# sunzeyeah/item-alignment

Hardware: AMD Instinct MI355X
Metric: item-pairs/sec (train step) RoBERTa-large+ViT-B two-tower (higher is better)
Workload: dtype bf16

## Files before the change

include/itemalign.h:

```cpp
#ifndef ITEMALIGN_H
#define ITEMALIGN_H
#include <stddef.h>
#include <stdint.h>

#ifdef __cplusplus
extern "C" {
#endif

typedef struct ihipStream_t* ia_stream_t;

#define IA_OK 0
#define IA_ERR_ARG (-1)
#define IA_ERR_LAUNCH (-2)
#define IA_ERR_WORKSPACE (-3)
#define IA_ERR_UNSUPPORTED (-4)

const char* ia_strerror(int code);
#define IA_ABI_VERSION 15
int ia_abi_version(void);

#define IA_EPI_NONE 0
#define IA_EPI_BIAS 1
#define IA_EPI_BIAS_GELU 2
#define IA_EPI_ADD 3
#define IA_EPI_DGELU 4
#define IA_EPI_BIAS_ADD 5
#define IA_EPI_DGELU_COLSUM 6
#define IA_EPI_BIAS_GELU_ACT 7
int ia_gemm_bf16(const void* A, int a_kstrided, int lda, const void* B, int b_kstrided, int ldb, void* C, int c_is_f32, int ldc,
                 int M, int N, int K, int epilogue, const float* bias, const void* aux, int ldaux, void* C2, int accumulate,
                 void* workspace, size_t workspace_bytes, ia_stream_t stream);
int ia_gemm_bf16_qscale(const void* A, int lda, const void* B, int ldb, void* C, int ldc, int M, int N, int K, const float* bias,
                        int scaled_cols, float col_scale, ia_stream_t stream);
size_t ia_gemm_workspace_bytes(int M, int N, int K, int c_is_f32);
size_t ia_gemm_colsum_workspace_bytes(int M, int N);

int ia_prof_begin(int variant, int max_launches);
int ia_prof_end(double* total_ms, double* total_flops, int* launches);
double ia_prof_bytes(void);
int ia_debug_cu_hog(int workgroups, float milliseconds, ia_stream_t stream);
int ia_debug_gemm_dynamic(int on);

int ia_ln_fwd(const void* x, const float* bias, const void* residual, void* z_out, void* y, float* mean, float* rstd,
              const float* gamma, const float* beta, int M, int H, float eps, float drop_p, uint32_t seed, uint32_t stream_id,
              ia_stream_t stream);
size_t ia_ln_bwd_workspace_bytes(int M, int H);
int ia_ln_bwd(const void* dy, const void* dres, const void* z, const float* mean, const float* rstd, const float* gamma, void* dz,
              void* dx, float* dgamma, float* dbeta, float* dbias, int M, int H, float drop_p, uint32_t seed, uint32_t stream_id,
              void* workspace, size_t workspace_bytes, int accumulate, ia_stream_t stream);
int ia_ln_bwd2(const void* dy, const void* dy2, const void* dres, const void* z, const float* mean, const float* rstd, const float* gamma,
               void* dz, void* dx, float* dgamma, float* dbeta, float* dbias, int M, int H, float drop_p, uint32_t seed, uint32_t stream_id,
               void* workspace, size_t workspace_bytes, int accumulate, ia_stream_t stream);
int ia_ln_bwd2_rows(const void* dy, const void* dy2, const void* dres, const void* z, const float* mean, const float* rstd,
                    const float* gamma, void* dz, void* dx, float* dgamma, float* dbeta, float* dbias, int M, int H, float drop_p,
                    uint32_t seed, uint32_t stream_id, const uint8_t* row_live, void* workspace, size_t workspace_bytes, int accumulate,
                    ia_stream_t stream);
size_t ia_colsum_workspace_bytes(int M, int N);
int ia_colsum(const void* x, int ld, int M, int N, float* out, int accumulate, void* workspace, size_t workspace_bytes,
              ia_stream_t stream);

int ia_attn_fwd(const void* q, const void* k, const void* v, int ld_qkv, const uint8_t* key_mask, void* out, int ld_o, float* lse2,
                int B, int nh, int L, float scale, float drop_p, uint32_t seed, ia_stream_t stream);
int ia_attn_bwd(const void* q, const void* k, const void* v, int ld_qkv, const uint8_t* key_mask, const void* out, const void* d_out,
                int ld_o, const float* lse2, float* delta, void* dq, void* dk, void* dv, int ld_dqkv, int B, int nh, int L,
                float scale, float drop_p, uint32_t seed, ia_stream_t stream);
size_t ia_attn_bwd_bias_workspace_bytes(int B, int nh, int L);
int ia_attn_bwd_bias(const void* q, const void* k, const void* v, int ld_qkv, const uint8_t* key_mask, const void* out, const void* d_out,
                     int ld_o, const float* lse2, float* delta, void* dq, void* dk, void* dv, int ld_dqkv, float* dbias, void* workspace,
                     size_t workspace_bytes, int B, int nh, int L, float scale, float drop_p, uint32_t seed, ia_stream_t stream);

int ia_attn_fwd_ps(const void* q, const void* k, const void* v, int ld_qkv, const uint8_t* key_mask, void* out, int ld_o, float* lse2,
                   int B, int nh, int L, float scale, float drop_p, uint32_t seed, ia_stream_t stream);
int ia_attn_bwd_bias_ps(const void* q, const void* k, const void* v, int ld_qkv, const uint8_t* key_mask, const void* out, const void* d_out,
                        int ld_o, const float* lse2, float* delta, void* dq, void* dk, void* dv, int ld_dqkv, float* dbias, void* workspace,
                        size_t workspace_bytes, int B, int nh, int L, float scale, float drop_p, uint32_t seed, ia_stream_t stream);
#define IA_ATTN_Q_PRESCALED 1
#define IA_ATTN_MASKED_ROWS_DEAD 2
int ia_attn_bwd_bias_ex(int flags, const void* q, const void* k, const void* v, int ld_qkv, const uint8_t* key_mask, const void* out,
                        const void* d_out, int ld_o, const float* lse2, float* delta, void* dq, void* dk, void* dv, int ld_dqkv, float* dbias,
                        void* workspace, size_t workspace_bytes, int B, int nh, int L, float scale, float drop_p, uint32_t seed,
                        ia_stream_t stream);

int ia_attn_fwd_x(const void* q, int ld_q, const void* k, const void* v, int ld_kv, const uint8_t* key_mask, void* out, int ld_o,
                  float* lse2, int B, int nh, int Lq, int Lk, float scale, float drop_p, uint32_t seed, ia_stream_t stream);
int ia_attn_bwd_x(const void* q, int ld_q, const void* k, const void* v, int ld_kv, const uint8_t* key_mask, const void* out,
                  const void* d_out, int ld_o, const float* lse2, float* delta, void* dq, int ld_dq, void* dk, void* dv, int ld_dkv,
                  int B, int nh, int Lq, int Lk, float scale, float drop_p, uint32_t seed, ia_stream_t stream);

int ia_rotary_split_fwd(const void* src, int ld_src, void* q_out, void* kv_out, int M, int n, int nh, ia_stream_t stream);
int ia_rotary_split_bwd(const void* dq, const void* dkv, void* dsrc, int ld_src, int M, int n, int nh, ia_stream_t stream);
int ia_swiglu_fwd(const void* src, int ld_src, void* out, int M, int F, ia_stream_t stream);
int ia_swiglu_bwd(const void* dout, const void* src, int ld_src, void* dsrc, int ld_dsrc, int M, int F, ia_stream_t stream);

int ia_kg_gather_fwd(const float* ent_table, const float* rel_table, const int64_t* ids, int ld_ids, int ent_col, int rel_lo,
                     float* h_sign, float* r, int B, int P, int Dk, ia_stream_t stream);
int ia_kg_gather_bwd(const float* dr, const int64_t* ids, int ld_ids, int rel_lo, float* rel_grad, int B, int P, int Dk,
                     ia_stream_t stream);
int ia_kg_rows_fwd(const float* h, const float* r, const float* hp, float* rows, int rows_per_item, int row0, int B, int P, int H,
                   ia_stream_t stream);
int ia_kg_rows_bwd(const float* drows, int rows_per_item, int row0, float* dh, float* dr, float* dhp, int B, int P, int H,
                   ia_stream_t stream);

#define IA_SIM_INNER 0
#define IA_SIM_COSINE 1
#define IA_SIM_L1 2
#define IA_SIM_L2 3
int ia_pair_sim_fwd(const float* x, const float* y, float* sim, float* probs, int B, int D, int measure, ia_stream_t stream);
int ia_pair_sim_bwd(const float* x, const float* y, const float* sim, const float* probs, const float* dsim, const float* dprobs,
                    float* dx, float* dy, int B, int D, int measure, ia_stream_t stream);

int ia_nchw_to_nhwc_bf16(const float* in, void* out, int B, int C, int H, int W, int Cp, ia_stream_t stream);
size_t ia_conv_nhwc_workspace_bytes(int B, int H, int W, int C, int Cout, int k, int stride, int groups);
int ia_conv_nhwc_fwd(const void* x, const void* what, const float* bias, void* y, int B, int H, int W, int C, int Cout, int k, int stride,
                     int groups, void* workspace, size_t workspace_bytes, ia_stream_t stream);
int ia_conv_nhwc_bwd_data(const void* dy, const void* what, void* dx, int B, int H, int W, int C, int Cout, int k, int stride, int groups,
                          void* workspace, size_t workspace_bytes, ia_stream_t stream);
int ia_conv_nhwc_bwd_weight(const void* x, const void* dy, float* dwhat, float* dbias, int B, int H, int W, int C, int Cout, int k,
                            int stride, int groups, int cols_valid, void* workspace, size_t workspace_bytes, ia_stream_t stream);
int ia_ws_conv_weight_fwd(const float* w, const float* gain, void* what, float* mean, float* rstd, int Cout, int Cg, int kk, int Cgp,
                          float scale, float eps, ia_stream_t stream);
int ia_ws_conv_weight_bwd(const float* dwhat, const float* w, const float* gain, const float* mean, const float* rstd, float* dw,
                          float* dgain, int Cout, int Cg, int kk, int Cgp, float scale, ia_stream_t stream);
int ia_silu_fwd(const void* x, void* y, size_t n, float scale, ia_stream_t stream);
int ia_silu_bwd(const void* dy, const void* x, const void* dadd, void* dx, size_t n, float scale, ia_stream_t stream);
int ia_silu_bwd_sum(const void* dy, const void* dy2, const void* x, const void* dadd, void* dx, size_t n, float scale, ia_stream_t stream);
int ia_avgpool2_fwd(const void* x, void* y, int B, int H, int W, int C, ia_stream_t stream);
int ia_avgpool2_bwd(const void* dy, void* dx, int B, int H, int W, int C, ia_stream_t stream);
size_t ia_gap_workspace_bytes(int B, int HW, int C);
int ia_gap_fwd(const void* x, float* pooled, int B, int HW, int C, void* workspace, size_t workspace_bytes, ia_stream_t stream);
int ia_gap_bwd(const float* dpooled, void* dx, int B, int HW, int C, ia_stream_t stream);
int ia_eca_fwd(const void* x, const float* conv_w, int k, const void* shortcut, void* out, float* pooled, float* gate, int B, int HW, int C,
               float coef, void* workspace, size_t workspace_bytes, ia_stream_t stream);
size_t ia_eca_fwd_linear_workspace_bytes(int B, int HW, int Cmid);
int ia_eca_fwd_linear(const void* x, const void* a, const void* what, const float* bias, int Cmid, const float* conv_w, int k,
                      const void* shortcut, void* out, void* act_out, float act_scale, float* pooled, float* gate, int B, int HW, int C,
                      float coef, void* workspace, size_t workspace_bytes, ia_stream_t stream);
int ia_eca_silu_bwd(const void* dact, const void* dact2, const void* out, const void* dout_direct, float act_scale, const void* x,
                    const float* conv_w, int k, const float* pooled, const float* gate, void* dtot, void* dx, float* dconv_w, int B, int HW,
                    int C, float coef, void* workspace, size_t workspace_bytes, ia_stream_t stream);
size_t ia_eca_bwd_workspace_bytes(int B, int HW, int C);
int ia_eca_bwd(const void* dout, const void* x, const float* conv_w, int k, const float* pooled, const float* gate, void* dx,
               float* dconv_w, int B, int HW, int C, float coef, void* workspace, size_t workspace_bytes, ia_stream_t stream);

int ia_conv3x3_padded_fwd(const void* xp, const void* what, const float* bias, void* yp, int B, int H, int W, int Cin, int Cout, int groups,
                          ia_stream_t stream);
int ia_conv3x3_padded_bwd_data(const void* dyp, const void* what, void* dxp, int B, int H, int W, int Cin, int Cout, int groups,
                               ia_stream_t stream);
int ia_conv3x3_direct_supported(int Cin, int Cout, int groups);
int ia_conv3x3_flip_weights(const void* what, void* what_t, int Cin, int Cout, int groups, ia_stream_t stream);
int ia_conv3x3_padded_bwd_data_t(const void* dyp, const void* what_t, void* dxp, int B, int H, int W, int Cin, int Cout, int groups,
                                 ia_stream_t stream);
size_t ia_conv3x3_padded_workspace_bytes(int B, int H, int W, int Cin, int Cout, int groups);
int ia_conv3x3_padded_bwd_weight(const void* xp, const void* dyp, float* dwhat, float* dbias, int B, int H, int W, int Cin, int Cout,
                                 int groups, void* workspace, size_t workspace_bytes, ia_stream_t stream);
int ia_conv3x3_s2_supported(int Cin, int Cout, int groups);
size_t ia_conv3x3_s2_padded_workspace_bytes(int B, int H, int W, int Cin, int Cout, int groups);
int ia_conv3x3_s2_padded_fwd(const void* xp, const void* what, const float* bias, void* yp, int B, int H, int W, int Cin, int Cout,
                             int groups, int y_compact, ia_stream_t stream);
int ia_conv3x3_s2_padded_bwd_weight(const void* xp, const void* dyp, float* dwhat, float* dbias, int B, int H, int W, int Cin, int Cout,
                                    int groups, int y_compact, void* workspace, size_t workspace_bytes, ia_stream_t stream);
int ia_conv3x3_s2_padded_bwd_data_t(const void* dyp, const void* what_t, void* dxp, int B, int H, int W, int Cin, int Cout, int groups,
                                    int y_compact, ia_stream_t stream);
int ia_silu_pad_fwd(const void* x, void* y, int B, int H, int W, int C, float scale, int in_padded, int out_padded, ia_stream_t stream);
int ia_pad_rows(const void* x, void* y, int B, int H, int W, int C, int in_padded, int out_padded, ia_stream_t stream);
int ia_silu_pad_bwd(const void* dy, const void* x, void* dx, int B, int H, int W, int C, float scale, int in_padded, int out_padded,
                    ia_stream_t stream);

size_t ia_bn_act_workspace_bytes(int rows, int C, int segments);
int ia_bn_act_fwd(const void* x, const float* gamma, const float* beta, float* running_mean, float* running_var, void* y, float* mean,
                  float* rstd, int rows, int C, int segments, float eps, float momentum, int training, int relu, void* workspace,
                  size_t workspace_bytes, ia_stream_t stream);
int ia_bn_act_bwd(const void* dy, const void* x, const float* gamma, const float* beta, const float* mean, const float* rstd,
                  const void* extra, void* dx, float* dgamma, float* dbeta, int rows, int C, int segments, int training, int relu,
                  void* workspace, size_t workspace_bytes, ia_stream_t stream);
size_t ia_gn_act_workspace_bytes(int rows, int C, int images);
int ia_gn_act_fwd(const void* x, const float* gamma, const float* beta, void* y, float* mean, float* rstd, int rows, int C, int images,
                  int groups, float eps, int relu, void* workspace, size_t workspace_bytes, ia_stream_t stream);
int ia_gn_act_bwd(const void* dy, const void* x, const float* gamma, const float* beta, const float* mean, const float* rstd,
                  const void* extra, void* dx, float* dgamma, float* dbeta, int rows, int C, int images, int groups, int relu,
                  void* workspace, size_t workspace_bytes, ia_stream_t stream);
int ia_patches_nchw(const float* images, void* cols, int B, int C, int H, int W, int k, int stride, int pad, int Kp, ia_stream_t stream);
int ia_maxpool3s2_fwd(const void* x, void* y, uint8_t* arg, int B, int H, int W, int C, ia_stream_t stream);
int ia_maxpool3s2_fwd_ex(const void* x, void* y, uint8_t* arg, int B, int H, int W, int C, int pad_zero, ia_stream_t stream);
int ia_maxpool3s2_bwd(const void* dy, const uint8_t* arg, void* dx, int B, int H, int W, int C, ia_stream_t stream);
int ia_rows_subsample_fwd(const void* x, void* y, int B, int H, int W, int C, int stride, ia_stream_t stream);
int ia_rows_subsample_bwd(const void* dy, const void* base, void* dx, int B, int H, int W, int C, int stride, ia_stream_t stream);
int ia_conv_weight_pack(const float* w, void* what, int Cout, int Cg, int kk, int Cgp, int ldw, ia_stream_t stream);
int ia_conv_weight_unpack_grad(const float* dwhat, float* dw, int Cout, int Cg, int kk, int Cgp, int ldw, ia_stream_t stream);

int ia_resize_pass_u8(const uint8_t* src, uint8_t* dst, const int* bounds, const int* coeffs, int ksize, int B, int in_len, int out_len,
                      int other_len, int horizontal, ia_stream_t stream);
int ia_resize_pass_u8_ex(const uint8_t* src, size_t src_pitch_bytes, size_t src_frame_bytes, uint8_t* dst, const int* bounds,
                         const int* coeffs, int ksize, int B, int in_len, int out_len, int other_len, int horizontal, ia_stream_t stream);
int ia_color_jitter_step_u8(uint8_t* frames, const int* op, const float* factor, void* scratch, int B, int H, int W, int any_contrast,
                            ia_stream_t stream);
int ia_u8_to_nchw_normalized(const uint8_t* src, const uint8_t* flip, float* out, int B, int S0, int S1, const float* mean3,
                             const float* std3, ia_stream_t stream);

int ia_embed_ln_fwd(const int64_t* ids, const int64_t* type_ids, const int64_t* pos_ids, const int32_t* extra_idx, const float* word,
                    const float* type, const float* pos, const float* extra, const float* gamma, const float* beta, void* z_out,
                    void* y, float* mean, float* rstd, int M, int H, float eps, float drop_p, uint32_t seed, uint32_t stream_id,
                    ia_stream_t stream);
size_t ia_embed_ln_bwd_workspace_bytes(int M, int H);
int ia_embed_ln_bwd(const void* dy, const void* z, const float* mean, const float* rstd, const float* gamma, const int64_t* ids,
                    const int64_t* type_ids, const int64_t* pos_ids, const int32_t* extra_idx, const int32_t* row_order,
                    const int32_t* word_order, const int32_t* pos_order, const int32_t* type_order, float* dword, float* dtype, float* dpos, float* dextra, float* dgamma, float* dbeta, int M, int H, int L, int word_pad, int pos_pad,
                    float drop_p, uint32_t seed, uint32_t stream_id, void* workspace, size_t workspace_bytes, ia_stream_t stream);

int ia_im2col_patch(const float* images, void* patches, int B, int C, int S, int P, ia_stream_t stream);
int ia_vit_tokens_fwd(const void* patch, const float* cls, const float* pos, void* tokens, int B, int NP, int H, ia_stream_t stream);
int ia_vit_tokens_bwd(const void* dtokens, void* dpatch, float* dcls, float* dpos, int B, int NP, int H, int accumulate,
                      ia_stream_t stream);

int ia_gather_rows_fwd(const void* src, int ld, const int32_t* rows, float* out, int B, int H, float drop_p, uint32_t seed,
                       uint32_t stream_id, ia_stream_t stream);
int ia_gather_rows_bwd(const float* dout, int ld, const int32_t* rows, void* dsrc, int B, int H, float drop_p, uint32_t seed,
                       uint32_t stream_id, int accumulate, ia_stream_t stream);

#define IA_ACT_NONE 0
#define IA_ACT_TANH 1
int ia_linear_small_fwd(const float* x, int ldx, const float* W, const float* bias, float* y, int B, int N, int K, int act,
                        ia_stream_t stream);
int ia_linear_small_bwd(const float* dy, const float* y, const float* x, int ldx, const float* W, float* dx, int lddx, float* dW,
                        float* db, int B, int N, int K, int act, ia_stream_t stream);
int ia_pair_head_ce_fwd(const float* x, const float* y, const float* W, const float* bias, const int64_t* labels, float* logits,
                        float* probs, float* loss, float* loss_per, int B, int D, int C, ia_stream_t stream);
int ia_pair_head_ce_bwd(const float* probs, const int64_t* labels, const float* dloss, const float* x, const float* y, const float* W,
                        float* dx, float* dy, float* dW, float* db, int B, int D, int C, ia_stream_t stream);

int ia_span_mean_fwd(const void* seq, int ld, const int* spans, float* out, int S, int H, ia_stream_t stream);
int ia_span_mean_bwd(const float* dout, const int* spans, const int* span_ptr, void* dseq, int B, int L, int H, ia_stream_t stream);

int ia_attn_fwd_varlen(const void* q, const void* k, const void* v, int ld_qkv, const int* cu_seqlens, int total_tokens, void* out, int ld_o,
                       float* lse2, int B, int nh, int Lmax, float scale, float drop_p, uint32_t seed, ia_stream_t stream);
int ia_attn_bwd_varlen(const void* q, const void* k, const void* v, int ld_qkv, const int* cu_seqlens, int total_tokens, const void* out,
                       const void* d_out, int ld_o, const float* lse2, float* delta, void* dq, void* dk, void* dv, int ld_dqkv, int B, int nh,
                       int Lmax, float scale, float drop_p, uint32_t seed, ia_stream_t stream);

int ia_attn_fwd_varlen_ps(const void* q, const void* k, const void* v, int ld_qkv, const int* cu_seqlens, int total_tokens, void* out, int ld_o,
                          float* lse2, int B, int nh, int Lmax, float scale, float drop_p, uint32_t seed, ia_stream_t stream);
int ia_attn_bwd_varlen_ps(const void* q, const void* k, const void* v, int ld_qkv, const int* cu_seqlens, int total_tokens, const void* out,
                          const void* d_out, int ld_o, const float* lse2, float* delta, void* dq, void* dk, void* dv, int ld_dqkv, int B, int nh,
                          int Lmax, float scale, float drop_p, uint32_t seed, ia_stream_t stream);

int ia_transpose_bf16_batched(const void* src, void* dst, const void* table, int n, int max_tiles, ia_stream_t stream);
int ia_adamw_flat(float* params, const float* grads, float* exp_avg, float* exp_avg_sq, void* shadow_bf16, const void* chunk_table,
                  int n_chunks, float lr, float beta1, float beta2, float eps, float weight_decay, int step, float grad_scale,
                  ia_stream_t stream);
int ia_cast_f32_to_bf16(const float* src, void* dst, size_t n, ia_stream_t stream);
int ia_cast_bf16_to_f32(const void* src, float* dst, size_t n, ia_stream_t stream);

#define IA_KGPT_SCORE 0
#define IA_KGPT_GRAD 1
#define IA_KGPT_MARGIN 2
size_t ia_kgpt_workspace_bytes(int B, int D, int use_proj);
int ia_kgpt_score(const float* ent, const float* rel, const float* proj, const int64_t* h, const int64_t* t, const int64_t* r,
                  const int64_t* nh, const int64_t* nt, int B, int D, int n_ent, int n_rel, int norm, int mode, float margin,
                  const float* dpos, const float* dneg, float* pos, float* neg, float* loss, const int32_t* ent_order, const int32_t* rel_order,
                  float* dent, float* drel, float* dproj, void* workspace, size_t workspace_bytes, ia_stream_t stream);
int ia_kgpt_adam_l2(float* params, float* grads, float* exp_avg, float* exp_avg_sq, size_t n, float lr, float beta1, float beta2,
                    float eps, float weight_decay, int step, ia_stream_t stream);
int ia_kgpt_row_normalize(float* x, int rows, int D, ia_stream_t stream);
int ia_kgpt_corrupt(const int64_t* h, const int64_t* t, const int64_t* r, int n, const float* bern_probs, int n_probs, int n_ent,
                    uint64_t seed, int64_t* nh, int64_t* nt, ia_stream_t stream);
#define IA_KGPT_LP_TAIL 0
#define IA_KGPT_LP_HEAD 1
size_t ia_kgpt_lp_workspace_bytes(int B, int D);
int ia_kgpt_lp_rank(const float* ent, const float* rel, const int64_t* h, const int64_t* t, const int64_t* r, int B, int D, int n_ent,
                    int n_rel, int norm, int side, const int64_t* grp_off, const int64_t* grp_ids, int n_grp, const int64_t* q_grp,
                    int64_t* rank, int64_t* filt_rank, float* scores, void* workspace, size_t workspace_bytes, ia_stream_t stream);

typedef struct {
  const void* w_qkv;
  const float* b_qkv;
  const void* w_o;
  const float* b_o;
  const float* ln1_g;
  const float* ln1_b;
  const void* w_fc1;
  const float* b_fc1;
  const void* w_fc2;
  const float* b_fc2;
  const float* ln2_g;
  const float* ln2_b;
  const void* wt_qkv;
  const void* wt_o;
  const void* wt_fc1;
  const void* wt_fc2;
} ia_layer_weights;

typedef struct {
  float* w_qkv; float* b_qkv; float* w_o; float* b_o; float* ln1_g; float* ln1_b;
  float* w_fc1; float* b_fc1; float* w_fc2; float* b_fc2; float* ln2_g; float* ln2_b;
} ia_layer_grads;

typedef struct {
  int B, L, H, I, nh;
  int pre_ln;
  float eps;
  float hidden_drop, attn_drop;
  uint32_t seed;
  uint32_t layer_id;
  const int* cu_seqlens;
  int total_tokens;
  float* dx_colsum_out;
  int dy_colsum_done;
  int masked_rows_dead;
} ia_layer_cfg;

size_t ia_layer_stash_bytes(const ia_layer_cfg* cfg);
size_t ia_layer_bwd_scratch_bytes(const ia_layer_cfg* cfg);
int ia_layer_fwd(const ia_layer_cfg* cfg, const ia_layer_weights* w, const void* x, const uint8_t* key_mask, void* y, void* stash,
                 ia_stream_t stream);
size_t ia_layer_infer_scratch_bytes(const ia_layer_cfg* cfg);
int ia_layer_fwd_infer(const ia_layer_cfg* cfg, const ia_layer_weights* w, const void* x, const uint8_t* key_mask, void* y, void* scratch,
                       size_t scratch_bytes, ia_stream_t stream);
int ia_layer_bwd(const ia_layer_cfg* cfg, const ia_layer_weights* w, const ia_layer_grads* g, const void* x, const uint8_t* key_mask,
                 const void* y, const void* stash, const void* dy, void* dx, void* scratch, size_t scratch_bytes, ia_stream_t stream);
int ia_layer_bwd2(const ia_layer_cfg* cfg, const ia_layer_weights* w, const ia_layer_grads* g, const void* x, const uint8_t* key_mask,
                  const void* y, const void* stash, const void* dy, const void* dy2, void* dx, void* dx2, void* scratch,
                  size_t scratch_bytes, ia_stream_t stream);

#define IA_GCN_LONG_ROW 512
#define IA_GCN_SLAB_ROWS 1024
int ia_gcn_propagate_fwd(const int64_t* rowptr, const void* col, int col_is_64, const float* val, const float* x, const float* x0,
                         float* h, int N, int C, float alpha, float drop_p, uint32_t seed, uint32_t stream_id,
                         const int32_t* long_rows, int n_long, ia_stream_t stream);
int ia_gcn_propagate_bwd(const int64_t* rowptr_t, const void* col_t, int col_is_64, const float* val_t, const float* dh, float* dx,
                         float* dx0, int dx0_accumulate, int N, int C, float alpha, float drop_p, uint32_t seed, uint32_t stream_id,
                         const int32_t* long_rows_t, int n_long_t, ia_stream_t stream);
int ia_gcn_mix_fwd(const float* h, const float* W, float* out, int N, int C, float beta, float drop_p, uint32_t seed, uint32_t stream_id,
                   ia_stream_t stream);
size_t ia_gcn_workspace_bytes(int N, int C, int F);
int ia_gcn_mix_bwd(const float* dout, const float* out, const float* h, const float* W, float* dh, float* dW, int N, int C, float beta,
                   float drop_p, void* workspace, size_t workspace_bytes, ia_stream_t stream);
int ia_gcn_input_fwd(const float* X, const float* W, const float* bias, float* x0, int N, int F, int C, float drop_p, uint32_t seed,
                     uint32_t stream_id, ia_stream_t stream);
int ia_gcn_input_bwd(const float* dx0, const float* x0, const float* X, float* dW, float* db, int N, int F, int C, float drop_p,
                     uint32_t seed, uint32_t stream_id, void* workspace, size_t workspace_bytes, ia_stream_t stream);
int ia_gcn_pair_gather_fwd(const float* x, const int32_t* idx, float* out, int R, int C, int N, float drop_p, uint32_t seed,
                           uint32_t stream_id, ia_stream_t stream);
int ia_gcn_pair_scatter_bwd(const float* dout, const int32_t* idx, const int32_t* order, float* dnode, int R, int C, int N, float drop_p,
                            uint32_t seed, uint32_t stream_id, ia_stream_t stream);

#define IA_TEXTCNN_MAX_SIZES 8
int ia_textcnn_pack_taps(const float* const* W, const int* sizes, int S, int F, int H, void* taps, ia_stream_t stream);
int ia_textcnn_pool_fwd(const float* P, int ldp, const float* const* bias, const int* sizes, int S, int F, int B, int L, float p1,
                        float p2, uint32_t seed, uint32_t stream_id1, uint32_t stream_id2, float* feat, int32_t* argmax,
                        ia_stream_t stream);
int ia_textcnn_pool_bwd_w(const float* g, const int32_t* argmax, const void* x0, const void* x1, const int* sizes, int S, int F, int B,
                          int L, int H, float p1, float p2, uint32_t seed, uint32_t stream_id1, uint32_t stream_id2, float* const* dW,
                          float* const* db, ia_stream_t stream);
int ia_textcnn_pool_bwd_x(const float* g, const int32_t* argmax, const float* const* W, const int* sizes, int S, int F, int B, int L,
                          int H, float p1, float p2, uint32_t seed, uint32_t stream_id1, uint32_t stream_id2, void* dx,
                          ia_stream_t stream);

#define IA_COMM_ID_BYTES 128
#define IA_COMM_F32 0
#define IA_COMM_BF16 1
int ia_comm_unique_id(void* id_out);
int ia_comm_init(const void* id, int rank, int world_size, void** comm_out);
int ia_comm_allreduce_bucket(void* comm, void* buf, size_t count, int dtype, ia_stream_t stream);
int ia_comm_finalize(void* comm);
const char* ia_comm_last_error(void);

#ifdef __cplusplus
}
#endif
#endif
```

item_alignment_amd/_lib.py:

```python
import ctypes as C
import os

_HERE = os.path.dirname(os.path.abspath(__file__))
LIB_PATH = os.path.join(_HERE, "libitemalign_hip.so")

vp, i32, u32, f32, sz = C.c_void_p, C.c_int, C.c_uint32, C.c_float, C.c_size_t
PP, IP = C.POINTER(C.c_void_p), C.POINTER(C.c_int)


class LayerWeights(C.Structure):
    _fields_ = [(n, vp) for n in ("w_qkv", "b_qkv", "w_o", "b_o", "ln1_g", "ln1_b", "w_fc1", "b_fc1", "w_fc2", "b_fc2",
                                  "ln2_g", "ln2_b", "wt_qkv", "wt_o", "wt_fc1", "wt_fc2")]


class LayerGrads(C.Structure):
    _fields_ = [(n, vp) for n in ("w_qkv", "b_qkv", "w_o", "b_o", "ln1_g", "ln1_b", "w_fc1", "b_fc1", "w_fc2", "b_fc2",
                                  "ln2_g", "ln2_b")]


class LayerCfg(C.Structure):
    _fields_ = [("B", i32), ("L", i32), ("H", i32), ("I", i32), ("nh", i32), ("pre_ln", i32), ("eps", f32),
                ("hidden_drop", f32), ("attn_drop", f32), ("seed", u32), ("layer_id", u32), ("cu_seqlens", vp), ("total_tokens", i32),
                ("dx_colsum_out", vp), ("dy_colsum_done", i32), ("masked_rows_dead", i32)]


SIGNATURES = {
    "ia_strerror": (C.c_char_p, [i32]),
    "ia_abi_version": (i32, []),
    "ia_gemm_bf16": (i32, [vp, i32, i32, vp, i32, i32, vp, i32, i32, i32, i32, i32, i32, vp, vp, i32, vp, i32, vp, sz, vp]),
    "ia_gemm_workspace_bytes": (sz, [i32, i32, i32, i32]),
    "ia_gemm_colsum_workspace_bytes": (sz, [i32, i32]),
    "ia_prof_begin": (i32, [i32, i32]),
    "ia_prof_end": (i32, [C.POINTER(C.c_double), C.POINTER(C.c_double), C.POINTER(i32)]),
    "ia_prof_bytes": (C.c_double, []),
    "ia_debug_cu_hog": (i32, [i32, C.c_float, vp]),
    "ia_debug_gemm_dynamic": (i32, [i32]),
    "ia_ln_fwd": (i32, [vp, vp, vp, vp, vp, vp, vp, vp, vp, i32, i32, f32, f32, u32, u32, vp]),
    "ia_ln_bwd_workspace_bytes": (sz, [i32, i32]),
    "ia_ln_bwd": (i32, [vp, vp, vp, vp, vp, vp, vp, vp, vp, vp, vp, i32, i32, f32, u32, u32, vp, sz, i32, vp]),
    "ia_ln_bwd2": (i32, [vp, vp, vp, vp, vp, vp, vp, vp, vp, vp, vp, vp, i32, i32, f32, u32, u32, vp, sz, i32, vp]),
    "ia_ln_bwd2_rows": (i32, [vp, vp, vp, vp, vp, vp, vp, vp, vp, vp, vp, vp, i32, i32, f32, u32, u32, vp, vp, sz, i32, vp]),
    "ia_colsum_workspace_bytes": (sz, [i32, i32]),
    "ia_colsum": (i32, [vp, i32, i32, i32, vp, i32, vp, sz, vp]),
    "ia_attn_fwd": (i32, [vp, vp, vp, i32, vp, vp, i32, vp, i32, i32, i32, f32, f32, u32, vp]),
    "ia_attn_bwd": (i32, [vp, vp, vp, i32, vp, vp, vp, i32, vp, vp, vp, vp, vp, i32, i32, i32, i32, f32, f32, u32, vp]),
    "ia_attn_bwd_bias_workspace_bytes": (sz, [i32, i32, i32]),
    "ia_attn_bwd_bias": (i32, [vp, vp, vp, i32, vp, vp, vp, i32, vp, vp, vp, vp, vp, i32, vp, vp, sz, i32, i32, i32, f32, f32, u32, vp]),
    "ia_attn_fwd_ps": (i32, [vp, vp, vp, i32, vp, vp, i32, vp, i32, i32, i32, f32, f32, u32, vp]),
    "ia_attn_bwd_bias_ps": (i32, [vp, vp, vp, i32, vp, vp, vp, i32, vp, vp, vp, vp, vp, i32, vp, vp, sz, i32, i32, i32, f32, f32, u32, vp]),
    "ia_attn_bwd_bias_ex": (i32, [i32, vp, vp, vp, i32, vp, vp, vp, i32, vp, vp, vp, vp, vp, i32, vp, vp, sz, i32, i32, i32, f32, f32, u32, vp]),
    "ia_gemm_bf16_qscale": (i32, [vp, i32, vp, i32, vp, i32, i32, i32, i32, vp, i32, f32, vp]),
    "ia_attn_fwd_x": (i32, [vp, i32, vp, vp, i32, vp, vp, i32, vp, i32, i32, i32, i32, f32, f32, u32, vp]),
    "ia_attn_bwd_x": (i32, [vp, i32, vp, vp, i32, vp, vp, vp, i32, vp, vp, vp, i32, vp, vp, i32, i32, i32, i32, i32, f32, f32, u32, vp]),
    "ia_rotary_split_fwd": (i32, [vp, i32, vp, vp, i32, i32, i32, vp]),
    "ia_rotary_split_bwd": (i32, [vp, vp, vp, i32, i32, i32, i32, vp]),
    "ia_swiglu_fwd": (i32, [vp, i32, vp, i32, i32, vp]),
    "ia_swiglu_bwd": (i32, [vp, vp, i32, vp, i32, i32, i32, vp]),
    "ia_kg_gather_fwd": (i32, [vp, vp, vp, i32, i32, i32, vp, vp, i32, i32, i32, vp]),
    "ia_kg_gather_bwd": (i32, [vp, vp, i32, i32, vp, i32, i32, i32, vp]),
    "ia_kg_rows_fwd": (i32, [vp, vp, vp, vp, i32, i32, i32, i32, i32, vp]),
    "ia_kg_rows_bwd": (i32, [vp, i32, i32, vp, vp, vp, i32, i32, i32, vp]),
    "ia_pair_sim_fwd": (i32, [vp, vp, vp, vp, i32, i32, i32, vp]),
    "ia_pair_sim_bwd": (i32, [vp, vp, vp, vp, vp, vp, vp, vp, i32, i32, i32, vp]),
    "ia_nchw_to_nhwc_bf16": (i32, [vp, vp, i32, i32, i32, i32, i32, vp]),
    "ia_conv_nhwc_workspace_bytes": (sz, [i32, i32, i32, i32, i32, i32, i32, i32]),
    "ia_conv_nhwc_fwd": (i32, [vp, vp, vp, vp, i32, i32, i32, i32, i32, i32, i32, i32, vp, sz, vp]),
    "ia_conv_nhwc_bwd_data": (i32, [vp, vp, vp, i32, i32, i32, i32, i32, i32, i32, i32, vp, sz, vp]),
    "ia_conv_nhwc_bwd_weight": (i32, [vp, vp, vp, vp, i32, i32, i32, i32, i32, i32, i32, i32, i32, vp, sz, vp]),
    "ia_ws_conv_weight_fwd": (i32, [vp, vp, vp, vp, vp, i32, i32, i32, i32, f32, f32, vp]),
    "ia_ws_conv_weight_bwd": (i32, [vp, vp, vp, vp, vp, vp, vp, i32, i32, i32, i32, f32, vp]),
    "ia_silu_fwd": (i32, [vp, vp, sz, f32, vp]),
    "ia_silu_bwd": (i32, [vp, vp, vp, vp, sz, f32, vp]),
    "ia_silu_bwd_sum": (i32, [vp, vp, vp, vp, vp, sz, f32, vp]),
    "ia_avgpool2_fwd": (i32, [vp, vp, i32, i32, i32, i32, vp]),
    "ia_avgpool2_bwd": (i32, [vp, vp, i32, i32, i32, i32, vp]),
    "ia_gap_workspace_bytes": (sz, [i32, i32, i32]),
    "ia_gap_fwd": (i32, [vp, vp, i32, i32, i32, vp, sz, vp]),
    "ia_gap_bwd": (i32, [vp, vp, i32, i32, i32, vp]),
    "ia_eca_fwd": (i32, [vp, vp, i32, vp, vp, vp, vp, i32, i32, i32, f32, vp, sz, vp]),
    "ia_eca_fwd_linear_workspace_bytes": (sz, [i32, i32, i32]),
    "ia_eca_fwd_linear": (i32, [vp, vp, vp, vp, i32, vp, i32, vp, vp, vp, f32, vp, vp, i32, i32, i32, f32, vp, sz, vp]),
    "ia_eca_silu_bwd": (i32, [vp, vp, vp, vp, f32, vp, vp, i32, vp, vp, vp, vp, vp, i32, i32, i32, f32, vp, sz, vp]),
    "ia_eca_bwd_workspace_bytes": (sz, [i32, i32, i32]),
    "ia_eca_bwd": (i32, [vp, vp, vp, i32, vp, vp, vp, vp, i32, i32, i32, f32, vp, sz, vp]),
    "ia_conv3x3_padded_fwd": (i32, [vp, vp, vp, vp, i32, i32, i32, i32, i32, i32, vp]),
    "ia_conv3x3_padded_bwd_data": (i32, [vp, vp, vp, i32, i32, i32, i32, i32, i32, vp]),
    "ia_conv3x3_direct_supported": (i32, [i32, i32, i32]),
    "ia_conv3x3_flip_weights": (i32, [vp, vp, i32, i32, i32, vp]),
    "ia_conv3x3_padded_bwd_data_t": (i32, [vp, vp, vp, i32, i32, i32, i32, i32, i32, vp]),
    "ia_conv3x3_padded_workspace_bytes": (sz, [i32, i32, i32, i32, i32, i32]),
    "ia_conv3x3_padded_bwd_weight": (i32, [vp, vp, vp, vp, i32, i32, i32, i32, i32, i32, vp, sz, vp]),
    "ia_pad_rows": (i32, [vp, vp, i32, i32, i32, i32, i32, i32, vp]),
    "ia_silu_pad_fwd": (i32, [vp, vp, i32, i32, i32, i32, f32, i32, i32, vp]),
    "ia_silu_pad_bwd": (i32, [vp, vp, vp, i32, i32, i32, i32, f32, i32, i32, vp]),
    "ia_bn_act_workspace_bytes": (sz, [i32, i32, i32]),
    "ia_bn_act_fwd": (i32, [vp, vp, vp, vp, vp, vp, vp, vp, i32, i32, i32, f32, f32, i32, i32, vp, sz, vp]),
    "ia_bn_act_bwd": (i32, [vp, vp, vp, vp, vp, vp, vp, vp, vp, vp, i32, i32, i32, i32, i32, vp, sz, vp]),
    "ia_patches_nchw": (i32, [vp, vp, i32, i32, i32, i32, i32, i32, i32, i32, vp]),
    "ia_conv3x3_s2_supported": (i32, [i32, i32, i32]),
    "ia_conv3x3_s2_padded_workspace_bytes": (sz, [i32, i32, i32, i32, i32, i32]),
    "ia_conv3x3_s2_padded_fwd": (i32, [vp, vp, vp, vp, i32, i32, i32, i32, i32, i32, i32, vp]),
    "ia_conv3x3_s2_padded_bwd_weight": (i32, [vp, vp, vp, vp, i32, i32, i32, i32, i32, i32, i32, vp, sz, vp]),
    "ia_conv3x3_s2_padded_bwd_data_t": (i32, [vp, vp, vp, i32, i32, i32, i32, i32, i32, i32, vp]),
    "ia_gn_act_workspace_bytes": (sz, [i32, i32, i32]),
    "ia_gn_act_fwd": (i32, [vp, vp, vp, vp, vp, vp, i32, i32, i32, i32, f32, i32, vp, sz, vp]),
    "ia_gn_act_bwd": (i32, [vp, vp, vp, vp, vp, vp, vp, vp, vp, vp, i32, i32, i32, i32, i32, vp, sz, vp]),
    "ia_maxpool3s2_fwd": (i32, [vp, vp, vp, i32, i32, i32, i32, vp]),
    "ia_maxpool3s2_fwd_ex": (i32, [vp, vp, vp, i32, i32, i32, i32, i32, vp]),
    "ia_maxpool3s2_bwd": (i32, [vp, vp, vp, i32, i32, i32, i32, vp]),
    "ia_rows_subsample_fwd": (i32, [vp, vp, i32, i32, i32, i32, i32, vp]),
    "ia_rows_subsample_bwd": (i32, [vp, vp, vp, i32, i32, i32, i32, i32, vp]),
    "ia_conv_weight_pack": (i32, [vp, vp, i32, i32, i32, i32, i32, vp]),
    "ia_conv_weight_unpack_grad": (i32, [vp, vp, i32, i32, i32, i32, i32, vp]),
    "ia_resize_pass_u8": (i32, [vp, vp, vp, vp, i32, i32, i32, i32, i32, i32, vp]),
    "ia_resize_pass_u8_ex": (i32, [vp, sz, sz, vp, vp, vp, i32, i32, i32, i32, i32, i32, vp]),
    "ia_color_jitter_step_u8": (i32, [vp, vp, vp, vp, i32, i32, i32, i32, vp]),
    "ia_u8_to_nchw_normalized": (i32, [vp, vp, vp, i32, i32, i32, C.POINTER(f32), C.POINTER(f32), vp]),
    "ia_embed_ln_fwd": (i32, [vp, vp, vp, vp, vp, vp, vp, vp, vp, vp, vp, vp, vp, vp, i32, i32, f32, f32, u32, u32, vp]),
    "ia_embed_ln_bwd_workspace_bytes": (sz, [i32, i32]),
    "ia_embed_ln_bwd": (i32, [vp, vp, vp, vp, vp, vp, vp, vp, vp, vp, vp, vp, vp, vp, vp, vp, vp, vp, vp, i32, i32, i32, i32, i32, f32, u32, u32,
                               vp, sz, vp]),
    "ia_im2col_patch": (i32, [vp, vp, i32, i32, i32, i32, vp]),
    "ia_vit_tokens_fwd": (i32, [vp, vp, vp, vp, i32, i32, i32, vp]),
    "ia_vit_tokens_bwd": (i32, [vp, vp, vp, vp, i32, i32, i32, i32, vp]),
    "ia_gather_rows_fwd": (i32, [vp, i32, vp, vp, i32, i32, f32, u32, u32, vp]),
    "ia_gather_rows_bwd": (i32, [vp, i32, vp, vp, i32, i32, f32, u32, u32, i32, vp]),
    "ia_linear_small_fwd": (i32, [vp, i32, vp, vp, vp, i32, i32, i32, i32, vp]),
    "ia_linear_small_bwd": (i32, [vp, vp, vp, i32, vp, vp, i32, vp, vp, i32, i32, i32, i32, vp]),
    "ia_pair_head_ce_fwd": (i32, [vp, vp, vp, vp, vp, vp, vp, vp, vp, i32, i32, i32, vp]),
    "ia_attn_fwd_varlen": (i32, [vp, vp, vp, i32, vp, i32, vp, i32, vp, i32, i32, i32, f32, f32, u32, vp]),
    "ia_attn_bwd_varlen": (i32, [vp, vp, vp, i32, vp, i32, vp, vp, i32, vp, vp, vp, vp, vp, i32, i32, i32, i32, f32, f32, u32, vp]),
    "ia_attn_fwd_varlen_ps": (i32, [vp, vp, vp, i32, vp, i32, vp, i32, vp, i32, i32, i32, f32, f32, u32, vp]),
    "ia_attn_bwd_varlen_ps": (i32, [vp, vp, vp, i32, vp, i32, vp, vp, i32, vp, vp, vp, vp, vp, i32, i32, i32, i32, f32, f32, u32, vp]),
    "ia_span_mean_fwd": (i32, [vp, i32, vp, vp, i32, i32, vp]),
    "ia_span_mean_bwd": (i32, [vp, vp, vp, vp, i32, i32, i32, vp]),
    "ia_pair_head_ce_bwd": (i32, [vp, vp, vp, vp, vp, vp, vp, vp, vp, vp, i32, i32, i32, vp]),
    "ia_transpose_bf16_batched": (i32, [vp, vp, vp, i32, i32, vp]),
    "ia_adamw_flat": (i32, [vp, vp, vp, vp, vp, vp, i32, f32, f32, f32, f32, f32, i32, f32, vp]),
    "ia_kgpt_workspace_bytes": (sz, [i32, i32, i32]),
    "ia_kgpt_score": (i32, [vp, vp, vp, vp, vp, vp, vp, vp, i32, i32, i32, i32, i32, i32, f32, vp, vp, vp, vp, vp, vp, vp, vp, vp, vp, vp, sz,
                            vp]),
    "ia_kgpt_adam_l2": (i32, [vp, vp, vp, vp, sz, f32, f32, f32, f32, f32, i32, vp]),
    "ia_kgpt_row_normalize": (i32, [vp, i32, i32, vp]),
    "ia_kgpt_corrupt": (i32, [vp, vp, vp, i32, vp, i32, i32, C.c_uint64, vp, vp, vp]),
    "ia_kgpt_lp_workspace_bytes": (sz, [i32, i32]),
    "ia_kgpt_lp_rank": (i32, [vp, vp, vp, vp, vp, i32, i32, i32, i32, i32, i32, vp, vp, i32, vp, vp, vp, vp, vp, sz, vp]),
    "ia_gcn_propagate_fwd": (i32, [vp, vp, i32, vp, vp, vp, vp, i32, i32, f32, f32, u32, u32, vp, i32, vp]),
    "ia_gcn_propagate_bwd": (i32, [vp, vp, i32, vp, vp, vp, vp, i32, i32, i32, f32, f32, u32, u32, vp, i32, vp]),
    "ia_gcn_mix_fwd": (i32, [vp, vp, vp, i32, i32, f32, f32, u32, u32, vp]),
    "ia_gcn_workspace_bytes": (sz, [i32, i32, i32]),
    "ia_gcn_mix_bwd": (i32, [vp, vp, vp, vp, vp, vp, i32, i32, f32, f32, vp, sz, vp]),
    "ia_gcn_input_fwd": (i32, [vp, vp, vp, vp, i32, i32, i32, f32, u32, u32, vp]),
    "ia_gcn_input_bwd": (i32, [vp, vp, vp, vp, vp, i32, i32, i32, f32, u32, u32, vp, sz, vp]),
    "ia_gcn_pair_gather_fwd": (i32, [vp, vp, vp, i32, i32, i32, f32, u32, u32, vp]),
    "ia_gcn_pair_scatter_bwd": (i32, [vp, vp, vp, vp, i32, i32, i32, f32, u32, u32, vp]),
    "ia_textcnn_pack_taps": (i32, [PP, IP, i32, i32, i32, vp, vp]),
    "ia_textcnn_pool_fwd": (i32, [vp, i32, PP, IP, i32, i32, i32, i32, f32, f32, u32, u32, u32, vp, vp, vp]),
    "ia_textcnn_pool_bwd_w": (i32, [vp, vp, vp, vp, IP, i32, i32, i32, i32, i32, f32, f32, u32, u32, u32, PP, PP, vp]),
    "ia_textcnn_pool_bwd_x": (i32, [vp, vp, PP, IP, i32, i32, i32, i32, i32, f32, f32, u32, u32, u32, vp, vp]),
    "ia_cast_f32_to_bf16": (i32, [vp, vp, sz, vp]),
    "ia_cast_bf16_to_f32": (i32, [vp, vp, sz, vp]),
    "ia_layer_stash_bytes": (sz, [C.POINTER(LayerCfg)]),
    "ia_layer_bwd_scratch_bytes": (sz, [C.POINTER(LayerCfg)]),
    "ia_layer_fwd": (i32, [C.POINTER(LayerCfg), C.POINTER(LayerWeights), vp, vp, vp, vp, vp]),
    "ia_comm_unique_id": (i32, [vp]),
    "ia_comm_init": (i32, [vp, i32, i32, C.POINTER(vp)]),
    "ia_comm_allreduce_bucket": (i32, [vp, vp, sz, i32, vp]),
    "ia_comm_finalize": (i32, [vp]),
    "ia_comm_last_error": (C.c_char_p, []),
    "ia_layer_infer_scratch_bytes": (sz, [C.POINTER(LayerCfg)]),
    "ia_layer_fwd_infer": (i32, [C.POINTER(LayerCfg), C.POINTER(LayerWeights), vp, vp, vp, vp, sz, vp]),
    "ia_layer_bwd": (i32, [C.POINTER(LayerCfg), C.POINTER(LayerWeights), C.POINTER(LayerGrads), vp, vp, vp, vp, vp, vp, vp, sz, vp]),
    "ia_layer_bwd2": (i32, [C.POINTER(LayerCfg), C.POINTER(LayerWeights), C.POINTER(LayerGrads), vp, vp, vp, vp, vp, vp, vp, vp, vp, sz, vp]),
}

_lib = None


ABI_VERSION = 15


class ItemAlignError(RuntimeError):
    pass


def load():
    global _lib
    if _lib is not None:
        return _lib
    if not os.path.exists(LIB_PATH):
        raise ItemAlignError(
            f"{LIB_PATH} not found: build it with `python -c 'import __graft_entry__ as g; g.build()'` "
            "(or `make -C item_alignment_amd/csrc`). The MI355X path has no CPU fallback.")
    import torch
    lib = C.CDLL(LIB_PATH)
    for name, (res, args) in SIGNATURES.items():
        fn = getattr(lib, name)
        fn.restype = res
        fn.argtypes = args
    got = lib.ia_abi_version()
    if got != ABI_VERSION:
        raise ItemAlignError(f"{LIB_PATH} has ABI version {got}, this package needs {ABI_VERSION} (include/itemalign.h: IA_ABI_VERSION): "
                             "stale build, run `make -C item_alignment_amd/csrc`")
    _lib = lib
    return lib


def check(rc, what):
    if rc != 0:
        msg = load().ia_strerror(rc).decode()
        raise ItemAlignError(f"{what} failed: {msg} (code {rc})")


def stream_ptr():
    import torch
    return torch.cuda.current_stream().cuda_stream


def ptr(t):
    return None if t is None else t.data_ptr()
```

item_alignment_amd/csrc/common.h:

```cpp
#pragma once
#include <hip/hip_runtime.h>
#include <stdint.h>

typedef __bf16 bf16;
typedef __attribute__((ext_vector_type(8))) __bf16 bf16x8;
typedef __attribute__((ext_vector_type(4))) __bf16 bf16x4;
typedef __attribute__((ext_vector_type(2))) __bf16 bf16x2;
typedef __attribute__((ext_vector_type(4))) short s16x4;
typedef __attribute__((ext_vector_type(8))) short s16x8;
typedef __attribute__((ext_vector_type(4))) float f32x4;
typedef __attribute__((ext_vector_type(2))) float f32x2;
typedef __attribute__((ext_vector_type(16))) float f32x16;
typedef __attribute__((ext_vector_type(4))) uint32_t u32x4;
typedef __attribute__((ext_vector_type(2))) uint32_t u32x2;

#define IA_LDS(p) ((__attribute__((address_space(3))) void*)(p))
#define IA_DEV __device__ __forceinline__

IA_DEV uint32_t ia_lds_addr(const void* p) { return (uint32_t)(uintptr_t)IA_LDS(p); }
template <int OFF>
IA_DEV s16x4 ia_tr_read(uint32_t lds_byte_addr) {
  s16x4 d;
  asm volatile("ds_read_b64_tr_b16 %0, %1 offset:%2" : "=v"(d) : "v"(lds_byte_addr), "n"(OFF));
  return d;
}

#define IA_OK 0
#define IA_ERR_ARG (-1)
#define IA_ERR_LAUNCH (-2)
#define IA_ERR_WORKSPACE (-3)
#define IA_ERR_UNSUPPORTED (-4)

IA_DEV float bf2f(bf16 v) { return (float)v; }
IA_DEV bf16 f2bf(float v) { return (bf16)v; }

IA_DEV __amdgpu_buffer_rsrc_t ia_rsrc(const void* p, uint32_t bytes) {
  return __builtin_amdgcn_make_buffer_rsrc(const_cast<void*>(p), 0, bytes, 0x00020000);
}

IA_DEV float ia_add_xor16(float x) {
  float a = x, b = x;
  asm volatile("s_nop 1\n\tv_permlane16_swap_b32 %0, %1\n\ts_nop 1" : "+v"(a), "+v"(b));
  return a + b;
}
IA_DEV float ia_add_xor32(float x) {
  float a = x, b = x;
  asm volatile("s_nop 1\n\tv_permlane32_swap_b32 %0, %1\n\ts_nop 1" : "+v"(a), "+v"(b));
  return a + b;
}

template <int CTRL>
IA_DEV float ia_dpp(float v) {
  return __builtin_bit_cast(float, __builtin_amdgcn_update_dpp(0, __builtin_bit_cast(int, v), CTRL, 0xF, 0xF, false));
}
IA_DEV float ia_lane(float v, int lane) { return __builtin_bit_cast(float, __builtin_amdgcn_readlane(__builtin_bit_cast(int, v), lane)); }
IA_DEV float row16_sum(float v) {
  v += ia_dpp<0xB1>(v);
  v += ia_dpp<0x4E>(v);
  v += ia_dpp<0x141>(v);
  v += ia_dpp<0x140>(v);
  return v;
}
IA_DEV float wave_sum(float v) {
  v = row16_sum(v);
  return (ia_lane(v, 0) + ia_lane(v, 16)) + (ia_lane(v, 32) + ia_lane(v, 48));
}
IA_DEV void half_wave_sums(float v, float& lo, float& hi) {
  v = row16_sum(v);
  lo = ia_lane(v, 0) + ia_lane(v, 16);
  hi = ia_lane(v, 32) + ia_lane(v, 48);
}
IA_DEV float wave_max(float v) {
  v = fmaxf(v, ia_dpp<0xB1>(v));
  v = fmaxf(v, ia_dpp<0x4E>(v));
  v = fmaxf(v, ia_dpp<0x141>(v));
  v = fmaxf(v, ia_dpp<0x140>(v));
  return fmaxf(fmaxf(ia_lane(v, 0), ia_lane(v, 16)), fmaxf(ia_lane(v, 32), ia_lane(v, 48)));
}

IA_DEV uint32_t ia_mix32(uint32_t x) {
  x ^= x >> 16; x *= 0x7feb352dU; x ^= x >> 15; x *= 0x846ca68bU; x ^= x >> 16;
  return x;
}
IA_DEV uint32_t ia_rng(uint32_t seed, uint32_t stream, uint32_t idx) {
  return ia_mix32(idx ^ ia_mix32(stream ^ (seed * 0x9E3779B9U)));
}

constexpr uint32_t IA_RNG_PAIR_C = 0x9E3779B1U;
IA_DEV uint32_t ia_rng_row(uint32_t seed, uint32_t stream, uint32_t row) { return ia_mix32(row ^ ia_mix32(stream ^ (seed * 0x9E3779B9U))); }
IA_DEV uint32_t ia_rng_pair(uint32_t rowkey, uint32_t pair_c) {
  const uint32_t h = (rowkey ^ pair_c) * 0x846ca68bU;
  return h ^ (h >> 16);
}

IA_DEV void gelu_parts(float x, float& cdf, float& pdf) {
  const float z = fabsf(x) * 0.70710678118654752f;
  const float t = __builtin_amdgcn_rcpf(1.0f + 0.3275911f * z);
  const float e = __builtin_amdgcn_exp2f(x * x * (-0.5f * 1.4426950408889634f));
  const float poly = t * (0.254829592f + t * (-0.284496736f + t * (1.421413741f + t * (-1.453152027f + t * 1.061405429f))));
  const float erf_abs = 1.0f - poly * e;
  cdf = 0.5f * (1.0f + copysignf(erf_abs, x));
  pdf = 0.3989422804014327f * e;
}
typedef float f32x2_t __attribute__((ext_vector_type(2)));
IA_DEV void gelu_pair(f32x2_t x, f32x2_t& act, f32x2_t& der) {
  constexpr float L2E = 1.4426950408889634f;
  constexpr float C0 = 1.5949398799788077f, C1 = 0.07403000634661838f, C2 = -0.0007007124749191571f;
  constexpr float U_MAX = C1 / (2.f * 0.0007007124749191571f);
  f32x2_t u = x * x;
  u[0] = __builtin_fminf(u[0], U_MAX); u[1] = __builtin_fminf(u[1], U_MAX);
  const f32x2_t np = (u * (-C2 * L2E) + (-C1 * L2E)) * u + (-C0 * L2E);
  const f32x2_t t = x * np;
  const f32x2_t e = {__builtin_amdgcn_exp2f(t[0]), __builtin_amdgcn_exp2f(t[1])};
  const f32x2_t den = e + 1.0f;
  const f32x2_t s = {__builtin_amdgcn_rcpf(den[0]), __builtin_amdgcn_rcpf(den[1])};
  act = x * s;
  const f32x2_t q = (u * (5.f * C2) + (3.f * C1)) * u + C0;
  const f32x2_t r = 1.0f - s;
  der = (act * r) * q + s;
}
IA_DEV f32x2_t gelu_act_pair(f32x2_t x) {
  constexpr float L2E = 1.4426950408889634f;
  constexpr float C0 = 1.5949398799788077f, C1 = 0.07403000634661838f, C2 = -0.0007007124749191571f;
  constexpr float U_MAX = C1 / (2.f * 0.0007007124749191571f);
  f32x2_t u = x * x;
  u[0] = __builtin_fminf(u[0], U_MAX); u[1] = __builtin_fminf(u[1], U_MAX);
  const f32x2_t t = x * ((u * (-C2 * L2E) + (-C1 * L2E)) * u + (-C0 * L2E));
  const f32x2_t e = {__builtin_amdgcn_exp2f(t[0]), __builtin_amdgcn_exp2f(t[1])};
  const f32x2_t den = e + 1.0f;
  return x * f32x2_t{__builtin_amdgcn_rcpf(den[0]), __builtin_amdgcn_rcpf(den[1])};
}
IA_DEV float gelu_erf(float x) { float c, d; gelu_parts(x, c, d); return x * c; }
IA_DEV float gelu_erf_grad(float x) { float c, d; gelu_parts(x, c, d); return c + x * d; }

inline hipError_t g_ia_last_hip_error = hipSuccess;
static inline int ia_check_launch() {
  hipError_t e = hipGetLastError();
  if (e != hipSuccess) g_ia_last_hip_error = e;
  return e == hipSuccess ? IA_OK : IA_ERR_LAUNCH;
}

struct IaViewGemm {
  const void* A; int a_kstrided, lda;
  const void* B; int b_kstrided, ldb;
  void* C; int c_is_f32, ldc;
  int M, N, K;
  const float* bias;
  float* rsum_out;
  void* workspace; size_t workspace_bytes;
  int a_view, b_view, pw, lca, lcbk, lcbn;
  size_t a_window, b_window;
  int groups; long ga, gb, gc, gbias;
};
__attribute__((visibility("hidden"))) int ia_gemm_view(const IaViewGemm& v, hipStream_t stream);
__attribute__((visibility("hidden"))) int ia_sum_rows_f32(const float* part, int nblk, int N, float* out, int accumulate, hipStream_t stream);
extern "C" size_t ia_colsum_workspace_bytes(int M, int N);
extern "C" int ia_colsum(const void* x, int ld, int M, int N, float* out, int accumulate, void* workspace, size_t workspace_bytes,
                         hipStream_t stream);
__attribute__((visibility("hidden"))) size_t ia_gemm_view_workspace_bytes(int M, int N, int K, int groups);
```

item_alignment_amd/csrc/engine.hip:

```cpp
#include "common.h"
#include "../../include/itemalign.h"

namespace {

inline size_t al(size_t b) { return (b + 255) & ~(size_t)255; }
inline size_t rows_of(const ia_layer_cfg* c) { return c->cu_seqlens ? (size_t)c->total_tokens : (size_t)c->B * c->L; }

struct Carver {
  char* base; size_t bytes = 0;
  char* take(size_t b) { char* r = base ? base + bytes : nullptr; bytes += al(b); return r; }
};

struct FwdBufs {
  char* qkv; char* ctx;
  char* xn;
  char* proj;
  char* ln;
  char* ffn;
  char* hpre;
  char* hact;
  float* lse; float* mean1; float* rstd1; float* mean2; float* rstd2;
  size_t bytes;
};

void name_rows(FwdBufs& s, bool pre_ln, char* t0, char* t1, char* t2) {
  if (pre_ln) { s.xn = t0; s.proj = t1; s.ln = t2; s.ffn = nullptr; }
  else { s.xn = nullptr; s.proj = t0; s.ln = t1; s.ffn = t2; }
}

FwdBufs carve_stash(const ia_layer_cfg* c, void* base) {
  const size_t M = rows_of(c), H = c->H, I = c->I;
  Carver a{(char*)base};
  FwdBufs s;
  s.qkv = a.take(M * 3 * H * 2); s.ctx = a.take(M * H * 2);
  char* t0 = a.take(M * H * 2); char* t1 = a.take(M * H * 2); char* t2 = a.take(M * H * 2);
  name_rows(s, c->pre_ln, t0, t1, t2);
  s.hpre = a.take(M * I * 2); s.hact = a.take(M * I * 2);
  s.lse = (float*)a.take((size_t)c->B * c->nh * c->L * 4);
  s.mean1 = (float*)a.take(M * 4); s.rstd1 = (float*)a.take(M * 4);
  s.mean2 = (float*)a.take(M * 4); s.rstd2 = (float*)a.take(M * 4);
  s.bytes = a.bytes;
  return s;
}

FwdBufs carve_infer(const ia_layer_cfg* c, void* base) {
  const size_t M = rows_of(c), H = c->H, I = c->I;
  Carver a{(char*)base};
  FwdBufs s;
  s.qkv = a.take(M * 3 * H * 2); s.ctx = a.take(M * H * 2);
  char* t0 = a.take(M * H * 2); char* t1 = a.take(M * H * 2);
  name_rows(s, c->pre_ln, t0, t1, t0);
  s.hpre = nullptr; s.hact = a.take(M * I * 2);
  s.lse = (float*)a.take((size_t)c->B * c->nh * c->L * 4);
  s.mean1 = s.mean2 = (float*)a.take(M * 4); s.rstd1 = s.rstd2 = (float*)a.take(M * 4);
  s.bytes = a.bytes;
  return s;
}

struct Scratch {
  char* g0; char* g1; char* g2; char* gI; char* gqkv; float* delta; char* ws; size_t ws_bytes; char* gws; size_t gws_bytes; size_t bytes;
};

size_t max3(size_t a, size_t b, size_t c) { return a > b ? (a > c ? a : c) : (b > c ? b : c); }

Scratch carve_scratch(const ia_layer_cfg* c, void* base) {
  const size_t M = rows_of(c), H = c->H, I = c->I;
  Carver a{(char*)base};
  Scratch s;
  s.g0 = a.take(M * H * 2); s.g1 = a.take(M * H * 2); s.g2 = a.take(M * H * 2);
  s.gI = a.take(M * I * 2); s.gqkv = a.take(M * 3 * H * 2);
  s.delta = (float*)a.take((size_t)c->B * c->nh * c->L * 4);
  s.ws_bytes = max3(ia_ln_bwd_workspace_bytes((int)M, (int)H), ia_gemm_colsum_workspace_bytes((int)M, (int)I),
                    max3(ia_colsum_workspace_bytes((int)M, (int)(3 * H)), ia_attn_bwd_bias_workspace_bytes(c->B, c->nh, c->L), 0));
  s.ws = a.take(s.ws_bytes);
  s.gws_bytes = max3(ia_gemm_workspace_bytes((int)(3 * H), (int)H, (int)M, 1), ia_gemm_workspace_bytes((int)I, (int)H, (int)M, 1),
                     max3(ia_gemm_workspace_bytes((int)H, (int)I, (int)M, 1), ia_gemm_workspace_bytes((int)H, (int)H, (int)M, 1), 0));
  s.gws = a.take(s.gws_bytes);
  s.bytes = a.bytes;
  return s;
}

bool cfg_ok(const ia_layer_cfg* c) {
  if (c && c->cu_seqlens && (c->total_tokens <= 0 || c->total_tokens > c->B * c->L)) return false;
  return c && c->B > 0 && c->L > 0 && c->H > 0 && c->I > 0 && c->nh > 0 && c->H == c->nh * 64 && (c->H & 7) == 0 && (c->I & 7) == 0;
}

#define IA_TRY(expr) do { int rc_ = (expr); if (rc_) return rc_; } while (0)

int dgrad(const void* dy, int k_out, const void* w, const void* wt, int n_in, void* dx, int M, int epilogue, const void* aux, int ldaux, void* c2,
          void* ws, size_t ws_bytes, ia_stream_t st) {
  if (wt)
    return ia_gemm_bf16(dy, 0, k_out, wt, 0, k_out, dx, 0, n_in, M, n_in, k_out, epilogue, nullptr, aux, ldaux, c2, 0, ws, ws_bytes, st);
  return ia_gemm_bf16(dy, 0, k_out, w, 1, n_in, dx, 0, n_in, M, n_in, k_out, epilogue, nullptr, aux, ldaux, c2, 0, ws, ws_bytes, st);
}

bool q_prescale(const ia_layer_cfg* c) { return (c->H & 127) == 0; }
int qkv_proj(const ia_layer_cfg* c, const void* x, const ia_layer_weights* w, void* qkv, int M, float scale, ia_stream_t st) {
  const int H = c->H;
  if (q_prescale(c)) return ia_gemm_bf16_qscale(x, H, w->w_qkv, H, qkv, 3 * H, M, 3 * H, H, w->b_qkv, H, scale * 1.4426950408889634f, st);
  return ia_gemm_bf16(x, 0, H, w->w_qkv, 0, H, qkv, 0, 3 * H, M, 3 * H, H, IA_EPI_BIAS, w->b_qkv, nullptr, 0, nullptr, 0, nullptr, 0, st);
}

int attn_fwd(const ia_layer_cfg* c, const char* qkv, const uint8_t* key_mask, char* ctx, float* lse, float scale, float drop, uint32_t seed,
             ia_stream_t st) {
  const int H = c->H;
  const bool ps = q_prescale(c);
  if (c->cu_seqlens)
    return (ps ? ia_attn_fwd_varlen_ps : ia_attn_fwd_varlen)(qkv, qkv + (size_t)H * 2, qkv + (size_t)2 * H * 2, 3 * H, c->cu_seqlens, c->total_tokens, ctx, H, lse, c->B, c->nh,
                              c->L, scale, drop, seed, st);
  return (ps ? ia_attn_fwd_ps : ia_attn_fwd)(qkv, qkv + (size_t)H * 2, qkv + (size_t)2 * H * 2, 3 * H, key_mask, ctx, H, lse, c->B, c->nh, c->L, scale, drop, seed, st);
}

int attn_bwd(const ia_layer_cfg* c, const char* qkv, const uint8_t* key_mask, const char* ctx, const char* dctx, const float* lse, float* delta,
             char* gqkv, float* db_qkv, void* ws, size_t ws_bytes, float scale, float drop, uint32_t seed, ia_stream_t st) {
  const int H = c->H;
  const bool ps = q_prescale(c);
  if (c->cu_seqlens) {
    int rc = (ps ? ia_attn_bwd_varlen_ps : ia_attn_bwd_varlen)(qkv, qkv + (size_t)H * 2, qkv + (size_t)2 * H * 2, 3 * H, c->cu_seqlens, c->total_tokens, ctx, dctx, H, lse, delta,
                                gqkv, gqkv + (size_t)H * 2, gqkv + (size_t)2 * H * 2, 3 * H, c->B, c->nh, c->L, scale, drop, seed, st);
    return rc ? rc : ia_colsum(gqkv, 3 * H, (int)rows_of(c), 3 * H, db_qkv, 1, ws, ws_bytes, st);
  }
  const int flags = (ps ? IA_ATTN_Q_PRESCALED : 0) | (c->masked_rows_dead ? IA_ATTN_MASKED_ROWS_DEAD : 0);
  return ia_attn_bwd_bias_ex(flags, qkv, qkv + (size_t)H * 2, qkv + (size_t)2 * H * 2, 3 * H, key_mask, ctx, dctx, H, lse, delta, gqkv,
                             gqkv + (size_t)H * 2, gqkv + (size_t)2 * H * 2, 3 * H, db_qkv, ws, ws_bytes, c->B, c->nh, c->L, scale, drop, seed, st);
}

int layer_forward(const ia_layer_cfg* c, const ia_layer_weights* w, const void* x, const uint8_t* key_mask, void* y, const FwdBufs& s,
                  bool keep, ia_stream_t st) {
  const int M = (int)rows_of(c), H = c->H, I = c->I;
  const float scale = 0.125f;
  const int gelu = keep ? IA_EPI_BIAS_GELU : IA_EPI_BIAS_GELU_ACT;
  if (!c->pre_ln) {
    const float hidden_drop = keep ? c->hidden_drop : 0.f, attn_drop = keep ? c->attn_drop : 0.f;
    const uint32_t seed = keep ? c->seed : 0u, attn_seed = keep ? c->seed * 2654435761u + c->layer_id * 97u + 17u : 0u;
    const uint32_t ln1_stream = keep ? c->layer_id * 4u + 0u : 0u, ln2_stream = keep ? c->layer_id * 4u + 1u : 0u;
    IA_TRY(qkv_proj(c, x, w, s.qkv, M, scale, st));
    IA_TRY(attn_fwd(c, s.qkv, key_mask, s.ctx, s.lse, scale, attn_drop, attn_seed, st));
    IA_TRY(ia_gemm_bf16(s.ctx, 0, H, w->w_o, 0, H, s.proj, 0, H, M, H, H, IA_EPI_NONE, nullptr, nullptr, 0, nullptr, 0, nullptr, 0, st));
    IA_TRY(ia_ln_fwd(s.proj, w->b_o, x, keep ? s.proj : nullptr, s.ln, s.mean1, s.rstd1, w->ln1_g, w->ln1_b, M, H, c->eps, hidden_drop, seed,
                     ln1_stream, st));
    IA_TRY(ia_gemm_bf16(s.ln, 0, H, w->w_fc1, 0, H, s.hact, 0, I, M, I, H, gelu, w->b_fc1, nullptr, 0, s.hpre, 0, nullptr, 0, st));
    IA_TRY(ia_gemm_bf16(s.hact, 0, I, w->w_fc2, 0, I, s.ffn, 0, H, M, H, I, IA_EPI_NONE, nullptr, nullptr, 0, nullptr, 0, nullptr, 0, st));
    IA_TRY(ia_ln_fwd(s.ffn, w->b_fc2, s.ln, keep ? s.ffn : nullptr, y, s.mean2, s.rstd2, w->ln2_g, w->ln2_b, M, H, c->eps, hidden_drop, seed,
                     ln2_stream, st));
  } else {
    IA_TRY(ia_ln_fwd(x, nullptr, nullptr, nullptr, s.xn, s.mean1, s.rstd1, w->ln1_g, w->ln1_b, M, H, c->eps, 0.f, 0, 0, st));
    IA_TRY(qkv_proj(c, s.xn, w, s.qkv, M, scale, st));
    IA_TRY(attn_fwd(c, s.qkv, key_mask, s.ctx, s.lse, scale, 0.f, 0, st));
    IA_TRY(ia_gemm_bf16(s.ctx, 0, H, w->w_o, 0, H, s.proj, 0, H, M, H, H, IA_EPI_NONE, nullptr, nullptr, 0, nullptr, 0, nullptr, 0, st));
    IA_TRY(ia_ln_fwd(s.proj, w->b_o, x, s.proj, s.ln, s.mean2, s.rstd2, w->ln2_g, w->ln2_b, M, H, c->eps, 0.f, 0, 0, st));
    IA_TRY(ia_gemm_bf16(s.ln, 0, H, w->w_fc1, 0, H, s.hact, 0, I, M, I, H, gelu, w->b_fc1, nullptr, 0, s.hpre, 0, nullptr, 0, st));
    IA_TRY(ia_gemm_bf16(s.hact, 0, I, w->w_fc2, 0, I, y, 0, H, M, H, I, IA_EPI_BIAS_ADD, w->b_fc2, s.proj, H, nullptr, 0, nullptr, 0, st));
  }
  return IA_OK;
}

}

extern "C" size_t ia_layer_stash_bytes(const ia_layer_cfg* cfg) {
  (void)hipGetLastError();
  if (!cfg_ok(cfg)) return 0;
  return carve_stash(cfg, nullptr).bytes;
}

extern "C" size_t ia_layer_bwd_scratch_bytes(const ia_layer_cfg* cfg) {
  (void)hipGetLastError();
  if (!cfg_ok(cfg)) return 0;
  return carve_scratch(cfg, nullptr).bytes;
}

extern "C" size_t ia_layer_infer_scratch_bytes(const ia_layer_cfg* cfg) {
  (void)hipGetLastError();
  if (!cfg_ok(cfg)) return 0;
  return carve_infer(cfg, nullptr).bytes;
}

extern "C" int ia_layer_fwd(const ia_layer_cfg* c, const ia_layer_weights* w, const void* x, const uint8_t* key_mask, void* y,
                            void* stash, ia_stream_t st) {
  (void)hipGetLastError();
  if (!cfg_ok(c) || !w || !x || !y || !stash) return IA_ERR_ARG;
  if (c->pre_ln && (c->hidden_drop > 0.f || c->attn_drop > 0.f)) return IA_ERR_UNSUPPORTED;
  return layer_forward(c, w, x, key_mask, y, carve_stash(c, stash), true, st);
}

extern "C" int ia_layer_fwd_infer(const ia_layer_cfg* c, const ia_layer_weights* w, const void* x, const uint8_t* key_mask, void* y,
                                  void* scratch, size_t scratch_bytes, ia_stream_t st) {
  (void)hipGetLastError();
  if (!cfg_ok(c) || !w || !x || !y || !scratch) return IA_ERR_ARG;
  if (scratch_bytes < ia_layer_infer_scratch_bytes(c)) return IA_ERR_WORKSPACE;
  return layer_forward(c, w, x, key_mask, y, carve_infer(c, scratch), false, st);
}

extern "C" int ia_layer_bwd2(const ia_layer_cfg* c, const ia_layer_weights* w, const ia_layer_grads* g, const void* x,
                             const uint8_t* key_mask, const void* y, const void* stash, const void* dy, const void* dy2, void* dx, void* dx2,
                             void* scratch, size_t scratch_bytes, ia_stream_t st);

extern "C" int ia_layer_bwd(const ia_layer_cfg* c, const ia_layer_weights* w, const ia_layer_grads* g, const void* x,
                            const uint8_t* key_mask, const void* y, const void* stash, const void* dy, void* dx, void* scratch,
                            size_t scratch_bytes, ia_stream_t st) {
  return ia_layer_bwd2(c, w, g, x, key_mask, y, stash, dy, nullptr, dx, nullptr, scratch, scratch_bytes, st);
}

extern "C" int ia_layer_bwd2(const ia_layer_cfg* c, const ia_layer_weights* w, const ia_layer_grads* g, const void* x,
                             const uint8_t* key_mask, const void* y, const void* stash, const void* dy, const void* dy2, void* dx, void* dx2,
                             void* scratch, size_t scratch_bytes, ia_stream_t st) {
  (void)hipGetLastError();
  (void)y;
  if (!cfg_ok(c) || !w || !g || !x || !stash || !dy || !dx || !scratch) return IA_ERR_ARG;
  if (c->pre_ln && (dy2 || dx2)) return IA_ERR_UNSUPPORTED;
  if (scratch_bytes < ia_layer_bwd_scratch_bytes(c)) return IA_ERR_WORKSPACE;
  const int M = (int)rows_of(c), H = c->H, I = c->I;
  const FwdBufs s = carve_stash(c, const_cast<void*>(stash));
  const Scratch k = carve_scratch(c, scratch);
  const float scale = 0.125f;
  const uint32_t attn_seed = c->seed * 2654435761u + c->layer_id * 97u + 17u;
  const bool drop = c->hidden_drop > 0.f;
  if (!c->pre_ln) {
    const uint8_t* const live = (c->masked_rows_dead && !c->cu_seqlens) ? key_mask : nullptr;
    IA_TRY(ia_ln_bwd2_rows(dy, dy2, nullptr, s.ffn, s.mean2, s.rstd2, w->ln2_g, k.g0, drop ? k.g1 : nullptr, g->ln2_g, g->ln2_b, g->b_fc2, M, H,
                           c->hidden_drop, c->seed, c->layer_id * 4u + 1u, live, k.ws, k.ws_bytes, 1, st));
    const char* d_ffn = drop ? k.g1 : k.g0;
    IA_TRY(ia_gemm_bf16(d_ffn, 1, H, s.hact, 1, I, g->w_fc2, 1, I, H, I, M, IA_EPI_NONE, nullptr, nullptr, 0, nullptr, 1, k.gws, k.gws_bytes, st));
    IA_TRY(dgrad(d_ffn, H, w->w_fc2, w->wt_fc2, I, k.gI, M, IA_EPI_DGELU_COLSUM, s.hpre, I, g->b_fc1, k.ws, k.ws_bytes, st));
    IA_TRY(ia_gemm_bf16(k.gI, 1, I, s.ln, 1, H, g->w_fc1, 1, H, I, H, M, IA_EPI_NONE, nullptr, nullptr, 0, nullptr, 1, k.gws, k.gws_bytes, st));
    IA_TRY(dgrad(k.gI, I, w->w_fc1, w->wt_fc1, H, k.g2, M, IA_EPI_NONE, nullptr, 0, nullptr, nullptr, 0, st));
    char* dz1buf = dx2 ? (char*)dx2 : k.g0;
    IA_TRY(ia_ln_bwd2_rows(k.g2, k.g0, nullptr, s.proj, s.mean1, s.rstd1, w->ln1_g, dz1buf, drop ? k.g1 : nullptr, g->ln1_g, g->ln1_b, g->b_o, M, H,
                           c->hidden_drop, c->seed, c->layer_id * 4u + 0u, live, k.ws, k.ws_bytes, 1, st));
    const char* d_att = drop ? k.g1 : dz1buf;
    IA_TRY(ia_gemm_bf16(d_att, 1, H, s.ctx, 1, H, g->w_o, 1, H, H, H, M, IA_EPI_NONE, nullptr, nullptr, 0, nullptr, 1, k.gws, k.gws_bytes, st));
    IA_TRY(dgrad(d_att, H, w->w_o, w->wt_o, H, k.g2, M, IA_EPI_NONE, nullptr, 0, nullptr, nullptr, 0, st));
    IA_TRY(attn_bwd(c, s.qkv, key_mask, s.ctx, k.g2, s.lse, k.delta, k.gqkv, g->b_qkv, k.ws, k.ws_bytes, scale, c->attn_drop, attn_seed, st));
    IA_TRY(ia_gemm_bf16(k.gqkv, 1, 3 * H, x, 1, H, g->w_qkv, 1, H, 3 * H, H, M, IA_EPI_NONE, nullptr, nullptr, 0, nullptr, 1, k.gws, k.gws_bytes, st));
    if (dx2)
      IA_TRY(dgrad(k.gqkv, 3 * H, w->w_qkv, w->wt_qkv, H, dx, M, IA_EPI_NONE, nullptr, 0, nullptr, nullptr, 0, st));
    else
      IA_TRY(dgrad(k.gqkv, 3 * H, w->w_qkv, w->wt_qkv, H, dx, M, IA_EPI_ADD, dz1buf, H, nullptr, nullptr, 0, st));
  } else {
    if (!c->dy_colsum_done) IA_TRY(ia_colsum(dy, H, M, H, g->b_fc2, 1, k.ws, k.ws_bytes, st));
    IA_TRY(ia_gemm_bf16(dy, 1, H, s.hact, 1, I, g->w_fc2, 1, I, H, I, M, IA_EPI_NONE, nullptr, nullptr, 0, nullptr, 1, k.gws, k.gws_bytes, st));
    IA_TRY(dgrad(dy, H, w->w_fc2, w->wt_fc2, I, k.gI, M, IA_EPI_DGELU_COLSUM, s.hpre, I, g->b_fc1, k.ws, k.ws_bytes, st));
    IA_TRY(ia_gemm_bf16(k.gI, 1, I, s.ln, 1, H, g->w_fc1, 1, H, I, H, M, IA_EPI_NONE, nullptr, nullptr, 0, nullptr, 1, k.gws, k.gws_bytes, st));
    IA_TRY(dgrad(k.gI, I, w->w_fc1, w->wt_fc1, H, k.g0, M, IA_EPI_NONE, nullptr, 0, nullptr, nullptr, 0, st));
    IA_TRY(ia_ln_bwd(k.g0, dy, s.proj, s.mean2, s.rstd2, w->ln2_g, k.g1, nullptr, g->ln2_g, g->ln2_b, g->b_o, M, H, 0.f, 0, 0, k.ws,
                     k.ws_bytes, 1, st));
    IA_TRY(ia_gemm_bf16(k.g1, 1, H, s.ctx, 1, H, g->w_o, 1, H, H, H, M, IA_EPI_NONE, nullptr, nullptr, 0, nullptr, 1, k.gws, k.gws_bytes, st));
    IA_TRY(dgrad(k.g1, H, w->w_o, w->wt_o, H, k.g2, M, IA_EPI_NONE, nullptr, 0, nullptr, nullptr, 0, st));
    IA_TRY(attn_bwd(c, s.qkv, key_mask, s.ctx, k.g2, s.lse, k.delta, k.gqkv, g->b_qkv, k.ws, k.ws_bytes, scale, 0.f, 0, st));
    IA_TRY(ia_gemm_bf16(k.gqkv, 1, 3 * H, s.xn, 1, H, g->w_qkv, 1, H, 3 * H, H, M, IA_EPI_NONE, nullptr, nullptr, 0, nullptr, 1, k.gws, k.gws_bytes, st));
    IA_TRY(dgrad(k.gqkv, 3 * H, w->w_qkv, w->wt_qkv, H, k.g0, M, IA_EPI_NONE, nullptr, 0, nullptr, nullptr, 0, st));
    IA_TRY(ia_ln_bwd(k.g0, k.g1, x, s.mean1, s.rstd1, w->ln1_g, dx, nullptr, g->ln1_g, g->ln1_b, c->dx_colsum_out, M, H, 0.f, 0, 0, k.ws,
                     k.ws_bytes, 1, st));
  }
  return IA_OK;
}
```

item_alignment_amd/csrc/gemm.hip:

```cpp
#include "common.h"
#include <atomic>
#include <cstdlib>
#include <type_traits>

#ifndef IA_GEMM_DBG_HOOKS
#define IA_GEMM_DBG_HOOKS 0
#endif
#define IA_DBG(p) (IA_GEMM_DBG_HOOKS ? (p).dbg : 0)

namespace {

constexpr int BK = 64;
constexpr uint32_t OOB = 0xFFFFFFF0u;

enum { EPI_NONE = 0, EPI_BIAS = 1, EPI_BIAS_GELU = 2, EPI_ADD = 3, EPI_DGELU = 4, EPI_BIAS_ADD = 5, EPI_DGELU_CS = 6, EPI_BIAS_GELU_ACT = 7 };

struct GemmArgs {
  const bf16* A; const bf16* B; void* C; bf16* C2; const float* bias; const bf16* aux;
  int M, N, K;
  int lda, ldb, ldc, ldaux;
  uint64_t a_bytes, b_bytes;
  int accumulate;
  int qcols; float qscale;
  int tiles_m, tiles_n;
  int splits, nk_per_split;
  float* csum_part;
  int split_id;
  float* ws;
  float* rsum_out;
  float* rsum_ws;
  int dbg;
  int a_view, b_view, pw, lca, lcbk, lcbn;
  int groups;
  long ga, gb, gc, gbias;
  uint32_t* tile_ctr;
};

constexpr int CTR_SLOTS = 1024, CTR_WORDS = 16;
__device__ uint32_t g_tile_ctr[CTR_SLOTS * CTR_WORDS];

IA_DEV int tap_delta(int t, int pw) { return (t / 3 - 1) * pw + (t % 3 - 1); }

IA_DEV __amdgpu_buffer_rsrc_t rsrc_at(const bf16* base, uint64_t total_bytes, uint64_t origin) {
  const uint64_t ob = origin * 2, rem = total_bytes > ob ? total_bytes - ob : 0;
  return ia_rsrc(base + origin, (uint32_t)(rem < 0x7FFFFFF0ull ? rem : 0x7FFFFFF0ull));
}

template <int EPI, bool OUTF32>
IA_DEV void epi_store4(const GemmArgs& p, int m, int n, f32x4 v) {
  if (EPI == EPI_BIAS || EPI == EPI_BIAS_GELU || EPI == EPI_BIAS_GELU_ACT || EPI == EPI_BIAS_ADD) {
    const f32x4 b = *reinterpret_cast<const f32x4*>(p.bias + n);
    v += b;
    if (EPI == EPI_BIAS && n < p.qcols) v *= p.qscale;
  }
  if (EPI == EPI_BIAS_GELU) {
    bf16x4 der;
#pragma unroll
    for (int r = 0; r < 4; r += 2) {
      f32x2_t a, d;
      gelu_pair(f32x2_t{v[r], v[r + 1]}, a, d);
      v[r] = a[0]; v[r + 1] = a[1];
      der[r] = f2bf(d[0]); der[r + 1] = f2bf(d[1]);
    }
    *reinterpret_cast<bf16x4*>(p.C2 + (size_t)m * p.ldc + n) = der;
  }
  if (EPI == EPI_BIAS_GELU_ACT) {
#pragma unroll
    for (int r = 0; r < 4; r += 2) {
      const f32x2_t a = gelu_act_pair(f32x2_t{v[r], v[r + 1]});
      v[r] = a[0]; v[r + 1] = a[1];
    }
  }
  if (EPI == EPI_ADD || EPI == EPI_BIAS_ADD) {
    const bf16x4 a = *reinterpret_cast<const bf16x4*>(p.aux + (size_t)m * p.ldaux + n);
#pragma unroll
    for (int r = 0; r < 4; ++r) v[r] += bf2f(a[r]);
  }
  if (EPI == EPI_DGELU || EPI == EPI_DGELU_CS) {
    const bf16x4 a = *reinterpret_cast<const bf16x4*>(p.aux + (size_t)m * p.ldaux + n);
#pragma unroll
    for (int r = 0; r < 4; ++r) v[r] *= bf2f(a[r]);
  }
  if (OUTF32) {
    if (p.splits > 1) {
      *reinterpret_cast<f32x4*>(p.ws + ((size_t)p.split_id * p.M + m) * p.N + n) = v;
      return;
    }
    float* c = reinterpret_cast<float*>(p.C) + (size_t)m * p.ldc + n;
    if (p.accumulate) { const f32x4 o = *reinterpret_cast<const f32x4*>(c); v += o; }
    *reinterpret_cast<f32x4*>(c) = v;
  } else {
    bf16x4 o = {f2bf(v[0]), f2bf(v[1]), f2bf(v[2]), f2bf(v[3])};
    *reinterpret_cast<bf16x4*>(reinterpret_cast<bf16*>(p.C) + (size_t)m * p.ldc + n) = o;
  }
}

template <typename V>
IA_DEV void gstore16(void* ptr, V v) {
  static_assert(sizeof(V) == 16, "16-byte store");
  *reinterpret_cast<V*>(ptr) = v;
}
template <int EPI, bool OUTF32>
constexpr int epi_stores_per_call() { return OUTF32 ? 2 : (EPI == EPI_BIAS_GELU ? 2 : 1); }
template <int EPI>
constexpr int epi_extra_stores() { return EPI == EPI_DGELU_CS ? 2 : 0; }

struct BufIO { __amdgpu_buffer_rsrc_t rsC, rsC2; uint32_t off; };
template <int EPI, bool OUTF32, bool PRE, bool BUF = false>
IA_DEV void epi_store8(const GemmArgs& p, int m, int n, f32x4 lo, f32x4 hi, f32x4 pb0, f32x4 pb1, bf16x8 ax, float (&cs)[8], const BufIO* io = nullptr) {
  float v[8] = {lo[0], lo[1], lo[2], lo[3], hi[0], hi[1], hi[2], hi[3]};
  if (EPI == EPI_BIAS || EPI == EPI_BIAS_GELU || EPI == EPI_BIAS_GELU_ACT || EPI == EPI_BIAS_ADD) {
    const f32x4 b0 = PRE ? pb0 : *reinterpret_cast<const f32x4*>(p.bias + n), b1 = PRE ? pb1 : *reinterpret_cast<const f32x4*>(p.bias + n + 4);
#pragma unroll
    for (int r = 0; r < 4; ++r) { v[r] += b0[r]; v[4 + r] += b1[r]; }
    if (EPI == EPI_BIAS && n < p.qcols) {
#pragma unroll
      for (int r = 0; r < 8; ++r) v[r] *= p.qscale;
    }
  }
  if (EPI == EPI_BIAS_GELU) {
    bf16x8 der;
    {
      constexpr float L2E = 1.4426950408889634f;
      constexpr float C0 = 1.5949398799788077f, C1 = 0.07403000634661838f, C2 = -0.0007007124749191571f;
      constexpr float U_MAX = C1 / (2.f * 0.0007007124749191571f);
      f32x2_t x[4], u[4], t[4], e[4], sg[4], act[4], q[4], d[4];
#pragma unroll
      for (int i = 0; i < 4; ++i) { x[i] = f32x2_t{v[2 * i], v[2 * i + 1]}; u[i] = x[i] * x[i]; }
#pragma unroll
      for (int i = 0; i < 4; ++i) { u[i][0] = __builtin_fminf(u[i][0], U_MAX); u[i][1] = __builtin_fminf(u[i][1], U_MAX); }
#pragma unroll
      for (int i = 0; i < 4; ++i) t[i] = x[i] * ((u[i] * (-C2 * L2E) + (-C1 * L2E)) * u[i] + (-C0 * L2E));
#pragma unroll
      for (int i = 0; i < 4; ++i) e[i] = f32x2_t{__builtin_amdgcn_exp2f(t[i][0]), __builtin_amdgcn_exp2f(t[i][1])};
#pragma unroll
      for (int i = 0; i < 4; ++i) { e[i] = e[i] + 1.0f; q[i] = (u[i] * (5.f * C2) + (3.f * C1)) * u[i] + C0; }
#pragma unroll
      for (int i = 0; i < 4; ++i) sg[i] = f32x2_t{__builtin_amdgcn_rcpf(e[i][0]), __builtin_amdgcn_rcpf(e[i][1])};
#pragma unroll
      for (int i = 0; i < 4; ++i) { act[i] = x[i] * sg[i]; d[i] = (act[i] * (1.0f - sg[i])) * q[i] + sg[i]; }
#pragma unroll
      for (int i = 0; i < 4; ++i) {
        v[2 * i] = act[i][0]; v[2 * i + 1] = act[i][1];
        der[2 * i] = f2bf(d[i][0]); der[2 * i + 1] = f2bf(d[i][1]);
      }
    }
    if (BUF) __builtin_amdgcn_raw_buffer_store_b128(__builtin_bit_cast(u32x4, der), io->rsC2, (int)io->off, 0, 0);
    else gstore16(((IA_DBG(p) & 1024) ? reinterpret_cast<bf16*>(p.C) : p.C2) + (size_t)m * p.ldc + n, der);
  }
  if (EPI == EPI_BIAS_GELU_ACT) {
    constexpr float L2E = 1.4426950408889634f;
    constexpr float C0 = 1.5949398799788077f, C1 = 0.07403000634661838f, C2 = -0.0007007124749191571f;
    constexpr float U_MAX = C1 / (2.f * 0.0007007124749191571f);
    f32x2_t x[4], u[4], t[4], e[4];
#pragma unroll
    for (int i = 0; i < 4; ++i) { x[i] = f32x2_t{v[2 * i], v[2 * i + 1]}; u[i] = x[i] * x[i]; }
#pragma unroll
    for (int i = 0; i < 4; ++i) { u[i][0] = __builtin_fminf(u[i][0], U_MAX); u[i][1] = __builtin_fminf(u[i][1], U_MAX); }
#pragma unroll
    for (int i = 0; i < 4; ++i) t[i] = x[i] * ((u[i] * (-C2 * L2E) + (-C1 * L2E)) * u[i] + (-C0 * L2E));
#pragma unroll
    for (int i = 0; i < 4; ++i) e[i] = f32x2_t{__builtin_amdgcn_exp2f(t[i][0]), __builtin_amdgcn_exp2f(t[i][1])} + 1.0f;
    f32x2_t sg[4], act[4];
#pragma unroll
    for (int i = 0; i < 4; ++i) sg[i] = f32x2_t{__builtin_amdgcn_rcpf(e[i][0]), __builtin_amdgcn_rcpf(e[i][1])};
#pragma unroll
    for (int i = 0; i < 4; ++i) act[i] = x[i] * sg[i];
#pragma unroll
    for (int i = 0; i < 4; ++i) { v[2 * i] = act[i][0]; v[2 * i + 1] = act[i][1]; }
  }
  if (EPI == EPI_ADD || EPI == EPI_BIAS_ADD || EPI == EPI_DGELU || EPI == EPI_DGELU_CS) {
    const bf16x8 a = PRE ? ax : *reinterpret_cast<const bf16x8*>(p.aux + (size_t)m * p.ldaux + n);
#pragma unroll
    for (int r = 0; r < 8; ++r) {
      if (EPI == EPI_DGELU || EPI == EPI_DGELU_CS) v[r] *= bf2f(a[r]);
      else v[r] += bf2f(a[r]);
      if (EPI == EPI_DGELU_CS) cs[r] += v[r];
    }
  }
  if (OUTF32) {
    float* c = p.splits > 1 ? p.ws + ((size_t)p.split_id * p.M + m) * p.N + n : reinterpret_cast<float*>(p.C) + (size_t)m * p.ldc + n;
    f32x4 o0 = {v[0], v[1], v[2], v[3]}, o1 = {v[4], v[5], v[6], v[7]};
    if (p.splits <= 1 && p.accumulate) { o0 += *reinterpret_cast<const f32x4*>(c); o1 += *reinterpret_cast<const f32x4*>(c + 4); }
    gstore16(c, o0);
    gstore16(c + 4, o1);
  } else {
    bf16x8 o;
#pragma unroll
    for (int r = 0; r < 8; ++r) o[r] = f2bf(v[r]);
    if (BUF) __builtin_amdgcn_raw_buffer_store_b128(__builtin_bit_cast(u32x4, o), io->rsC, (int)io->off, 0, 0);
    else gstore16(reinterpret_cast<bf16*>(p.C) + (size_t)m * p.ldc + n, o);
  }
}

IA_DEV int xcd_chunk(int bid, int nwg) {
  const int q = nwg >> 3, r = nwg & 7, xcd = bid & 7, idx = bid >> 3;
  return (xcd < r ? xcd * (q + 1) : r * (q + 1) + (xcd - r) * q) + idx;
}
IA_DEV void tile_of_order(const GemmArgs& p, int t, int& bm, int& bn) {
  const int GM = 8;
  const int group = t / (GM * p.tiles_n);
  const int first_m = group * GM;
  const int gsz = min(p.tiles_m - first_m, GM);
  bm = first_m + (t % (GM * p.tiles_n)) % gsz;
  bn = (t % (GM * p.tiles_n)) / gsz;
}
IA_DEV void tile_of_index(const GemmArgs& p, int bid, int nwg, int& bm, int& bn) { tile_of_order(p, xcd_chunk(bid, nwg), bm, bn); }

namespace t128 {
constexpr int BM = 128, BN = 128, TILE_BYTES = 16384;
constexpr int A3_ROWS = 136, A3_BYTES = A3_ROWS * 128, SMEM_BYTES = 2 * A3_BYTES + 2 * TILE_BYTES;
static_assert(SMEM_BYTES >= 4 * TILE_BYTES && 2 * SMEM_BYTES <= 160 * 1024, "two workgroups per CU");

IA_DEV int ks_swz(int k) { return ((k & 3) | (((k >> 3) & 1) << 2)) << 1; }

template <bool KS>
IA_DEV void stage_tile(__amdgpu_buffer_rsrc_t rs, char* s, int kt, int x0, int ld, int K, int tid, int wave, int korg, int view = 0, int pw = 0,
                       int lck = 6, int lcn = 6) {
#pragma unroll
  for (int issue = 0; issue < 4; ++issue) {
    uint32_t off;
    if (!KS) {
      const int row = issue * 32 + (tid >> 3);
      const int c = (tid & 7) ^ (row & 7);
      const int k = kt * BK + c * 8;
      if (view == 0) off = (uint32_t)(((x0 + row) * ld + k) * 2);
      else off = (uint32_t)(((x0 + row + view * tap_delta(k >> lck, pw)) * ld + (k & ((1 << lck) - 1))) * 2);
      if (k >= K) off = OOB;
    } else {
      const int row = issue * 16 + (tid >> 4);
      const int c = (tid & 15) ^ ks_swz(row);
      const int k = kt * BK + row;
      if (view == 0) off = (uint32_t)(((k - korg) * ld + x0 + c * 8) * 2);
      else if (view == 1) off = (uint32_t)(((k & ((1 << lck) - 1)) * ld + ((k >> lck) << lcn) + x0 + c * 8) * 2);
      else { const int col = x0 + c * 8; off = (uint32_t)(((k - korg + tap_delta(col >> lcn, pw)) * ld + (col & ((1 << lcn) - 1))) * 2); }
      if (k >= K) off = OOB;
    }
    __builtin_amdgcn_raw_ptr_buffer_load_lds(rs, IA_LDS(s + issue * 4096 + wave * 1024), 16, off, 0, 0, 0);
  }
}

IA_DEV bf16x8 frag_kc(const char* s, int row, int chunk) {
  return *reinterpret_cast<const bf16x8*>(s + row * 128 + ((chunk ^ (row & 7)) << 4));
}

IA_DEV bf16x8 frag_ks(const char* s, int k, int col) {
  const int addr = k * 256 + ((((col >> 3) ^ ks_swz(k))) << 4) + (col & 7) * 2;
  const uint32_t a = ia_lds_addr(s) + (uint32_t)addr;
  s16x4 lo = ia_tr_read<0>(a);
  s16x4 hi = ia_tr_read<4 * 256>(a);
  s16x8 r = {lo[0], lo[1], lo[2], lo[3], hi[0], hi[1], hi[2], hi[3]};
  return __builtin_bit_cast(bf16x8, r);
}

template <bool AKS, bool BKS, int EPI, bool OUTF32>
__global__ __launch_bounds__(256, 2) void gemm_kernel(GemmArgs p) {
  __shared__ __attribute__((aligned(16))) char smem[SMEM_BYTES];
  const int tid = threadIdx.x, lane = tid & 63;
  const int wave = __builtin_amdgcn_readfirstlane(tid >> 6);
  const int wm = wave >> 1, wn = wave & 1;
  int bm, bn, grp = 0;
  p.split_id = 0;
  if (p.groups > 1 || p.splits > 1) {
    int w = xcd_chunk(blockIdx.x, gridDim.x);
    bn = w % p.tiles_n; w /= p.tiles_n;
    grp = w % p.groups; w /= p.groups;
    bm = w % p.tiles_m;
    p.split_id = w / p.tiles_m;
  } else {
    tile_of_index(p, blockIdx.x, gridDim.x, bm, bn);
  }
  const int m0 = bm * BM, n0 = bn * BN;
  if (p.groups > 1) {
    const long z = grp;
    p.A += z * p.ga; p.B += z * p.gb;
    p.a_bytes -= (uint64_t)(z * p.ga * 2); p.b_bytes -= (uint64_t)(z * p.gb * 2);
    p.C = reinterpret_cast<char*>(p.C) + z * p.gc * (OUTF32 ? 4 : 2);
    if (p.bias) p.bias += z * p.gbias;
    if (p.ws) p.ws += z * (long)p.splits * p.M * p.N;
  }

  f32x4 acc[4][4];
#pragma unroll
  for (int i = 0; i < 4; ++i)
#pragma unroll
    for (int j = 0; j < 4; ++j) acc[i][j] = f32x4{0.f, 0.f, 0.f, 0.f};

  const int nk_all = (p.K + BK - 1) / BK;
  const int kt0 = p.split_id * p.nk_per_split;
  const int nk = min(nk_all, kt0 + p.nk_per_split);
  const int a_org = !AKS ? max(0, m0 - (p.a_view ? p.pw + 1 : 0)) : kt0 * BK;
  const int b_org = !BKS ? n0 : (p.b_view == 1 ? 0 : max(0, kt0 * BK - (p.b_view == 2 ? p.pw + 1 : 0)));
  const __amdgpu_buffer_rsrc_t rsA = rsrc_at(p.A, p.a_bytes, (uint64_t)a_org * p.lda);
  const __amdgpu_buffer_rsrc_t rsB = rsrc_at(p.B, p.b_bytes, (uint64_t)b_org * p.ldb);
  const int xa = AKS ? m0 : m0 - a_org, xb = BKS ? n0 : 0;
  const bool row3 = !AKS && p.a_view != 0 && p.lca == 6 && p.K == 9 * BK && p.splits == 1 && p.N <= 64;
  if (!row3) {
    stage_tile<AKS>(rsA, smem, kt0, xa, p.lda, p.K, tid, wave, a_org, p.a_view, p.pw, p.lca, 0);
    stage_tile<BKS>(rsB, smem + TILE_BYTES, kt0, xb, p.ldb, p.K, tid, wave, b_org, p.b_view, p.pw, p.lcbk, p.lcbn);
    asm volatile("s_waitcnt vmcnt(0)" ::: "memory");
    __syncthreads();
  }

  const int g = lane >> 4, li = lane & 15;
  const bool m_narrow = p.M - m0 <= 64, n_narrow = p.N - n0 <= 64;
  const bool ksplit = m_narrow || n_narrow;
  int qm = wm, qn = wn, my_ks = 0;
  bool helper_idle = false;
  if (n_narrow && !m_narrow) { qn = 0; my_ks = wn; }
  else if (m_narrow && !n_narrow) { qm = 0; my_ks = wm; }
  else if (m_narrow && n_narrow) { qm = 0; qn = 0; my_ks = wave & 1; helper_idle = wave >= 2; }
  const bool quadrant_live = !helper_idle && m0 + qm * 64 < p.M && n0 + qn * 64 < p.N;
  constexpr bool WGRAD = AKS && BKS && OUTF32 && EPI == EPI_NONE;
  const bool row_sums = WGRAD && p.rsum_out != nullptr && bn == 0 && qn == 0;
  f32x4 racc[4];
  bf16x8 ones;
#pragma unroll
  for (int i = 0; i < 4; ++i) racc[i] = f32x4{0.f, 0.f, 0.f, 0.f};
#pragma unroll
  for (int i = 0; i < 8; ++i) ones[i] = f2bf(1.0f);
  if (row3) {
    char* const A3 = smem;
    char* const B2 = smem + 2 * A3_BYTES;
    auto stage_a3 = [&](int gy, int b3) {
      char* const s3 = A3 + b3 * A3_BYTES;
      const int shift = p.a_view * (gy - 1) * p.pw - 1;
#pragma unroll
      for (int issue = 0; issue < 4; ++issue) {
        const int j = issue * 32 + (tid >> 3);
        const uint32_t off = (uint32_t)(((xa + j + shift) * p.lda + (((tid & 7) ^ (j & 7)) * 8)) * 2);
        __builtin_amdgcn_raw_ptr_buffer_load_lds(rsA, IA_LDS(s3 + issue * 4096 + wave * 1024), 16, off, 0, 0, 0);
      }
      if (wave == 0) {
        const int j = 128 + (lane >> 3);
        const uint32_t off = (uint32_t)(((xa + j + shift) * p.lda + (((lane & 7) ^ (j & 7)) * 8)) * 2);
        __builtin_amdgcn_raw_ptr_buffer_load_lds(rsA, IA_LDS(s3 + 16384), 16, off, 0, 0, 0);
      }
    };
    stage_a3(0, 0);
    stage_tile<BKS>(rsB, B2, 0, xb, p.ldb, p.K, tid, wave, b_org, p.b_view, p.pw, p.lcbk, p.lcbn);
    asm volatile("s_waitcnt vmcnt(0)" ::: "memory");
    __syncthreads();
    for (int kt = 0; kt < 9; ++kt) {
      const int gy = kt / 3, dxi = kt - 3 * gy, bb = kt & 1;
      if (kt + 1 < 9) stage_tile<BKS>(rsB, B2 + (bb ^ 1) * TILE_BYTES, kt + 1, xb, p.ldb, p.K, tid, wave, b_org, p.b_view, p.pw, p.lcbk, p.lcbn);
      if (dxi == 0 && gy < 2) stage_a3(gy + 1, (gy + 1) & 1);
      const char* sA = A3 + (gy & 1) * A3_BYTES;
      const char* sB = B2 + bb * TILE_BYTES;
      const int rowoff = 1 + p.a_view * (dxi - 1);
      if (quadrant_live)
#pragma unroll
      for (int ks = 0; ks < 2; ++ks) {
        if (ksplit && ks != my_ks) continue;
        bf16x8 af[4], bfr[4];
#pragma unroll
        for (int mi = 0; mi < 4; ++mi) af[mi] = frag_kc(sA, qm * 64 + mi * 16 + li + rowoff, ks * 4 + g);
#pragma unroll
        for (int ni = 0; ni < 4; ++ni) {
          if (!BKS) bfr[ni] = frag_kc(sB, qn * 64 + (li >> 2) * 16 + ni * 4 + (li & 3), ks * 4 + g);
          else      bfr[ni] = frag_ks(sB, ks * 32 + g * 8 + (li >> 2), qn * 64 + ni * 16 + (li & 3) * 4);
        }
        if (BKS) {
          asm volatile("s_waitcnt lgkmcnt(0)" ::: "memory");
          __builtin_amdgcn_sched_barrier(0);
        }
#pragma unroll
        for (int mi = 0; mi < 4; ++mi)
#pragma unroll
          for (int ni = 0; ni < 4; ++ni)
            acc[mi][ni] = __builtin_amdgcn_mfma_f32_16x16x32_bf16(bfr[ni], af[mi], acc[mi][ni], 0, 0, 0);
      }
      asm volatile("s_waitcnt vmcnt(0)" ::: "memory");
      __syncthreads();
    }
  } else
  for (int kt = kt0; kt < nk; ++kt) {
    const int buf = (kt - kt0) & 1;
    if (kt + 1 < nk) {
      char* nb = smem + (buf ^ 1) * 2 * TILE_BYTES;
      stage_tile<AKS>(rsA, nb, kt + 1, xa, p.lda, p.K, tid, wave, a_org, p.a_view, p.pw, p.lca, 0);
      stage_tile<BKS>(rsB, nb + TILE_BYTES, kt + 1, xb, p.ldb, p.K, tid, wave, b_org, p.b_view, p.pw, p.lcbk, p.lcbn);
    }
    const char* sA = smem + buf * 2 * TILE_BYTES;
    const char* sB = sA + TILE_BYTES;
    if (quadrant_live)
#pragma unroll
    for (int ks = 0; ks < 2; ++ks) {
      if (ksplit && ks != my_ks) continue;
      bf16x8 af[4], bfr[4];
#pragma unroll
      for (int mi = 0; mi < 4; ++mi) {
        if (!AKS) af[mi] = frag_kc(sA, qm * 64 + mi * 16 + li, ks * 4 + g);
        else      af[mi] = frag_ks(sA, ks * 32 + g * 8 + (li >> 2), qm * 64 + mi * 16 + (li & 3) * 4);
      }
#pragma unroll
      for (int ni = 0; ni < 4; ++ni) {
        if (!BKS) bfr[ni] = frag_kc(sB, qn * 64 + (li >> 2) * 16 + ni * 4 + (li & 3), ks * 4 + g);
        else      bfr[ni] = frag_ks(sB, ks * 32 + g * 8 + (li >> 2), qn * 64 + ni * 16 + (li & 3) * 4);
      }
      if (AKS || BKS) {
        asm volatile("s_waitcnt lgkmcnt(0)" ::: "memory");
        __builtin_amdgcn_sched_barrier(0);
      }
#pragma unroll
      for (int mi = 0; mi < 4; ++mi)
#pragma unroll
        for (int ni = 0; ni < 4; ++ni)
          acc[mi][ni] = __builtin_amdgcn_mfma_f32_16x16x32_bf16(bfr[ni], af[mi], acc[mi][ni], 0, 0, 0);
      if (WGRAD && row_sums)
#pragma unroll
        for (int mi = 0; mi < 4; ++mi) racc[mi] = __builtin_amdgcn_mfma_f32_16x16x32_bf16(ones, af[mi], racc[mi], 0, 0, 0);
    }
    asm volatile("s_waitcnt vmcnt(0)" ::: "memory");
    __syncthreads();
  }

  if (ksplit) {
    float* const xch = reinterpret_cast<float*>(smem) + (size_t)(qm * 2 + qn) * (20 * 64 * 4);
    if (quadrant_live && my_ks == 1) {
#pragma unroll
      for (int mi = 0; mi < 4; ++mi) {
#pragma unroll
        for (int ni = 0; ni < 4; ++ni) *reinterpret_cast<f32x4*>(xch + ((mi * 4 + ni) * 64 + lane) * 4) = acc[mi][ni];
        *reinterpret_cast<f32x4*>(xch + ((16 + mi) * 64 + lane) * 4) = racc[mi];
      }
    }
    __syncthreads();
    if (!quadrant_live || my_ks == 1) return;
#pragma unroll
    for (int mi = 0; mi < 4; ++mi) {
#pragma unroll
      for (int ni = 0; ni < 4; ++ni) acc[mi][ni] += *reinterpret_cast<const f32x4*>(xch + ((mi * 4 + ni) * 64 + lane) * 4);
      racc[mi] += *reinterpret_cast<const f32x4*>(xch + ((16 + mi) * 64 + lane) * 4);
    }
  }

#pragma unroll
  for (int mi = 0; mi < 4; ++mi) {
    const int m = m0 + qm * 64 + mi * 16 + li;
    if (m >= p.M) continue;
#pragma unroll
    for (int ni = 0; ni < 4; ++ni) {
      const int n = n0 + qn * 64 + (BKS ? ni * 16 + g * 4 : g * 16 + ni * 4);
      if (n >= p.N) continue;
      epi_store4<EPI, OUTF32>(p, m, n, acc[mi][ni]);
    }
  }
  if (WGRAD && row_sums && g == 0) {
#pragma unroll
    for (int mi = 0; mi < 4; ++mi) {
      const int m = m0 + qm * 64 + mi * 16 + li;
      if (m >= p.M) continue;
      if (p.splits > 1) p.rsum_ws[((size_t)grp * p.splits + p.split_id) * p.M + m] = racc[mi][0];
      else p.rsum_out[(size_t)grp * p.M + m] += racc[mi][0];
    }
  }
}
}

namespace t256w {
constexpr int BM = 256, BN = 256, TILE_BYTES = 32768;
constexpr int STAGE_BYTES = 16 * 64 * 4;
constexpr int LDS_BYTES = 2 * 2 * TILE_BYTES + 8 * STAGE_BYTES;

template <bool KS> struct Op;
template <> struct Op<false> { bf16x8 v[4]; };
template <> struct Op<true> { s16x4 lo[4], hi[4]; };
IA_DEV bf16x8 frag_of(const Op<false>& o, int j) { return o.v[j]; }
IA_DEV bf16x8 frag_of(const Op<true>& o, int j) {
  s16x8 r = {o.lo[j][0], o.lo[j][1], o.lo[j][2], o.lo[j][3], o.hi[j][0], o.hi[j][1], o.hi[j][2], o.hi[j][3]};
  return __builtin_bit_cast(bf16x8, r);
}

template <int IMM>
IA_DEV bf16x8 rd128(uint32_t addr) {
  bf16x8 d;
  asm volatile("ds_read_b128 %0, %1 offset:%2" : "=v"(d) : "v"(addr), "n"(IMM));
  return d;
}
template <int IMM>
IA_DEV s16x4 rd_tr(uint32_t addr) {
  s16x4 d;
  asm volatile("ds_read_b64_tr_b16 %0, %1 offset:%2" : "=v"(d) : "v"(addr), "n"(IMM));
  return d;
}

template <bool KS>
IA_DEV void frag_bases(uint32_t (&base)[4], uint32_t tile_addr, int x0, int lane, int nperm_row) {
  if (!KS) {
    const int hh = lane >> 5;
    const int row = x0 + nperm_row;
#pragma unroll
    for (int ks = 0; ks < 4; ++ks) base[ks] = tile_addr + row * 128 + ((((ks * 2 + hh) ^ ((row >> 1) & 7))) << 4);
  } else {
    const int p = lane & 15, G = lane >> 4;
#pragma unroll
    for (int j = 0; j < 4; ++j) {
      const int row = 8 * (G >> 1) + (p >> 2);
      const int col = x0 + j * 32 + 16 * (G & 1) + (p & 3) * 4;
      base[j] = tile_addr + row * 512 + ((((col >> 3) ^ ((row & 3) << 2))) << 4) + (col & 7) * 2;
    }
  }
}

template <int N> IA_DEV void tie(Op<false>& o) {
  asm volatile("s_waitcnt lgkmcnt(%4)" : "+v"(o.v[0]), "+v"(o.v[1]), "+v"(o.v[2]), "+v"(o.v[3]) : "n"(N));
}
template <int N> IA_DEV void tie2(Op<false>& a, Op<false>& b) {
  asm volatile("s_waitcnt lgkmcnt(%8)" : "+v"(a.v[0]), "+v"(a.v[1]), "+v"(a.v[2]), "+v"(a.v[3]), "+v"(b.v[0]), "+v"(b.v[1]), "+v"(b.v[2]), "+v"(b.v[3]) : "n"(N));
}
template <int N> IA_DEV void tie6(Op<false>& a, Op<false>& b, Op<false>& c, Op<false>& d, Op<false>& e, Op<false>& f) {
  asm volatile("s_waitcnt lgkmcnt(%24)"
               : "+v"(a.v[0]), "+v"(a.v[1]), "+v"(a.v[2]), "+v"(a.v[3]), "+v"(b.v[0]), "+v"(b.v[1]), "+v"(b.v[2]), "+v"(b.v[3]),
                 "+v"(c.v[0]), "+v"(c.v[1]), "+v"(c.v[2]), "+v"(c.v[3]), "+v"(d.v[0]), "+v"(d.v[1]), "+v"(d.v[2]), "+v"(d.v[3]),
                 "+v"(e.v[0]), "+v"(e.v[1]), "+v"(e.v[2]), "+v"(e.v[3]), "+v"(f.v[0]), "+v"(f.v[1]), "+v"(f.v[2]), "+v"(f.v[3])
               : "n"(N));
}
template <int N> IA_DEV void tie(Op<true>& o) {
  asm volatile("s_waitcnt lgkmcnt(%8)" : "+v"(o.lo[0]), "+v"(o.lo[1]), "+v"(o.lo[2]), "+v"(o.lo[3]), "+v"(o.hi[0]), "+v"(o.hi[1]), "+v"(o.hi[2]), "+v"(o.hi[3]) : "n"(N));
}
template <int N> IA_DEV void tie2(Op<true>& a, Op<true>& b) { tie<N>(a); tie<N>(b); }
template <int N> IA_DEV void tie6(Op<true>& a, Op<true>& b, Op<true>& c, Op<true>& d, Op<true>& e, Op<true>& f) {
  tie<N>(a); tie<N>(b); tie<N>(c); tie<N>(d); tie<N>(e); tie<N>(f);
}


template <int S, bool KS>
IA_DEV void read_frag(Op<KS>& f, int j, const uint32_t (&base)[4], uint32_t bufoff) {
  if constexpr (!KS) {
    const uint32_t a = base[S] + bufoff;
    if (j == 0) f.v[0] = rd128<0>(a);
    if (j == 1) f.v[1] = rd128<4096>(a);
    if (j == 2) f.v[2] = rd128<8192>(a);
    if (j == 3) f.v[3] = rd128<12288>(a);
  } else {
    f.lo[j] = rd_tr<S * 8192>(base[j] + bufoff);
    f.hi[j] = rd_tr<S * 8192 + 4 * 512>(base[j] + bufoff);
  }
}

template <bool FRESH, typename FA, typename FB, typename Filler>
IA_DEV void mfma_step(f32x16 (&acc)[4][4], const FA& fa, const FB& fb, Filler&& filler) {
  bf16x8 va[4], vb[4];
#pragma unroll
  for (int j = 0; j < 4; ++j) { va[j] = frag_of(fa, j); vb[j] = frag_of(fb, j); }
#pragma unroll
  for (int mi = 0; mi < 4; ++mi)
#pragma unroll
    for (int ni = 0; ni < 4; ++ni) {
      if constexpr (FRESH) {
        const f32x16 z = {0.f, 0.f, 0.f, 0.f, 0.f, 0.f, 0.f, 0.f, 0.f, 0.f, 0.f, 0.f, 0.f, 0.f, 0.f, 0.f};
        acc[mi][ni] = __builtin_amdgcn_mfma_f32_32x32x16_bf16(vb[ni], va[mi], z, 0, 0, 0);
      } else acc[mi][ni] = __builtin_amdgcn_mfma_f32_32x32x16_bf16(vb[ni], va[mi], acc[mi][ni], 0, 0, 0);
      filler(mi * 4 + ni);
      __builtin_amdgcn_sched_barrier(0);
    }
}

template <bool AKS, bool BKS, int PEND, bool PEEL_OK = true>
IA_DEV void main_loop(const GemmArgs& p, char* smem, f32x16 (&acc)[4][4], __amdgpu_buffer_rsrc_t rsA, __amdgpu_buffer_rsrc_t rsB, int xa, int xb,
                      int kt0, int ktaA0, int ktaB0, int n_tiles, int nk_all, int wm, int wn, int wave, int lane, bool prologue_only,
                      bool stores_in_flight) {
  constexpr bool ROUND = !AKS && !BKS;
  const int li = lane & 31;
  const int gt = wave * 64 + lane;
  uint32_t voffA, stepA, voffB, stepB;
  if (!AKS) { const int row = gt >> 3; voffA = (uint32_t)(((xa + row) * p.lda + (((gt & 7) ^ ((row >> 1) & 7)) * 8)) * 2); stepA = (uint32_t)(32 * p.lda * 2); }
  else { const int row = gt >> 5; voffA = (uint32_t)((row * p.lda + xa + (((gt & 31) ^ ((row & 3) << 2)) * 8)) * 2); stepA = (uint32_t)(8 * p.lda * 2); }
  if (!BKS) { const int row = gt >> 3; voffB = (uint32_t)(((xb + row) * p.ldb + (((gt & 7) ^ ((row >> 1) & 7)) * 8)) * 2); stepB = (uint32_t)(32 * p.ldb * 2); }
  else { const int row = gt >> 5; voffB = (uint32_t)((row * p.ldb + xb + (((gt & 31) ^ ((row & 3) << 2)) * 8)) * 2); stepB = (uint32_t)(8 * p.ldb * 2); }
  const uint32_t kstepA = AKS ? (uint32_t)(BK * p.lda * 2) : (uint32_t)(BK * 2), kstepB = BKS ? (uint32_t)(BK * p.ldb * 2) : (uint32_t)(BK * 2);
  const int klA = AKS ? (gt >> 5) : ((gt & 7) ^ (((gt >> 3) >> 1) & 7)) * 8;
  const int klB = BKS ? (gt >> 5) : ((gt & 7) ^ (((gt >> 3) >> 1) & 7)) * 8;
  char* const my_part = smem + wave * 1024;
  const int dbg = IA_GEMM_DBG_HOOKS ? p.dbg : 0;
  const bool dma_on = !(dbg & 2);

  auto dma_piece = [&](int u, int i) {
    const bool isB = i >= 8;
    const int j = i & 7;
    char* dst = my_part + (isB ? TILE_BYTES : 0) + (u & 1) * 2 * TILE_BYTES + j * 4096;
    const int kt = kt0 + u, kta = (dbg & 4) ? 0 : (isB ? ktaB0 : ktaA0) + u;
    const bool ks = isB ? BKS : AKS;
    const uint32_t soff = (uint32_t)kta * (isB ? kstepB : kstepA) + (uint32_t)j * (isB ? stepB : stepA);
    if (ks) {
      const uint32_t off = dma_on ? (isB ? voffB : voffA) + soff : OOB;
      __builtin_amdgcn_raw_ptr_buffer_load_lds(isB ? rsB : rsA, IA_LDS(dst), 16, off, 0, 0, 0);
    } else {
      const int lim = (u < n_tiles && dma_on) ? p.K - kt * BK : 0;
      const uint32_t off = (isB ? klB : klA) + (ks ? j * 8 : 0) < lim ? (isB ? voffB : voffA) : OOB;
      __builtin_amdgcn_raw_ptr_buffer_load_lds(isB ? rsB : rsA, IA_LDS(dst), 16, off, (int)soff, 0, 0);
    }
  };

  auto off_of = [&](int u, bool isB) -> uint32_t {
    const int lim = (u < n_tiles && dma_on) ? p.K - (kt0 + u) * BK : 0;
    return (isB ? klB : klA) < lim ? (isB ? voffB : voffA) : OOB;
  };
  auto dma_c = [&](int u, int i, uint32_t off) {
    const bool isB = i >= 8;
    const int j = i & 7;
    char* dst = my_part + (isB ? TILE_BYTES : 0) + (u & 1) * 2 * TILE_BYTES + j * 4096;
    const int kta = (dbg & 4) ? 0 : (isB ? ktaB0 : ktaA0) + u;
    const uint32_t soff = (uint32_t)kta * (isB ? kstepB : kstepA) + (uint32_t)j * (isB ? stepB : stepA);
    __builtin_amdgcn_raw_ptr_buffer_load_lds(isB ? rsB : rsA, IA_LDS(dst), 16, off, (int)soff, 0, 0);
  };

  uint32_t runA = voffA + (uint32_t)((dbg & 4) ? 0 : ktaA0 + 2) * kstepA, runB = voffB + (uint32_t)((dbg & 4) ? 0 : ktaB0 + 2) * kstepB;
  auto dma_run = [&](int u, int i) {
    const bool isB = i >= 8;
    if (!(isB ? BKS : AKS) || (dbg & 4)) { dma_piece(u, i); return; }
    const int j = i & 7;
    char* dst = my_part + (isB ? TILE_BYTES : 0) + (u & 1) * 2 * TILE_BYTES + j * 4096;
    const uint32_t off = (isB ? runB : runA) + (uint32_t)j * (isB ? stepB : stepA);
    __builtin_amdgcn_raw_ptr_buffer_load_lds(isB ? rsB : rsA, IA_LDS(dst), 16, dma_on ? off : OOB, 0, 0, 0);
  };

  if (prologue_only) {
#pragma unroll
    for (int i = 0; i < 16; ++i) dma_piece(0, i);
#pragma unroll
    for (int i = 0; i < (ROUND ? 12 : 16); ++i) dma_piece(1, i);
    return;
  }
  if (stores_in_flight) asm volatile("s_waitcnt vmcnt(%0)" : : "n"(PEND < 60 ? PEND : 60) : "memory");
  else asm volatile("s_waitcnt vmcnt(0)" ::: "memory");
  __builtin_amdgcn_s_barrier();

  const int nperm = ((li >> 2) & 1) * 16 + (li >> 3) * 4 + (li & 3);
  uint32_t baseA[4], baseB[4];
  const uint32_t smem_addr = ia_lds_addr(smem);
  frag_bases<AKS>(baseA, smem_addr, wm * 128, lane, li);
  frag_bases<BKS>(baseB, smem_addr + TILE_BYTES, wn * 128, lane, nperm);
  constexpr int NRA = AKS ? 8 : 4, NRB = BKS ? 8 : 4, NR = NRA + NRB;
  constexpr int NR15 = NR > 15 ? 15 : NR;

  Op<AKS> a0, a1, a2, a3;
  Op<BKS> b0, b1, b2, b3;
#pragma unroll
  for (int j = 0; j < 4; ++j) read_frag<0>(a0, j, baseA, 0u);
#pragma unroll
  for (int j = 0; j < 4; ++j) read_frag<0>(b0, j, baseB, 0u);

  using Acc = std::false_type;

  uint32_t bo = 0;
  int u = 0;
  if constexpr (ROUND) {
  uint32_t offA = OOB, offB = off_of(1, true);
  auto trip = [&](auto FIRST_T) {
    const uint32_t bn = bo ^ (uint32_t)(2 * TILE_BYTES);
    tie2<0>(a0, b0);
    mfma_step<decltype(FIRST_T)::value>(acc, a0, b0, [&](int i) {
      if (i < 4) { read_frag<1>(a1, i, baseA, bo); read_frag<1>(b1, i, baseB, bo); }
      else if (i < 8) { read_frag<2>(a2, i - 4, baseA, bo); read_frag<2>(b2, i - 4, baseB, bo); }
      else if (i < 12) { read_frag<3>(a3, i - 8, baseA, bo); read_frag<3>(b3, i - 8, baseB, bo); }
      if (i % 4 == 3) dma_c(u + 1, 12 + i / 4, offB);
      if (i == 12) offA = off_of(u + 2, false);
    });
    tie6<0>(a1, b1, a2, b2, a3, b3);
    __builtin_amdgcn_sched_barrier(0);
    if (!(dbg & 16)) __builtin_amdgcn_s_barrier();
    __builtin_amdgcn_sched_barrier(0);
    mfma_step<false>(acc, a1, b1, [&](int i) {
      if (i % 4 == 1) dma_c(u + 2, i / 4, offA);
    });
    mfma_step<false>(acc, a2, b2, [&](int i) {
      if (i % 4 == 1) dma_c(u + 2, 4 + i / 4, offA);
      if (i == 14) offB = off_of(u + 2, true);
    });
    asm volatile("s_waitcnt vmcnt(8)" ::: "memory");
    __builtin_amdgcn_sched_barrier(0);
    if (!(dbg & 16)) __builtin_amdgcn_s_barrier();
    __builtin_amdgcn_sched_barrier(0);
    mfma_step<false>(acc, a3, b3, [&](int i) {
      if (i < 4) read_frag<0>(a0, i, baseA, bn);
      else if (i < 8) read_frag<0>(b0, i - 4, baseB, bn);
      if (i % 4 == 3) dma_c(u + 2, 8 + i / 4, offB);
    });
    bo = bn;
    ++u;
    };
  if constexpr (PEEL_OK) {
    trip(std::true_type{});
    do { trip(Acc{}); } while (u < n_tiles);
  } else {
    do { trip(Acc{}); } while (u < n_tiles);
  }
  tie2<0>(a0, b0);
  return;
  }
  do {
    const uint32_t bn = bo ^ (uint32_t)(2 * TILE_BYTES);
    tie<0>(a0); tie<0>(b0);
    mfma_step<false>(acc, a0, b0, [&](int i) {
      if (i < 4) read_frag<1>(a1, i, baseA, bo);
      else if (i < 8) read_frag<1>(b1, i - 4, baseB, bo);
      else if (i < 12) read_frag<2>(a2, i - 8, baseA, bo);
      else read_frag<2>(b2, i - 12, baseB, bo);
    });
    tie<NR15>(a1); tie<NR15>(b1);
    mfma_step<false>(acc, a1, b1, [&](int i) {
      if (i < 4) read_frag<3>(a3, i, baseA, bo);
      else if (i < 8) read_frag<3>(b3, i - 4, baseB, bo);
    });
    tie<0>(a2); tie<0>(b2); tie<0>(a3); tie<0>(b3);
    __builtin_amdgcn_sched_barrier(0);
    if (!(dbg & 16)) __builtin_amdgcn_s_barrier();
    __builtin_amdgcn_sched_barrier(0);
    mfma_step<false>(acc, a2, b2, [&](int i) {
      if (i & 1) dma_run(u + 2, i >> 1);
    });
    asm volatile("s_waitcnt vmcnt(8)" ::: "memory");
    __builtin_amdgcn_sched_barrier(0);
    if (!(dbg & 16)) __builtin_amdgcn_s_barrier();
    __builtin_amdgcn_sched_barrier(0);
    mfma_step<false>(acc, a3, b3, [&](int i) {
      if (i & 1) dma_run(u + 2, 8 + (i >> 1));
      if (!(i & 1)) {
        if (i < 8) read_frag<0>(a0, i >> 1, baseA, bn);
        else read_frag<0>(b0, (i - 8) >> 1, baseB, bn);
      }
    });
    bo = bn;
    ++u;
    if (AKS) { runA += kstepA; asm volatile("" : "+v"(runA)); }
    if (BKS) { runB += kstepB; asm volatile("" : "+v"(runB)); }
  } while (u < n_tiles);
  tie<0>(a0); tie<0>(b0);
}

template <bool BKS, int NH, bool WITH_BIAS>
IA_DEV void drain_half_plain(const GemmArgs& p, f32x16 (&acc)[4][4], int m0, int n0, char* stg, int lane_e, const f32x4 (&bct)[4][4], float ts = 1.f) {
  static_assert(!(WITH_BIAS && BKS), "bias rows are laid out for the k-contiguous B fragment permutation");
  const int hh = lane_e >> 5, li = lane_e & 31, rrow = lane_e >> 3, c8 = lane_e & 7;
  auto stage = [&](int mi) {
    char* const sl = stg + (mi & 1) * 4096;
#pragma unroll
    for (int ni = 0; ni < 2; ++ni) {
      f32x16& a = acc[mi][NH * 2 + ni];
      if (!BKS) {
#pragma unroll
        for (int h8 = 0; h8 < 2; ++h8) {
          f32x4 t0, t1;
#pragma unroll
          for (int j = 0; j < 4; ++j) {
            asm volatile("v_accvgpr_read_b32 %0, %1" : "=v"(t0[j]) : "a"(a[h8 * 8 + j]));
            asm volatile("v_accvgpr_read_b32 %0, %1" : "=v"(t1[j]) : "a"(a[h8 * 8 + 4 + j]));
          }
          if (WITH_BIAS) { t0 = t0 * ts + bct[NH * 2 + ni][h8 * 2]; t1 = t1 * ts + bct[NH * 2 + ni][h8 * 2 + 1]; }
          const bf16x8 v = {f2bf(t0[0]), f2bf(t0[1]), f2bf(t0[2]), f2bf(t0[3]), f2bf(t1[0]), f2bf(t1[1]), f2bf(t1[2]), f2bf(t1[3])};
          const int chunk = (ni * 32 + hh * 16 + h8 * 8) >> 3;
          *reinterpret_cast<bf16x8*>(sl + li * 128 + ((chunk ^ (li & 7)) << 4)) = v;
        }
      } else {
#pragma unroll
        for (int rg = 0; rg < 4; ++rg) {
          f32x4 t0;
#pragma unroll
          for (int j = 0; j < 4; ++j) asm volatile("v_accvgpr_read_b32 %0, %1" : "=v"(t0[j]) : "a"(a[rg * 4 + j]));
          const bf16x4 v = {f2bf(t0[0]), f2bf(t0[1]), f2bf(t0[2]), f2bf(t0[3])};
          const int col = ni * 32 + rg * 8 + hh * 4;
          *reinterpret_cast<bf16x4*>(sl + li * 128 + (((col >> 3) ^ (li & 7)) << 4) + (col & 7) * 2) = v;
        }
      }
#pragma unroll
      for (int r = 0; r < 16; ++r) a[r] = 0.f;
      __builtin_amdgcn_sched_barrier(0);
    }
  };
  const int rows_left = p.M - m0;
  const uint64_t wbytes = rows_left > 0 ? (uint64_t)rows_left * p.ldc * 2 : 0;
  const __amdgpu_buffer_rsrc_t rsC = ia_rsrc(reinterpret_cast<bf16*>(p.C) + (size_t)m0 * p.ldc, (uint32_t)(wbytes < 0x7FFFFFF0ull ? wbytes : 0x7FFFFFF0ull));
  const int ncol = n0 + c8 * 8;
  const uint32_t voffC = ncol < p.N ? (uint32_t)((rrow * p.ldc + ncol) * 2) : 0x80000000u;
  stage(0);
#pragma unroll
  for (int mi = 0; mi < 4; ++mi) {
    __builtin_amdgcn_wave_barrier();
    const char* const sl = stg + (mi & 1) * 4096;
    u32x4 v[4];
#pragma unroll
    for (int it = 0; it < 4; ++it) {
      const int row = it * 8 + rrow;
      v[it] = *reinterpret_cast<const u32x4*>(sl + row * 128 + ((c8 ^ (row & 7)) << 4));
    }
    __builtin_amdgcn_wave_barrier();
    if (mi < 3) stage(mi + 1);
#pragma unroll
    for (int it = 0; it < 4; ++it) {
      const uint32_t off = voffC + (uint32_t)((mi * 32 + it * 8) * p.ldc * 2);
      if (!IA_GEMM_DBG_HOOKS || !(p.dbg & 64)) __builtin_amdgcn_raw_buffer_store_b128(v[it], rsC, (int)off, 0, 0);
      else asm volatile("" : : "v"(v[it]));
    }
  }
}

template <int EPI, bool OUTF32, bool BKS, int NH>
IA_DEV void drain_half(const GemmArgs& p, f32x16 (&acc)[4][4], int m0, int n0, char* stg, int lane_e, bool full, bool bias_ready, f32x4 bias_lo,
                       f32x4 bias_hi) {
  const int hh = lane_e >> 5, li = lane_e & 31;
  const int rrow = lane_e >> 3, c8 = lane_e & 7;
  constexpr bool HAS_BIAS = EPI == EPI_BIAS || EPI == EPI_BIAS_GELU || EPI == EPI_BIAS_GELU_ACT || EPI == EPI_BIAS_ADD;
  constexpr bool HAS_AUX = EPI == EPI_ADD || EPI == EPI_BIAS_ADD || EPI == EPI_DGELU || EPI == EPI_DGELU_CS;
  constexpr int AHEAD = 4;
  auto drain = [&](auto PREFETCHED) {
    constexpr bool PRE = decltype(PREFETCHED)::value;
    f32x4 pb0, pb1;
    float cs[8];
    if (EPI == EPI_DGELU_CS) {
#pragma unroll
      for (int j = 0; j < 8; ++j) asm volatile("v_mov_b32 %0, 0" : "=v"(cs[j]));
    }
    bf16x8 ax[AHEAD + 1];
    constexpr bool BUF = PRE && !OUTF32;
    const auto window = [&](const void* base, int ld) {
      const uint64_t bytes = (uint64_t)(p.M - m0) * ld * 2;
      return ia_rsrc(reinterpret_cast<const bf16*>(base) + (size_t)m0 * ld, (uint32_t)(bytes < 0x7FFFFFF0ull ? bytes : 0x7FFFFFF0ull));
    };
    BufIO io{ia_rsrc(nullptr, 0), ia_rsrc(nullptr, 0), 0u};
    __amdgpu_buffer_rsrc_t rsAux = ia_rsrc(nullptr, 0);
    uint32_t voffC = 0, voffAux = 0;
    if (BUF) {
      io.rsC = window(p.C, p.ldc);
      if (EPI == EPI_BIAS_GELU) io.rsC2 = window(p.C2, p.ldc);
      voffC = (uint32_t)((rrow * p.ldc + n0 + c8 * 8) * 2);
      if (HAS_AUX) { rsAux = window(p.aux, p.ldaux); voffAux = (uint32_t)((rrow * p.ldaux + n0 + c8 * 8) * 2); }
    }
    auto aux_of = [&](int c) {
      const int row_in = (c >> 2) * 32 + ((c >> 1) & 1) * 16 + (c & 1) * 8;
      if (BUF) return __builtin_bit_cast(bf16x8, __builtin_amdgcn_raw_buffer_load_b128(rsAux, (int)(voffAux + (uint32_t)(row_in * p.ldaux * 2)), 0, 0));
      return *reinterpret_cast<const bf16x8*>(p.aux + (size_t)(m0 + row_in + rrow) * p.ldaux + n0 + c8 * 8);
    };
    if (PRE && HAS_BIAS) {
      if (bias_ready) { pb0 = bias_lo; pb1 = bias_hi; }
      else { pb0 = *reinterpret_cast<const f32x4*>(p.bias + n0 + c8 * 8); pb1 = *reinterpret_cast<const f32x4*>(p.bias + n0 + c8 * 8 + 4); }
    }
    if (PRE && HAS_AUX) {
#pragma unroll
      for (int c = 0; c < AHEAD; ++c) ax[c] = aux_of(c);
    }
    auto stage = [&](int mi) {
#pragma unroll
      for (int ni = 0; ni < 2; ++ni)
#pragma unroll
        for (int rg = 0; rg < 4; ++rg) {
          const int chunk = (ni * 32 + (BKS ? rg * 8 + hh * 4 : hh * 16 + rg * 4)) >> 2;
          f32x16& a = acc[mi][NH * 2 + ni];
          const f32x4 v = {a[rg * 4], a[rg * 4 + 1], a[rg * 4 + 2], a[rg * 4 + 3]};
          *reinterpret_cast<f32x4*>(stg + li * 256 + ((chunk ^ (li & 15)) << 4)) = v;
          a[rg * 4] = 0.f; a[rg * 4 + 1] = 0.f; a[rg * 4 + 2] = 0.f; a[rg * 4 + 3] = 0.f;
        }
    };
    stage(0);
#pragma unroll
    for (int mi = 0; mi < 4; ++mi) {
      __builtin_amdgcn_wave_barrier();
      f32x4 lo[4], hi[4];
#pragma unroll
      for (int it = 0; it < 4; ++it) {
        const int row = it * 8 + rrow;
        lo[it] = *reinterpret_cast<const f32x4*>(stg + row * 256 + (((2 * c8) ^ (row & 15)) << 4));
        hi[it] = *reinterpret_cast<const f32x4*>(stg + row * 256 + (((2 * c8 + 1) ^ (row & 15)) << 4));
      }
      asm volatile("s_waitcnt lgkmcnt(0)" : "+v"(lo[0]), "+v"(lo[1]), "+v"(lo[2]), "+v"(lo[3]), "+v"(hi[0]), "+v"(hi[1]), "+v"(hi[2]), "+v"(hi[3]));
      __builtin_amdgcn_wave_barrier();
      if (mi < 3) stage(mi + 1);
#pragma unroll
      for (int it = 0; it < 4; ++it) {
        const int row = it * 8 + rrow;
        const int m = m0 + mi * 32 + row, n = n0 + c8 * 8;
        const int c = mi * 4 + it;
        if (PRE) {
          if (HAS_AUX && c + AHEAD < 16) {
            ax[(c + AHEAD) % (AHEAD + 1)] = aux_of(c + AHEAD);
            asm volatile("" ::: "memory");
          }
          io.off = voffC + (uint32_t)((mi * 32 + it * 8) * p.ldc * 2);
          if (!(IA_DBG(p) & 64)) epi_store8<EPI, OUTF32, true, BUF>(p, m, n, lo[it], hi[it], pb0, pb1, ax[c % (AHEAD + 1)], cs, &io);
        } else {
          if (m < p.M && n < p.N && !(IA_DBG(p) & 64)) epi_store8<EPI, OUTF32, false>(p, m, n, lo[it], hi[it], pb0, pb1, ax[0], cs);
        }
        if (IA_DBG(p) & 64) asm volatile("" : : "v"(lo[it]), "v"(hi[it]));
      }
    }
    if (EPI == EPI_DGELU_CS) {
#pragma unroll
      for (int r = 0; r < 8; ++r) {
        float v = cs[r];
        v += __builtin_bit_cast(float, __builtin_amdgcn_update_dpp(__builtin_bit_cast(int, v), __builtin_bit_cast(int, v), 0x128, 0xF, 0xF, false));
        v = ia_add_xor32(ia_add_xor16(v));
        cs[r] = v;
      }
      if (rrow == 0 && n0 + c8 * 8 < p.N) {
        float* dst = p.csum_part + (size_t)(m0 >> 7) * p.N + n0 + c8 * 8;
        gstore16(dst, f32x4{cs[0], cs[1], cs[2], cs[3]});
        gstore16(dst + 4, f32x4{cs[4], cs[5], cs[6], cs[7]});
      }
    }
  };
  if (full && (HAS_BIAS || HAS_AUX) && !(IA_DBG(p) & 256)) drain(std::true_type{}); else drain(std::false_type{});
}

template <bool AKS, bool BKS, int EPI, bool OUTF32>
__global__ __launch_bounds__(256) void gemm_kernel(GemmArgs p) {
  extern __shared__ __attribute__((aligned(16))) char smem[];
  const int tid = threadIdx.x, lane0 = tid & 63;
  const int wave = __builtin_amdgcn_readfirstlane(tid >> 6);
  const int wm = wave >> 1, wn = wave & 1;
  const int nk_all = (p.K + BK - 1) / BK;
  const int total_tiles = p.tiles_m * p.tiles_n;
  int first_tile = blockIdx.x;
  bool ordered = false;
  p.split_id = 0;
  if (p.splits > 1) {
    const int w = xcd_chunk(blockIdx.x, gridDim.x);
    p.split_id = w / total_tiles;
    first_tile = w % total_tiles;
    ordered = true;
  }
  const int kt0 = p.split_id * p.nk_per_split;
  const int n_tiles = min(nk_all, kt0 + p.nk_per_split) - kt0;
  constexpr int PEND = 2 * (16 * epi_stores_per_call<EPI, OUTF32>() + epi_extra_stores<EPI>());
  auto coords = [&](int tile, int& bm, int& bn) {
    if (ordered) tile_of_order(p, tile, bm, bn); else tile_of_index(p, tile, total_tiles, bm, bn);
  };
  auto run = [&](int tile, bool prologue_only, f32x16 (&acc)[4][4], bool stores_in_flight) {
    int bm, bn;
    coords(tile, bm, bn);
    int lane = lane0;
    asm volatile("" : "+v"(lane));
    const uint64_t oa = (uint64_t)(AKS ? kt0 * BK : bm * BM) * p.lda, ob = (uint64_t)(BKS ? kt0 * BK : bn * BN) * p.ldb;
    constexpr bool PEEL_OK = !(EPI == EPI_BIAS && !OUTF32 && !BKS);
    main_loop<AKS, BKS, PEND, PEEL_OK>(p, smem, acc, rsrc_at(p.A, p.a_bytes, oa), rsrc_at(p.B, p.b_bytes, ob), AKS ? bm * BM : 0, BKS ? bn * BN : 0, kt0,
                              AKS ? 0 : kt0, BKS ? 0 : kt0, n_tiles, nk_all, wm, wn, wave, lane, prologue_only, stores_in_flight);
  };

  const bool dyn = p.tile_ctr != nullptr && !ordered;
  const int xcd = blockIdx.x & 7, q8 = total_tiles >> 3, r8 = total_tiles & 7;
  auto run_start = [&](int x) { return x < r8 ? x * (q8 + 1) : r8 * (q8 + 1) + (x - r8) * q8; };
  auto run_len = [&](int x) { return q8 + (x < r8 ? 1 : 0); };
  int* const mailbox = reinterpret_cast<int*>(smem + 2 * 2 * TILE_BYTES);
  uint32_t claimed = 0;
  auto claim_issue = [&]() {
    if (wave == 0 && lane0 == 0)
      {
        const uint64_t a64 = (uint64_t)(p.tile_ctr + xcd);
        const uint32_t alo = __builtin_amdgcn_readfirstlane((uint32_t)a64), ahi = __builtin_amdgcn_readfirstlane((uint32_t)(a64 >> 32));
        const uint64_t addr = ((uint64_t)ahi << 32) | alo;
        asm volatile("s_nop 4\n\tglobal_atomic_add %0, %1, %2, %3 sc0" : "=v"(claimed) : "v"(0u), "v"(1u), "s"(addr) : "memory");
      }
  };
  auto claim_resolve = [&]() -> int {
    asm volatile("s_waitcnt vmcnt(0)" : "+v"(claimed));
    if (wave == 0) {
      int pos = (int)__builtin_amdgcn_readfirstlane(claimed), w = -1;
      if (pos < run_len(xcd)) w = run_start(xcd) + pos;
      else {
        uint32_t seen = 0xFFFFFFFFu;
        if (lane0 < 8) seen = __hip_atomic_load(p.tile_ctr + lane0, __ATOMIC_RELAXED, __HIP_MEMORY_SCOPE_AGENT);
        const uint32_t mask = (uint32_t)__ballot((int)seen >= q8 + (lane0 < r8 ? 1 : 0)) | (1u << xcd);
        for (int d = 1; d < 8 && w < 0; ++d) {
          const int x = (xcd + d) & 7;
          if ((mask >> x) & 1u) continue;
          uint32_t got = 0;
          if (lane0 == 0) got = __hip_atomic_fetch_add(p.tile_ctr + x, 1u, __ATOMIC_RELAXED, __HIP_MEMORY_SCOPE_AGENT);
          pos = (int)__builtin_amdgcn_readfirstlane(got);
          if (pos < run_len(x)) w = run_start(x) + pos;
        }
      }
      if (lane0 == 0) *reinterpret_cast<volatile int*>(mailbox) = w;
    }
    __syncthreads();
    const int w = __builtin_amdgcn_readfirstlane(*reinterpret_cast<volatile int*>(mailbox));
    __syncthreads();
    return w;
  };
  auto leave = [&]() {
    asm volatile("s_waitcnt vmcnt(0)" : "+v"(claimed) : : "memory");
    if (dyn && wave == 0 && lane0 == 0) {
      const uint32_t d = __hip_atomic_fetch_add(p.tile_ctr + 8, 1u, __ATOMIC_RELAXED, __HIP_MEMORY_SCOPE_AGENT);
      if (d == gridDim.x - 1) {
#pragma unroll
        for (int i = 0; i < 9; ++i) __hip_atomic_store(p.tile_ctr + i, 0u, __ATOMIC_RELAXED, __HIP_MEMORY_SCOPE_AGENT);
      }
    }
  };
  if (dyn) {
    ordered = true;
    claim_issue();
    first_tile = claim_resolve();
    if (first_tile < 0) { leave(); return; }
    claim_issue();
  }

  f32x16 acc[4][4];
#pragma unroll
  for (int i = 0; i < 4; ++i)
#pragma unroll
    for (int j = 0; j < 4; ++j)
#pragma unroll
      for (int r = 0; r < 16; ++r) acc[i][j][r] = 0.f;
  int tile = first_tile;
  run(tile, true, acc, false);
  bool stores_in_flight = false;
  constexpr bool HAS_BIAS_K = EPI == EPI_BIAS || EPI == EPI_BIAS_GELU || EPI == EPI_BIAS_GELU_ACT || EPI == EPI_BIAS_ADD;
  while (true) {
    int bm, bn;
    coords(tile, bm, bn);
    const int m0_pre = bm * BM + wm * 128, n0_pre = bn * BN + wn * 128;
    const bool full = m0_pre + 128 <= p.M && n0_pre + 128 <= p.N;
    constexpr bool BIAS_CT = EPI == EPI_BIAS && !OUTF32 && !BKS;
    f32x4 pbv[4] = {};
    f32x4 bct[4][4] = {};
    int lane_b = lane0;
    asm volatile("" : "+v"(lane_b));
    const bool bias_pre = HAS_BIAS_K && full;
    if (bias_pre && BIAS_CT) {
      const float* bp = p.bias + n0_pre + (lane_b >> 5) * 16;
#pragma unroll
      for (int ni = 0; ni < 4; ++ni)
#pragma unroll
        for (int q = 0; q < 4; ++q) bct[ni][q] = *reinterpret_cast<const f32x4*>(bp + ni * 32 + q * 4);
    } else if (bias_pre) {
      const float* bp = p.bias + n0_pre + (lane_b & 7) * 8;
      pbv[0] = *reinterpret_cast<const f32x4*>(bp); pbv[1] = *reinterpret_cast<const f32x4*>(bp + 4);
      pbv[2] = *reinterpret_cast<const f32x4*>(bp + 64); pbv[3] = *reinterpret_cast<const f32x4*>(bp + 68);
    }
    run(tile, false, acc, stores_in_flight);
    float ts = 1.f;
    if (bias_pre && BIAS_CT) {
#pragma unroll
      for (int ni = 0; ni < 4; ++ni)
        asm volatile("s_waitcnt vmcnt(0)" : "+v"(bct[ni][0]), "+v"(bct[ni][1]), "+v"(bct[ni][2]), "+v"(bct[ni][3]));
      if (n0_pre < p.qcols) {
        ts = p.qscale;
#pragma unroll
        for (int ni = 0; ni < 4; ++ni)
#pragma unroll
          for (int q = 0; q < 4; ++q) bct[ni][q] *= ts;
      }
    } else if (bias_pre) asm volatile("s_waitcnt vmcnt(0)" : "+v"(pbv[0]), "+v"(pbv[1]), "+v"(pbv[2]), "+v"(pbv[3]));
    int next = ordered ? total_tiles : tile + gridDim.x;
    if (dyn) {
      next = claim_resolve();
      claim_issue();
      if (next < 0) next = total_tiles;
    }
    if (next < total_tiles) run(next, true, acc, false);

    int lane_e = lane0;
    asm volatile("" : "+v"(lane_e));
    int m0 = m0_pre, n0 = n0_pre;
    asm volatile("" : "+s"(m0), "+s"(n0));
    char* stg = smem + 2 * 2 * TILE_BYTES + wave * 2 * STAGE_BYTES;
    if (!(IA_DBG(p) & 32)) {
      if constexpr (EPI == EPI_NONE && !OUTF32) {
        drain_half_plain<BKS, 0, false>(p, acc, m0, n0, stg, lane_e, bct);
        drain_half_plain<BKS, 1, false>(p, acc, m0, n0 + 64, stg, lane_e, bct);
      } else if (BIAS_CT && bias_pre) {
        drain_half_plain<false, 0, BIAS_CT>(p, acc, m0, n0, stg, lane_e, bct, ts);
        drain_half_plain<false, 1, BIAS_CT>(p, acc, m0, n0 + 64, stg, lane_e, bct, ts);
      } else {
        drain_half<EPI, OUTF32, BKS, 0>(p, acc, m0, n0, stg, lane_e, full || (m0 + 128 <= p.M && n0 + 64 <= p.N), bias_pre, pbv[0], pbv[1]);
        drain_half<EPI, OUTF32, BKS, 1>(p, acc, m0, n0 + 64, stg, lane_e, full, bias_pre, pbv[2], pbv[3]);
      }
    }
    if (next >= total_tiles) break;
    stores_in_flight = !(IA_DBG(p) & 96) && full;
    if (!stores_in_flight) asm volatile("s_waitcnt vmcnt(0)" ::: "memory");
    tile = next;
  }
  leave();
}
}



namespace t256la {
using namespace t256w;

__global__ __launch_bounds__(256) void gemm_kernel(GemmArgs p) {
  extern __shared__ __attribute__((aligned(16))) char smem[];
  const int tid = threadIdx.x, lane0 = tid & 63;
  const int wave = __builtin_amdgcn_readfirstlane(tid >> 6);
  const int wm = wave >> 1, wn = wave & 1;
  const int nk_all = (p.K + BK - 1) / BK;
  const int total_tiles = p.tiles_m * p.tiles_n;
  const int n_tiles = nk_all;
  auto coords = [&](int tile, int& bm, int& bn) { tile_of_index(p, tile, total_tiles, bm, bn); };
  auto window_a = [&](int tile) {
    int bm = 0, bn = 0;
    if (tile < total_tiles) coords(tile, bm, bn);
    return tile < total_tiles ? rsrc_at(p.A, p.a_bytes, (uint64_t)bm * BM * p.lda) : ia_rsrc(p.A, 0u);
  };
  auto window_b = [&](int tile) {
    int bm = 0, bn = 0;
    if (tile < total_tiles) coords(tile, bm, bn);
    return tile < total_tiles ? rsrc_at(p.B, p.b_bytes, (uint64_t)bn * BN * p.ldb) : ia_rsrc(p.B, 0u);
  };

  int lane = lane0;
  asm volatile("" : "+v"(lane));
  const int li = lane & 31;
  const int gt = wave * 64 + lane;
  const int rowd = gt >> 3;
  const uint32_t voffA = (uint32_t)((rowd * p.lda + (((gt & 7) ^ ((rowd >> 1) & 7)) * 8)) * 2), stepA = (uint32_t)(32 * p.lda * 2);
  const uint32_t voffB = (uint32_t)((rowd * p.ldb + (((gt & 7) ^ ((rowd >> 1) & 7)) * 8)) * 2), stepB = (uint32_t)(32 * p.ldb * 2);
  const int kl = ((gt & 7) ^ (((gt >> 3) >> 1) & 7)) * 8;
  char* const my_part = smem + wave * 1024;
  const int nperm = ((li >> 2) & 1) * 16 + (li >> 3) * 4 + (li & 3);
  uint32_t baseA[4], baseB[4];
  const uint32_t smem_addr = ia_lds_addr(smem);
  frag_bases<false>(baseA, smem_addr, wm * 128, lane, li);
  frag_bases<false>(baseB, smem_addr + TILE_BYTES, wn * 128, lane, nperm);

  int tile = blockIdx.x;
  __amdgpu_buffer_rsrc_t rsA = window_a(tile), rsB = window_b(tile);
  __amdgpu_buffer_rsrc_t rsAn = window_a(tile + (int)gridDim.x), rsBn = window_b(tile + (int)gridDim.x);

  auto off_of = [&](int v) -> uint32_t {
    const int kt = v >= n_tiles ? v - n_tiles : v;
    return kl < p.K - kt * BK ? 1u : 0u;
  };
  auto dma = [&](int v, int i, uint32_t ok, uint32_t buf) {
    const bool isB = i >= 8, nx = v >= n_tiles;
    const int j = i & 7, kt = nx ? v - n_tiles : v;
    char* dst = my_part + (isB ? TILE_BYTES : 0) + buf + j * 4096;
    const uint32_t soff = (uint32_t)kt * (uint32_t)(BK * 2) + (uint32_t)j * (isB ? stepB : stepA);
    const uint32_t off = ok ? (isB ? voffB : voffA) : OOB;
    __builtin_amdgcn_raw_ptr_buffer_load_lds(isB ? (nx ? rsBn : rsB) : (nx ? rsAn : rsA), IA_LDS(dst), 16, off, (int)soff, 0, 0);
  };

#pragma unroll
  for (int i = 0; i < 16; ++i) dma(0, i, off_of(0), 0u);
#pragma unroll
  for (int i = 0; i < 16; ++i) dma(1, i, off_of(1), (uint32_t)(2 * TILE_BYTES));
  asm volatile("s_waitcnt vmcnt(0)" ::: "memory");
  __builtin_amdgcn_s_barrier();
  Op<false> a0, a1, a2, a3, b0, b1, b2, b3;
#pragma unroll
  for (int j = 0; j < 4; ++j) read_frag<0>(a0, j, baseA, 0u);
#pragma unroll
  for (int j = 0; j < 4; ++j) read_frag<0>(b0, j, baseB, 0u);
  uint32_t bo = 0;

  f32x16 acc[4][4];
#pragma unroll
  for (int i = 0; i < 4; ++i)
#pragma unroll
    for (int j = 0; j < 4; ++j)
#pragma unroll
      for (int r = 0; r < 16; ++r) acc[i][j][r] = 0.f;

  using Acc = std::false_type;

  const f32x4 no_bias[4][4] = {};
  while (true) {
    int bm, bn;
    coords(tile, bm, bn);
    const int m0_pre = bm * BM + wm * 128, n0_pre = bn * BN + wn * 128;
    int u = 0;
    uint32_t okA = 0u, okB = off_of(1);
    auto trip = [&](auto FIRST_T) {
      constexpr bool FIRST = decltype(FIRST_T)::value;
      const uint32_t bn_ = bo ^ (uint32_t)(2 * TILE_BYTES);
      tie2<0>(a0, b0);
      mfma_step<FIRST>(acc, a0, b0, [&](int i) {
        if (i < 4) { read_frag<1>(a1, i, baseA, bo); read_frag<1>(b1, i, baseB, bo); }
        else if (i < 8) { read_frag<2>(a2, i - 4, baseA, bo); read_frag<2>(b2, i - 4, baseB, bo); }
        else if (i < 12) { read_frag<3>(a3, i - 8, baseA, bo); read_frag<3>(b3, i - 8, baseB, bo); }
        if (!FIRST && i % 4 == 3) dma(u + 1, 12 + i / 4, okB, bn_);
        if (i == 12) okA = off_of(u + 2);
      });
      tie6<0>(a1, b1, a2, b2, a3, b3);
      __builtin_amdgcn_sched_barrier(0);
      __builtin_amdgcn_s_barrier();
      __builtin_amdgcn_sched_barrier(0);
      mfma_step<false>(acc, a1, b1, [&](int i) {
        if (i % 4 == 1) dma(u + 2, i / 4, okA, bo);
      });
      mfma_step<false>(acc, a2, b2, [&](int i) {
        if (i % 4 == 1) dma(u + 2, 4 + i / 4, okA, bo);
        if (i == 14) okB = off_of(u + 2);
      });
      if constexpr (FIRST) asm volatile("s_waitcnt vmcnt(40)" ::: "memory");
      else asm volatile("s_waitcnt vmcnt(8)" ::: "memory");
      __builtin_amdgcn_sched_barrier(0);
      __builtin_amdgcn_s_barrier();
      __builtin_amdgcn_sched_barrier(0);
      mfma_step<false>(acc, a3, b3, [&](int i) {
        if (i < 4) read_frag<0>(a0, i, baseA, bn_);
        else if (i < 8) read_frag<0>(b0, i - 4, baseB, bn_);
        if (i % 4 == 3) dma(u + 2, 8 + i / 4, okB, bo);
      });
      bo = bn_;
      ++u;
    };
    trip(std::true_type{});
    do { trip(Acc{}); } while (u < n_tiles);
    {
      const uint32_t ok1 = off_of(n_tiles + 1), b1_ = bo ^ (uint32_t)(2 * TILE_BYTES);
#pragma unroll
      for (int i = 12; i < 16; ++i) dma(n_tiles + 1, i, ok1, b1_);
    }

    int lane_e = lane0;
    asm volatile("" : "+v"(lane_e));
    int m0 = m0_pre, n0 = n0_pre;
    asm volatile("" : "+s"(m0), "+s"(n0));
    char* stg = smem + 2 * 2 * TILE_BYTES + wave * 2 * STAGE_BYTES;
    drain_half_plain<false, 0, false>(p, acc, m0, n0, stg, lane_e, no_bias);
    drain_half_plain<false, 1, false>(p, acc, m0, n0 + 64, stg, lane_e, no_bias);
    tile += (int)gridDim.x;
    if (tile >= total_tiles) break;
    rsA = rsAn; rsB = rsBn;
    rsAn = window_a(tile + (int)gridDim.x); rsBn = window_b(tile + (int)gridDim.x);
  }
  tie2<0>(a0, b0);
  asm volatile("s_waitcnt vmcnt(0)" ::: "memory");
}
}

struct GemmProf {
  bool on = false;
  int variant = -1, n = 0, cap = 0;
  double flops = 0.0, bytes = 0.0;
  hipEvent_t* ev = nullptr;
};
GemmProf g_prof;

IA_DEV void fold_row_sums(const float* rsum_ws, float* rsum_out, int M, int splits) {
  __shared__ float rs[256];
  if (!rsum_ws || (int)blockIdx.x * 32 >= M) return;
  const int lane = threadIdx.x & 7, m = blockIdx.x * 32 + (threadIdx.x >> 3);
  float a = 0.f;
  if (m < M)
    for (int sp = lane; sp < splits; sp += 8) a += rsum_ws[((size_t)blockIdx.y * splits + sp) * M + m];
  rs[threadIdx.x] = a;
  __syncthreads();
  if (lane == 0 && m < M) {
    float sum = rs[threadIdx.x];
#pragma unroll
    for (int l = 1; l < 8; ++l) sum += rs[threadIdx.x + l];
    rsum_out[(size_t)blockIdx.y * M + m] += sum;
  }
  __syncthreads();
}

__global__ __launch_bounds__(256) void splitk_reduce_kernel(const float* __restrict__ ws, float* __restrict__ C, int M, int N, int ldc,
                                                            int splits, int accumulate, long gc, const float* rsum_ws, float* rsum_out) {
  fold_row_sums(rsum_ws, rsum_out, M, splits);
  ws += (size_t)blockIdx.y * splits * M * N;
  C += (size_t)blockIdx.y * gc;
  const size_t total4 = (size_t)M * N / 4;
  for (size_t t = (size_t)blockIdx.x * 256 + threadIdx.x; t < total4; t += (size_t)gridDim.x * 256) {
    const size_t e = t * 4;
    const int m = (int)(e / N), n = (int)(e % N);
    f32x4 acc = *reinterpret_cast<const f32x4*>(ws + e);
    for (int s = 1; s < splits; ++s) acc += *reinterpret_cast<const f32x4*>(ws + (size_t)s * M * N + e);
    float* c = C + (size_t)m * ldc + n;
    if (accumulate) acc += *reinterpret_cast<const f32x4*>(c);
    *reinterpret_cast<f32x4*>(c) = acc;
  }
}

__global__ __launch_bounds__(256) void splitk_reduce_deep_kernel(const float* __restrict__ ws, float* __restrict__ C, int M, int N, int ldc,
                                                                 int splits, int accumulate, long gc, const float* rsum_ws, float* rsum_out) {
  __shared__ f32x4 red[256];
  fold_row_sums(rsum_ws, rsum_out, M, splits);
  ws += (size_t)blockIdx.y * splits * M * N;
  C += (size_t)blockIdx.y * gc;
  const size_t total4 = (size_t)M * N / 4;
  const int lane = threadIdx.x & 7;
  const size_t t = (size_t)blockIdx.x * 32 + (threadIdx.x >> 3);
  f32x4 acc = {0.f, 0.f, 0.f, 0.f};
  if (t < total4)
    for (int sp = lane; sp < splits; sp += 8) acc += *reinterpret_cast<const f32x4*>(ws + (size_t)sp * M * N + t * 4);
  red[threadIdx.x] = acc;
  __syncthreads();
  if (lane == 0 && t < total4) {
    f32x4 sum = red[threadIdx.x];
#pragma unroll
    for (int l = 1; l < 8; ++l) sum += red[threadIdx.x + l];
    const size_t e = t * 4;
    float* c = C + (size_t)(e / N) * ldc + (e % N);
    if (accumulate) sum += *reinterpret_cast<const f32x4*>(c);
    *reinterpret_cast<f32x4*>(c) = sum;
  }
}

struct Plan { bool big; int splits; };

Plan make_plan(int M, int N, int K, bool f32_out, int groups = 1) {
  Plan pl;
  const int nk = (K + BK - 1) / BK;
  const long t256n = (long)((M + 255) / 256) * ((N + 255) / 256);
  const int smax = f32_out ? (nk / 8 > 32 ? 32 : (nk / 8 < 1 ? 1 : nk / 8)) : 1;
  pl.big = M >= 256 && N >= 256 && (N & 7) == 0 && t256n * smax >= 160;
  if (groups > 1) pl.big = false;
  const long tiles = pl.big ? t256n : (long)((M + 127) / 128) * ((N + 127) / 128) * groups;
  const long slots = pl.big ? 256 : 512;
  int smax2 = smax;
  if (f32_out && slots / tiles > smax2) { smax2 = (int)(slots / tiles); if (smax2 > nk / 8) smax2 = nk / 8 < 1 ? 1 : nk / 8; if (smax2 < smax) smax2 = smax; }
  const double reduce_per_split = (double)tiles * (pl.big ? 0.0244 : 0.0061);
  int best = 1;
  double best_cost = 1e30;
  for (int s = 1; s <= smax2; ++s) {
    const long rounds = (tiles * s + slots - 1) / slots;
    const double cost = (double)rounds * ((nk + s - 1) / s + 6) + (s > 1 ? s * reduce_per_split : 0.0);
    if (cost < best_cost - 1e-9) { best_cost = cost; best = s; }
  }
  pl.splits = best;
  return pl;
}

int g_dynamic = -1;
constexpr int MAX_DEVICES = 16;
uint32_t* g_ctr_base[MAX_DEVICES] = {};
std::atomic<unsigned> g_launch_seq{0};
uint32_t* next_ctr_slot() {
  if (g_dynamic < 0) {
    const char* e = getenv("IA_GEMM_DYNAMIC");
    g_dynamic = e ? atoi(e) : 0;
  }
  if (!g_dynamic) return nullptr;
  int dev = 0;
  if (hipGetDevice(&dev) != hipSuccess || dev < 0 || dev >= MAX_DEVICES) return nullptr;
  uint32_t* base = __atomic_load_n(&g_ctr_base[dev], __ATOMIC_ACQUIRE);
  if (!base) {
    if (hipGetSymbolAddress((void**)&base, HIP_SYMBOL(g_tile_ctr)) != hipSuccess || !base) return nullptr;
    __atomic_store_n(&g_ctr_base[dev], base, __ATOMIC_RELEASE);
  }
  return base + (size_t)(g_launch_seq.fetch_add(1u, std::memory_order_relaxed) % CTR_SLOTS) * CTR_WORDS;
}

template <bool AKS, bool BKS, int EPI, bool OUTF32>
int launch(GemmArgs a, bool big, hipStream_t st) {
  constexpr int vid = AKS * 1000 + BKS * 100 + EPI * 10 + (OUTF32 ? 1 : 0);
  const bool rec = g_prof.on && g_prof.variant == vid && g_prof.n < g_prof.cap;
  if (rec) (void)hipEventRecord(g_prof.ev[2 * g_prof.n], st);
  if (big) {
    a.tiles_m = (a.M + t256w::BM - 1) / t256w::BM; a.tiles_n = (a.N + t256w::BN - 1) / t256w::BN;
    const int ntile = a.tiles_m * a.tiles_n;
    const int gx = a.splits > 1 ? ntile * a.splits : (ntile < 256 ? ntile : 256);
    a.tile_ctr = (a.splits == 1 && ntile > gx) ? next_ctr_slot() : nullptr;
    void (*kern)(GemmArgs) = t256w::gemm_kernel<AKS, BKS, EPI, OUTF32>;
    static bool attr_set[2] = {false, false};
    int la = 0;
    if constexpr (!AKS && !BKS && EPI == EPI_NONE && !OUTF32) {
      const char* e = getenv("IA_GEMM_LA");
      if ((e ? atoi(e) : 1) && a.splits == 1 && ntile > gx && !a.tile_ctr && a.K >= 2 * BK && !(IA_DBG(a))) { kern = t256la::gemm_kernel; la = 1; }
    }
    if (!attr_set[la]) {
      if (hipFuncSetAttribute((const void*)kern, hipFuncAttributeMaxDynamicSharedMemorySize, t256w::LDS_BYTES) != hipSuccess) return IA_ERR_LAUNCH;
      attr_set[la] = true;
    }
    hipLaunchKernelGGL(kern, dim3(gx), dim3(256), t256w::LDS_BYTES, st, a);
  } else {
    a.tiles_m = (a.M + t128::BM - 1) / t128::BM; a.tiles_n = (a.N + t128::BN - 1) / t128::BN;
    hipLaunchKernelGGL((t128::gemm_kernel<AKS, BKS, EPI, OUTF32>), dim3(a.tiles_m * a.tiles_n * a.splits * a.groups), dim3(256), 0, st, a);
  }
  if (OUTF32 && a.splits > 16) {
    size_t g = ((size_t)a.M * a.N / 4 + 31) / 32;
    if (a.rsum_out && g < (size_t)(a.M + 31) / 32) g = (size_t)(a.M + 31) / 32;
    hipLaunchKernelGGL(splitk_reduce_deep_kernel, dim3((unsigned)g, a.groups), dim3(256), 0, st, a.ws, (float*)a.C, a.M, a.N, a.ldc, a.splits,
                       a.accumulate, a.gc, a.rsum_out ? a.rsum_ws : nullptr, a.rsum_out);
  } else if (OUTF32 && a.splits > 1) {
    size_t g = ((size_t)a.M * a.N / 4 + 255) / 256; if (g > 4096) g = 4096;
    if (a.rsum_out && g < (size_t)(a.M + 31) / 32) g = (size_t)(a.M + 31) / 32;
    hipLaunchKernelGGL(splitk_reduce_kernel, dim3((int)g, a.groups), dim3(256), 0, st, a.ws, (float*)a.C, a.M, a.N, a.ldc, a.splits, a.accumulate,
                       a.gc, a.rsum_out ? a.rsum_ws : nullptr, a.rsum_out);
  }
  if (rec) {
    (void)hipEventRecord(g_prof.ev[2 * g_prof.n + 1], st);
    g_prof.flops += 2.0 * a.M * a.N * a.K;
    g_prof.bytes += 2.0 * ((double)a.M * a.K + (double)a.N * a.K) + (OUTF32 ? 4.0 : 2.0) * a.M * a.N;
    ++g_prof.n;
  }
  return ia_check_launch();
}

}

extern "C" size_t ia_gemm_workspace_bytes(int M, int N, int K, int c_is_f32) {
  if (!c_is_f32 || M <= 0 || N <= 0 || K <= 0) return 0;
  const Plan pl = make_plan(M, N, K, true);
  return pl.splits > 1 ? (size_t)pl.splits * M * (N + 1) * sizeof(float) : 0;
}

static int gemm_core(const void* A, int a_kstrided, int lda, const void* B, int b_kstrided, int ldb, void* C, int c_is_f32, int ldc, int M,
                     int N, int K, int epilogue, const float* bias, const void* aux, int ldaux, void* C2, int accumulate, void* workspace,
                     size_t workspace_bytes, const IaViewGemm* view, hipStream_t stream, int qcols = 0, float qscale = 1.f);

extern "C" size_t ia_gemm_colsum_workspace_bytes(int M, int N) {
  if (M <= 0 || N <= 0) return 0;
  const size_t fused = (size_t)((M + 255) / 256) * 2 * N * sizeof(float), plain = ia_colsum_workspace_bytes(M, N);
  return fused > plain ? fused : plain;
}

extern "C" int ia_gemm_bf16(const void* A, int a_kstrided, int lda, const void* B, int b_kstrided, int ldb,
                            void* C, int c_is_f32, int ldc, int M, int N, int K, int epilogue,
                            const float* bias, const void* aux, int ldaux, void* C2, int accumulate, void* workspace,
                            size_t workspace_bytes, hipStream_t stream) {
  return gemm_core(A, a_kstrided, lda, B, b_kstrided, ldb, C, c_is_f32, ldc, M, N, K, epilogue, bias, aux, ldaux, C2, accumulate, workspace,
                   workspace_bytes, nullptr, stream);
}

extern "C" int ia_gemm_bf16_qscale(const void* A, int lda, const void* B, int ldb, void* C, int ldc, int M, int N, int K, const float* bias,
                                   int scaled_cols, float col_scale, hipStream_t stream) {
  return gemm_core(A, 0, lda, B, 0, ldb, C, 0, ldc, M, N, K, EPI_BIAS, bias, nullptr, 0, nullptr, 0, nullptr, 0, nullptr, stream, scaled_cols,
                   col_scale);
}

int ia_gemm_view(const IaViewGemm& v, hipStream_t stream) {
  if ((v.a_view && (v.a_kstrided || (v.a_view != 1 && v.a_view != -1))) || (v.b_view && (!v.b_kstrided || v.b_view < 1 || v.b_view > 2)) ||
      v.pw <= 2 || (!v.a_view && !v.b_view) || v.groups < 1 || v.lca < 3 || v.lcbk < 3 || v.lcbn < 3)
    return IA_ERR_ARG;
  return gemm_core(v.A, v.a_kstrided, v.lda, v.B, v.b_kstrided, v.ldb, v.C, v.c_is_f32, v.ldc, v.M, v.N, v.K, v.bias ? EPI_BIAS : EPI_NONE,
                   v.bias, nullptr, 0, v.rsum_out, 0, v.workspace, v.workspace_bytes, &v, stream);
}

size_t ia_gemm_view_workspace_bytes(int M, int N, int K, int groups) {
  if (M <= 0 || N <= 0 || K <= 0 || groups <= 0) return 0;
  const Plan pl = make_plan(M, N, K, true, groups);
  return pl.splits > 1 ? (size_t)groups * pl.splits * M * (N + 1) * sizeof(float) : 0;
}

template <bool BKS>
static int launch_dgelu_colsum(GemmArgs& g, bool big, float* csum, void* workspace, size_t workspace_bytes, hipStream_t stream) {
  if (!csum || !workspace || workspace_bytes < ia_gemm_colsum_workspace_bytes(g.M, g.N) || g.ldc != g.N) return IA_ERR_WORKSPACE;
  if (!big) {
    int rc = launch<false, BKS, EPI_DGELU, false>(g, false, stream);
    return rc ? rc : ia_colsum(g.C, g.ldc, g.M, g.N, csum, 1, workspace, workspace_bytes, stream);
  }
  g.csum_part = (float*)workspace;
  int rc = launch<false, BKS, EPI_DGELU_CS, false>(g, true, stream);
  return rc ? rc : ia_sum_rows_f32((const float*)workspace, ((g.M + 255) / 256) * 2, g.N, csum, 1, stream);
}

static int gemm_core(const void* A, int a_kstrided, int lda, const void* B, int b_kstrided, int ldb, void* C, int c_is_f32, int ldc, int M,
                     int N, int K, int epilogue, const float* bias, const void* aux, int ldaux, void* C2, int accumulate, void* workspace,
                     size_t workspace_bytes, const IaViewGemm* view, hipStream_t stream, int qcols, float qscale) {
  const uint64_t a_window = view ? view->a_window : 0, b_window = view ? view->b_window : 0;
  const int groups = view ? view->groups : 1;
  (void)hipGetLastError();
  if (!A || !B || !C || M <= 0 || N <= 0 || K <= 0) return IA_ERR_ARG;
  if ((lda & 7) || (ldb & 7) || (ldc & 3) || (N & 3)) return IA_ERR_ARG;
  if (((uintptr_t)A & 15) || ((uintptr_t)B & 15) || ((uintptr_t)C & 15)) return IA_ERR_ARG;
  GemmArgs g;
  g.A = (const bf16*)A; g.B = (const bf16*)B; g.C = C; g.C2 = (bf16*)C2; g.bias = bias; g.aux = (const bf16*)aux;
  g.M = M; g.N = N; g.K = K; g.lda = lda; g.ldb = ldb; g.ldc = ldc; g.ldaux = ldaux; g.accumulate = accumulate;
  if (qcols < 0 || qcols > N || (qcols & 127) || (qcols && (epilogue != EPI_BIAS || c_is_f32 || a_kstrided || b_kstrided))) return IA_ERR_ARG;
  g.qcols = qcols; g.qscale = qscale;
  const uint64_t ab = a_window ? a_window : (a_kstrided ? ((uint64_t)(K - 1) * lda + M) * 2 : ((uint64_t)(M - 1) * lda + K) * 2);
  const uint64_t bb = b_window ? b_window : (b_kstrided ? ((uint64_t)(K - 1) * ldb + N) * 2 : ((uint64_t)(N - 1) * ldb + K) * 2);
  g.csum_part = nullptr; g.split_id = 0; g.tile_ctr = nullptr;
  g.a_view = g.b_view = g.pw = 0; g.lca = g.lcbk = g.lcbn = 6;
  g.groups = 1; g.ga = g.gb = g.gc = g.gbias = 0;
  if (view) {
    g.a_view = view->a_view; g.b_view = view->b_view; g.pw = view->pw; g.lca = view->lca; g.lcbk = view->lcbk; g.lcbn = view->lcbn;
    g.groups = groups; g.ga = view->ga; g.gb = view->gb; g.gc = view->gc; g.gbias = view->gbias;
  }
  if (!a_kstrided && (K & 7)) return IA_ERR_ARG;
  g.a_bytes = ab; g.b_bytes = bb;
  g.tiles_m = g.tiles_n = 0;
  { static int dbg = -1; if (dbg < 0) { const char* e = getenv("IA_GEMM_DBG"); dbg = e ? atoi(e) : 0; } g.dbg = dbg; }
  const int nk = (K + BK - 1) / BK;
  Plan pl = make_plan(M, N, K, c_is_f32 != 0, groups);
  g.splits = 1; g.nk_per_split = nk; g.ws = nullptr;
  const bool big = pl.big && !view && !(g.dbg & 128);
  const bool wgrad_form = a_kstrided && b_kstrided && c_is_f32 && epilogue == EPI_NONE;
  g.rsum_out = (wgrad_form && !big) ? (float*)C2 : nullptr;
  g.rsum_ws = nullptr;
  if (c_is_f32 && epilogue == EPI_NONE && pl.splits > 1 && workspace &&
      workspace_bytes >= (size_t)groups * pl.splits * M * (N + (g.rsum_out ? 1 : 0)) * sizeof(float)) {
    g.nk_per_split = (nk + pl.splits - 1) / pl.splits;
    g.splits = (nk + g.nk_per_split - 1) / g.nk_per_split;
    g.ws = (float*)workspace;
    g.rsum_ws = g.ws + (size_t)groups * g.splits * M * N;
  }
  {
    const uint64_t margin = view ? 2 * (uint64_t)(view->pw + 1) : 0, slab = (uint64_t)g.nk_per_split * BK + margin, tile = 256 + margin;
    const uint64_t wa = (a_kstrided ? slab : tile) * (uint64_t)lda * 2 + (a_kstrided ? 0 : (uint64_t)K * 2);
    const uint64_t wb = (b_kstrided ? slab : tile) * (uint64_t)ldb * 2 + (b_kstrided ? 0 : (uint64_t)K * 2);
    if (wa >= 0x7FFFFFF0ull || wb >= 0x7FFFFFF0ull) return IA_ERR_ARG;
  }
  const bool needs_bias = epilogue == EPI_BIAS || epilogue == EPI_BIAS_GELU || epilogue == EPI_BIAS_GELU_ACT || epilogue == EPI_BIAS_ADD;
  const bool needs_aux = epilogue == EPI_ADD || epilogue == EPI_DGELU || epilogue == EPI_BIAS_ADD || epilogue == EPI_DGELU_CS;
  if (needs_bias && !bias) return IA_ERR_ARG;
  if (needs_aux && (!aux || (ldaux & 3))) return IA_ERR_ARG;
  if (epilogue == EPI_BIAS_GELU && !C2) return IA_ERR_ARG;

  if (!a_kstrided && !b_kstrided && !c_is_f32) {
    switch (epilogue) {
      case EPI_NONE: return launch<false, false, EPI_NONE, false>(g, big, stream);
      case EPI_BIAS: return launch<false, false, EPI_BIAS, false>(g, big, stream);
      case EPI_BIAS_GELU: return launch<false, false, EPI_BIAS_GELU, false>(g, big, stream);
      case EPI_BIAS_GELU_ACT: return launch<false, false, EPI_BIAS_GELU_ACT, false>(g, big, stream);
      case EPI_BIAS_ADD: return launch<false, false, EPI_BIAS_ADD, false>(g, big, stream);
      case EPI_ADD: return launch<false, false, EPI_ADD, false>(g, big, stream);
      case EPI_DGELU: return launch<false, false, EPI_DGELU, false>(g, big, stream);
      case EPI_DGELU_CS: return launch_dgelu_colsum<false>(g, big, (float*)C2, workspace, workspace_bytes, stream);
    }
  } else if (!a_kstrided && b_kstrided && !c_is_f32) {
    switch (epilogue) {
      case EPI_NONE: return launch<false, true, EPI_NONE, false>(g, big, stream);
      case EPI_ADD: return launch<false, true, EPI_ADD, false>(g, big, stream);
      case EPI_DGELU: return launch<false, true, EPI_DGELU, false>(g, big, stream);
      case EPI_DGELU_CS: return launch_dgelu_colsum<true>(g, big, (float*)C2, workspace, workspace_bytes, stream);
    }
  } else if (a_kstrided && b_kstrided && c_is_f32) {
    if (epilogue == EPI_NONE) {
      int rc = launch<true, true, EPI_NONE, true>(g, big, stream);
      if (!rc && C2 && big) rc = ia_colsum(A, lda, K, M, (float*)C2, 1, workspace, workspace_bytes, stream);
      return rc;
    }
  } else if (!a_kstrided && !b_kstrided && c_is_f32) {
    if (epilogue == EPI_NONE) return launch<false, false, EPI_NONE, true>(g, big, stream);
    if (epilogue == EPI_BIAS) return launch<false, false, EPI_BIAS, true>(g, big, stream);
  }
  return IA_ERR_UNSUPPORTED;
}

extern "C" int ia_prof_begin(int variant, int max_launches) {
  (void)hipGetLastError();
  if (max_launches <= 0) return IA_ERR_ARG;
  if (g_prof.cap < max_launches) {
    for (int i = 0; i < 2 * g_prof.cap; ++i) (void)hipEventDestroy(g_prof.ev[i]);
    delete[] g_prof.ev;
    g_prof.ev = new hipEvent_t[2 * max_launches];
    for (int i = 0; i < 2 * max_launches; ++i)
      if (hipEventCreate(&g_prof.ev[i]) != hipSuccess) return IA_ERR_LAUNCH;
    g_prof.cap = max_launches;
  }
  g_prof.variant = variant; g_prof.n = 0; g_prof.flops = 0.0; g_prof.bytes = 0.0; g_prof.on = true;
  return IA_OK;
}

extern "C" int ia_prof_end(double* total_ms, double* total_flops, int* launches) {
  (void)hipGetLastError();
  g_prof.on = false;
  double ms = 0.0;
  for (int i = 0; i < g_prof.n; ++i) {
    if (hipEventSynchronize(g_prof.ev[2 * i + 1]) != hipSuccess) return IA_ERR_LAUNCH;
    float t = 0.f;
    if (hipEventElapsedTime(&t, g_prof.ev[2 * i], g_prof.ev[2 * i + 1]) != hipSuccess) return IA_ERR_LAUNCH;
    ms += t;
  }
  if (total_ms) *total_ms = ms;
  if (total_flops) *total_flops = g_prof.flops;
  if (launches) *launches = g_prof.n;
  return IA_OK;
}

namespace {
__global__ __launch_bounds__(256) void cu_hog_kernel(unsigned long long ticks) {
  extern __shared__ __attribute__((aligned(16))) char hog_smem[];
  if (threadIdx.x == 0) *reinterpret_cast<volatile int*>(hog_smem) = 1;
  const unsigned long long t0 = wall_clock64();
  while (wall_clock64() - t0 < ticks) __builtin_amdgcn_s_sleep(32);
}
}
extern "C" int ia_debug_gemm_dynamic(int on) {
  if (g_dynamic < 0) (void)next_ctr_slot();
  const int prev = g_dynamic;
  if (on >= 0) g_dynamic = on ? 1 : 0;
  return prev;
}
extern "C" int ia_debug_cu_hog(int workgroups, float milliseconds, hipStream_t stream) {
  (void)hipGetLastError();
  if (workgroups <= 0 || workgroups > 256 || !(milliseconds > 0.f) || milliseconds > 1000.f) return IA_ERR_ARG;
  static bool attr_set = false;
  if (!attr_set) {
    if (hipFuncSetAttribute((const void*)cu_hog_kernel, hipFuncAttributeMaxDynamicSharedMemorySize, t256w::LDS_BYTES) != hipSuccess) return IA_ERR_LAUNCH;
    attr_set = true;
  }
  hipLaunchKernelGGL(cu_hog_kernel, dim3(workgroups), dim3(256), t256w::LDS_BYTES, stream, (unsigned long long)(milliseconds * 1e5f));
  return ia_check_launch();
}

extern "C" double ia_prof_bytes(void) { return g_prof.bytes; }
```

item_alignment_amd/ops.py:

```python
import torch

from . import _lib
from ._lib import check, ptr, stream_ptr

EPI_NONE, EPI_BIAS, EPI_BIAS_GELU, EPI_ADD, EPI_DGELU, EPI_BIAS_ADD, EPI_DGELU_COLSUM = 0, 1, 2, 3, 4, 5, 6
ACT_NONE, ACT_TANH = 0, 1
BF16, F32 = torch.bfloat16, torch.float32


def _need(t, dtype, name):
    if t is None:
        return
    if not t.is_cuda:
        raise _lib.ItemAlignError(f"{name} must live on the GPU (the HIP path has no CPU fallback)")
    if t.dtype != dtype:
        raise TypeError(f"{name}: expected {dtype}, got {t.dtype}")
    if not t.is_contiguous():
        raise ValueError(f"{name} must be contiguous")


def gemm(a, b, *, a_kstrided=False, b_kstrided=False, epilogue=EPI_NONE, bias=None, aux=None, out=None, out_f32=False,
         accumulate=False, pre_out=None, colsum_out=None):
    lib = _lib.load()
    _need(a, BF16, "a"); _need(b, BF16, "b"); _need(bias, F32, "bias"); _need(aux, BF16, "aux")
    if a_kstrided:
        K, M = a.shape
    else:
        M, K = a.shape
    if b_kstrided:
        Kb, N = b.shape
    else:
        N, Kb = b.shape
    if K != Kb:
        raise ValueError(f"gemm: inner dims differ ({K} vs {Kb})")
    if out is None:
        out = torch.empty((M, N), device=a.device, dtype=F32 if out_f32 else BF16)
    _need(out, F32 if out_f32 else BF16, "out")
    if epilogue == EPI_BIAS_GELU and pre_out is None:
        pre_out = torch.empty((M, N), device=a.device, dtype=BF16)
    ws_bytes = lib.ia_gemm_workspace_bytes(M, N, K, int(out_f32))
    if epilogue == EPI_DGELU_COLSUM:
        _need(colsum_out, F32, "colsum_out")
        if colsum_out is None:
            raise ValueError("gemm: EPI_DGELU_COLSUM needs colsum_out")
        pre_out = colsum_out
        ws_bytes = max(ws_bytes, lib.ia_gemm_colsum_workspace_bytes(M, N))
    ws = torch.empty(ws_bytes, device=a.device, dtype=torch.uint8) if ws_bytes else None
    check(lib.ia_gemm_bf16(a.data_ptr(), int(a_kstrided), a.shape[1], b.data_ptr(), int(b_kstrided), b.shape[1], out.data_ptr(),
                           int(out_f32), N, M, N, K, epilogue, ptr(bias), ptr(aux), N if aux is not None else 0, ptr(pre_out),
                           int(accumulate), ptr(ws), ws_bytes, stream_ptr()), "ia_gemm_bf16")
    if epilogue == EPI_BIAS_GELU:
        return out, pre_out
    return out


def ln_fwd(x, gamma, beta, eps, *, bias=None, residual=None, write_z=True, drop_p=0.0, seed=0, stream_id=0):
    lib = _lib.load()
    _need(x, BF16, "x"); _need(gamma, F32, "gamma"); _need(beta, F32, "beta"); _need(bias, F32, "bias"); _need(residual, BF16, "residual")
    M, H = x.shape
    y = torch.empty_like(x)
    z = torch.empty_like(x) if write_z else None
    mean = torch.empty(M, device=x.device, dtype=F32)
    rstd = torch.empty(M, device=x.device, dtype=F32)
    check(lib.ia_ln_fwd(x.data_ptr(), ptr(bias), ptr(residual), ptr(z), y.data_ptr(), mean.data_ptr(), rstd.data_ptr(),
                        gamma.data_ptr(), ptr(beta), M, H, eps, drop_p, seed, stream_id, stream_ptr()), "ia_ln_fwd")
    return y, z, mean, rstd


def ln_bwd(dy, z, mean, rstd, gamma, *, dres=None, dgamma=None, dbeta=None, dbias=None, drop_p=0.0, seed=0, stream_id=0):
    lib = _lib.load()
    _need(dy, BF16, "dy"); _need(z, BF16, "z"); _need(dres, BF16, "dres")
    M, H = dy.shape
    dz = torch.empty_like(dy)
    dx = torch.empty_like(dy) if drop_p > 0 else None
    ws_bytes = lib.ia_ln_bwd_workspace_bytes(M, H)
    ws = torch.empty(ws_bytes, device=dy.device, dtype=torch.uint8)
    check(lib.ia_ln_bwd(dy.data_ptr(), ptr(dres), z.data_ptr(), mean.data_ptr(), rstd.data_ptr(), gamma.data_ptr(), dz.data_ptr(),
                        ptr(dx), ptr(dgamma), ptr(dbeta), ptr(dbias), M, H, drop_p, seed, stream_id, ws.data_ptr(), ws_bytes, 1,
                        stream_ptr()), "ia_ln_bwd")
    return dz, dx


def colsum(x, out, accumulate=True):
    lib = _lib.load()
    _need(x, BF16, "x"); _need(out, F32, "out")
    M, N = x.shape
    ws_bytes = lib.ia_colsum_workspace_bytes(M, N)
    ws = torch.empty(ws_bytes, device=x.device, dtype=torch.uint8)
    check(lib.ia_colsum(x.data_ptr(), N, M, N, out.data_ptr(), int(accumulate), ws.data_ptr(), ws_bytes, stream_ptr()), "ia_colsum")
    return out


def gemm_qscale(a, b, bias, scaled_cols, col_scale):
    lib = _lib.load()
    _need(a, BF16, "a"); _need(b, BF16, "b"); _need(bias, F32, "bias")
    M, K = a.shape
    N = b.shape[0]
    out = torch.empty((M, N), device=a.device, dtype=BF16)
    check(lib.ia_gemm_bf16_qscale(a.data_ptr(), K, b.data_ptr(), K, out.data_ptr(), N, M, N, K, bias.data_ptr(), scaled_cols, col_scale,
                                  stream_ptr()), "ia_gemm_bf16_qscale")
    return out


def attn_fwd(qkv, B, L, nh, *, key_mask=None, scale=0.125, drop_p=0.0, seed=0, q_prescaled=False):
    lib = _lib.load()
    _need(qkv, BF16, "qkv"); _need(key_mask, torch.uint8, "key_mask")
    H = nh * 64
    out = torch.empty((B * L, H), device=qkv.device, dtype=BF16)
    lse = torch.empty((B, nh, L), device=qkv.device, dtype=F32)
    base = qkv.data_ptr()
    fn = lib.ia_attn_fwd_ps if q_prescaled else lib.ia_attn_fwd
    check(fn(base, base + 2 * H, base + 4 * H, 3 * H, ptr(key_mask), out.data_ptr(), H, lse.data_ptr(), B, nh, L, scale, drop_p, seed,
             stream_ptr()), "ia_attn_fwd")
    return out, lse


def attn_bwd(qkv, ctx, d_ctx, lse, B, L, nh, *, key_mask=None, scale=0.125, drop_p=0.0, seed=0, dbias=None, q_prescaled=False, return_delta=False,
             masked_rows_dead=False):
    lib = _lib.load()
    _need(qkv, BF16, "qkv"); _need(ctx, BF16, "ctx"); _need(d_ctx, BF16, "d_ctx"); _need(lse, F32, "lse")
    H = nh * 64
    dqkv = torch.empty_like(qkv)
    delta = torch.empty((B, nh, L), device=qkv.device, dtype=F32)
    base, dbase = qkv.data_ptr(), dqkv.data_ptr()
    if (q_prescaled or masked_rows_dead) and dbias is None:
        dbias = torch.zeros(3 * H, device=qkv.device, dtype=F32)
    if masked_rows_dead:
        ws = torch.empty(lib.ia_attn_bwd_bias_workspace_bytes(B, nh, L), device=qkv.device, dtype=torch.uint8)
        check(lib.ia_attn_bwd_bias_ex((1 if q_prescaled else 0) | 2, base, base + 2 * H, base + 4 * H, 3 * H, ptr(key_mask), ctx.data_ptr(),
                                      d_ctx.data_ptr(), H, lse.data_ptr(), delta.data_ptr(), dbase, dbase + 2 * H, dbase + 4 * H, 3 * H,
                                      dbias.data_ptr(), ws.data_ptr(), ws.numel(), B, nh, L, scale, drop_p, seed, stream_ptr()), "ia_attn_bwd_bias_ex")
        return (dqkv, delta) if return_delta else dqkv
    if dbias is not None:
        _need(dbias, F32, "dbias")
        ws = torch.empty(lib.ia_attn_bwd_bias_workspace_bytes(B, nh, L), device=qkv.device, dtype=torch.uint8)
        fn = lib.ia_attn_bwd_bias_ps if q_prescaled else lib.ia_attn_bwd_bias
        check(fn(base, base + 2 * H, base + 4 * H, 3 * H, ptr(key_mask), ctx.data_ptr(), d_ctx.data_ptr(), H, lse.data_ptr(),
                                   delta.data_ptr(), dbase, dbase + 2 * H, dbase + 4 * H, 3 * H, dbias.data_ptr(), ws.data_ptr(), ws.numel(),
                                   B, nh, L, scale, drop_p, seed, stream_ptr()), "ia_attn_bwd_bias")
        return (dqkv, delta) if return_delta else dqkv
    check(lib.ia_attn_bwd(base, base + 2 * H, base + 4 * H, 3 * H, ptr(key_mask), ctx.data_ptr(), d_ctx.data_ptr(), H, lse.data_ptr(),
                          delta.data_ptr(), dbase, dbase + 2 * H, dbase + 4 * H, 3 * H, B, nh, L, scale, drop_p, seed, stream_ptr()),
          "ia_attn_bwd")
    return (dqkv, delta) if return_delta else dqkv


def cast_to_bf16(src, dst=None):
    lib = _lib.load()
    _need(src, F32, "src")
    if dst is None:
        dst = torch.empty(src.shape, device=src.device, dtype=BF16)
    check(lib.ia_cast_f32_to_bf16(src.data_ptr(), dst.data_ptr(), src.numel(), stream_ptr()), "ia_cast_f32_to_bf16")
    return dst


def cast_to_f32(src, dst=None):
    lib = _lib.load()
    _need(src, BF16, "src")
    if dst is None:
        dst = torch.empty(src.shape, device=src.device, dtype=F32)
    check(lib.ia_cast_bf16_to_f32(src.data_ptr(), dst.data_ptr(), src.numel(), stream_ptr()), "ia_cast_bf16_to_f32")
    return dst


def textcnn_taps(sizes, num_filters):
    nt = num_filters * sum(sizes)
    return nt, (nt + 7) & ~7


def _ptr_array(tensors):
    return (_lib.vp * len(tensors))(*(None if t is None else t.data_ptr() for t in tensors))


def _int_array(values):
    return (_lib.i32 * len(values))(*values)


def textcnn_pack_taps(weights, sizes, taps=None):
    lib = _lib.load()
    for w in weights:
        _need(w, F32, "conv weight")
    F_, H = weights[0].shape[0], weights[0].shape[3]
    if taps is None:
        taps = torch.empty((2, textcnn_taps(sizes, F_)[1], H), device=weights[0].device, dtype=BF16)
    _need(taps, BF16, "taps")
    check(lib.ia_textcnn_pack_taps(_ptr_array(weights), _int_array(sizes), len(sizes), F_, H, taps.data_ptr(), stream_ptr()),
          "ia_textcnn_pack_taps")
    return taps


def textcnn_pool_fwd(P, biases, sizes, B, L, *, p1=0.0, p2=0.0, seed=0, stream_id1=0, stream_id2=0):
    lib = _lib.load()
    _need(P, F32, "P")
    for b in biases:
        _need(b, F32, "conv bias")
    F_ = biases[0].shape[0]
    feat = torch.empty((B, F_ * len(sizes)), device=P.device, dtype=F32)
    arg = torch.empty((B, F_ * len(sizes)), device=P.device, dtype=torch.int32)
    check(lib.ia_textcnn_pool_fwd(P.data_ptr(), P.shape[1], _ptr_array(biases), _int_array(sizes), len(sizes), F_, B, L, p1, p2, seed,
                                  stream_id1, stream_id2, feat.data_ptr(), arg.data_ptr(), stream_ptr()), "ia_textcnn_pool_fwd")
    return feat, arg


def textcnn_pool_bwd_w(g, arg, x0, x1, sizes, num_filters, L, *, p1=0.0, p2=0.0, seed=0, stream_id1=0, stream_id2=0):
    lib = _lib.load()
    _need(g, F32, "g"); _need(arg, torch.int32, "argmax"); _need(x0, BF16, "x0"); _need(x1, BF16, "x1")
    B, H = g.shape[0], x0.shape[1]
    dW = [torch.empty((num_filters, 2, K, H), device=g.device, dtype=F32) for K in sizes]
    db = [torch.empty(num_filters, device=g.device, dtype=F32) for _ in sizes]
    check(lib.ia_textcnn_pool_bwd_w(g.data_ptr(), arg.data_ptr(), x0.data_ptr(), x1.data_ptr(), _int_array(sizes), len(sizes), num_filters,
                                    B, L, H, p1, p2, seed, stream_id1, stream_id2, _ptr_array(dW), _ptr_array(db), stream_ptr()),
          "ia_textcnn_pool_bwd_w")
    return dW, db


def textcnn_pool_bwd_x(g, arg, weights, sizes, L, *, p1=0.0, p2=0.0, seed=0, stream_id1=0, stream_id2=0):
    lib = _lib.load()
    _need(g, F32, "g"); _need(arg, torch.int32, "argmax")
    for w in weights:
        _need(w, F32, "conv weight")
    B, F_, H = g.shape[0], weights[0].shape[0], weights[0].shape[3]
    dx = torch.empty((B * L, H), device=g.device, dtype=BF16)
    check(lib.ia_textcnn_pool_bwd_x(g.data_ptr(), arg.data_ptr(), _ptr_array(weights), _int_array(sizes), len(sizes), F_, B, L, H, p1, p2,
                                    seed, stream_id1, stream_id2, dx.data_ptr(), stream_ptr()), "ia_textcnn_pool_bwd_x")
    return dx
```

Measured before the change: 610.2.

## Skip fully-masked K-tiles in weight-gradient GEMMs using a live-row tile mask

Adds a per-K-tile liveness bitmask built from the padded-row key mask, and a variant of the 256x256 weight-gradient GEMM that visits only live K-tiles while walking buffer offsets by the gap between them. The post-LN layer backward routes its four weight-gradient GEMMs through this path when masked rows are known dead, so padding tokens no longer cost any MMA or load work. It adds one small mask kernel per layer and some wave-level bookkeeping in the main loop, and dead rows must contribute exactly zero for the result to stay correct.

```diff
diff --git a/include/itemalign.h b/include/itemalign.h
--- a/include/itemalign.h
+++ b/include/itemalign.h
@@ -16,7 +16,7 @@
 #define IA_ERR_UNSUPPORTED (-4)
 
 const char* ia_strerror(int code);
-#define IA_ABI_VERSION 15
+#define IA_ABI_VERSION 16
 int ia_abi_version(void);
 
 #define IA_EPI_NONE 0
@@ -34,6 +34,13 @@
                         int scaled_cols, float col_scale, ia_stream_t stream);
 size_t ia_gemm_workspace_bytes(int M, int N, int K, int c_is_f32);
 size_t ia_gemm_colsum_workspace_bytes(int M, int N);
+size_t ia_gemm_wgrad_rows_workspace_bytes(int N_out, int N_in, int M_rows);
+int ia_gemm_wgrad_rows_filters(int N_out, int N_in, int M_rows);
+int ia_gemm_wgrad_rows(const void* dY, int ldy, const void* X, int ldx, float* dW, int ldw, int N_out, int N_in, int M_rows,
+                       const uint8_t* row_live, int accumulate, void* workspace, size_t workspace_bytes, ia_stream_t stream);
+size_t ia_ktile_mask_bytes(int M_rows);
+int ia_ktile_mask(const uint8_t* row_live, int M_rows, uint32_t* mask, ia_stream_t stream);
+int ia_ktile_mask_host(const uint8_t* row_live, int M_rows, uint32_t* mask);
 
 int ia_prof_begin(int variant, int max_launches);
 int ia_prof_end(double* total_ms, double* total_flops, int* launches);
diff --git a/item_alignment_amd/_lib.py b/item_alignment_amd/_lib.py
--- a/item_alignment_amd/_lib.py
+++ b/item_alignment_amd/_lib.py
@@ -30,6 +30,12 @@
     "ia_gemm_bf16": (i32, [vp, i32, i32, vp, i32, i32, vp, i32, i32, i32, i32, i32, i32, vp, vp, i32, vp, i32, vp, sz, vp]),
     "ia_gemm_workspace_bytes": (sz, [i32, i32, i32, i32]),
     "ia_gemm_colsum_workspace_bytes": (sz, [i32, i32]),
+    "ia_gemm_wgrad_rows_workspace_bytes": (sz, [i32, i32, i32]),
+    "ia_gemm_wgrad_rows_filters": (i32, [i32, i32, i32]),
+    "ia_gemm_wgrad_rows": (i32, [vp, i32, vp, i32, vp, i32, i32, i32, i32, vp, i32, vp, sz, vp]),
+    "ia_ktile_mask_bytes": (sz, [i32]),
+    "ia_ktile_mask": (i32, [vp, i32, vp, vp]),
+    "ia_ktile_mask_host": (i32, [vp, i32, vp]),
     "ia_prof_begin": (i32, [i32, i32]),
     "ia_prof_end": (i32, [C.POINTER(C.c_double), C.POINTER(C.c_double), C.POINTER(i32)]),
     "ia_prof_bytes": (C.c_double, []),
@@ -177,7 +183,7 @@
 _lib = None
 
 
-ABI_VERSION = 15
+ABI_VERSION = 16
 
 
 class ItemAlignError(RuntimeError):
diff --git a/item_alignment_amd/csrc/common.h b/item_alignment_amd/csrc/common.h
--- a/item_alignment_amd/csrc/common.h
+++ b/item_alignment_amd/csrc/common.h
@@ -158,3 +158,6 @@
 extern "C" int ia_colsum(const void* x, int ld, int M, int N, float* out, int accumulate, void* workspace, size_t workspace_bytes,
                          hipStream_t stream);
 __attribute__((visibility("hidden"))) size_t ia_gemm_view_workspace_bytes(int M, int N, int K, int groups);
+__attribute__((visibility("hidden"))) int ia_gemm_wgrad_masked(const void* dY, int ldy, const void* X, int ldx, float* dW, int ldw, int N_out,
+                                                               int N_in, int M_rows, const uint32_t* ktile_mask, int accumulate,
+                                                               void* workspace, size_t workspace_bytes, hipStream_t stream);
diff --git a/item_alignment_amd/csrc/engine.hip b/item_alignment_amd/csrc/engine.hip
--- a/item_alignment_amd/csrc/engine.hip
+++ b/item_alignment_amd/csrc/engine.hip
@@ -58,7 +58,7 @@
 }
 
 struct Scratch {
-  char* g0; char* g1; char* g2; char* gI; char* gqkv; float* delta; char* ws; size_t ws_bytes; char* gws; size_t gws_bytes; size_t bytes;
+  char* g0; char* g1; char* g2; char* gI; char* gqkv; float* delta; char* ws; size_t ws_bytes; char* gws; size_t gws_bytes; uint32_t* live_kt; size_t bytes;
 };
 
 size_t max3(size_t a, size_t b, size_t c) { return a > b ? (a > c ? a : c) : (b > c ? b : c); }
@@ -76,6 +76,7 @@
   s.gws_bytes = max3(ia_gemm_workspace_bytes((int)(3 * H), (int)H, (int)M, 1), ia_gemm_workspace_bytes((int)I, (int)H, (int)M, 1),
                      max3(ia_gemm_workspace_bytes((int)H, (int)I, (int)M, 1), ia_gemm_workspace_bytes((int)H, (int)H, (int)M, 1), 0));
   s.gws = a.take(s.gws_bytes);
+  s.live_kt = (uint32_t*)a.take(ia_ktile_mask_bytes((int)M));
   s.bytes = a.bytes;
   return s;
 }
@@ -92,6 +93,11 @@
   if (wt)
     return ia_gemm_bf16(dy, 0, k_out, wt, 0, k_out, dx, 0, n_in, M, n_in, k_out, epilogue, nullptr, aux, ldaux, c2, 0, ws, ws_bytes, st);
   return ia_gemm_bf16(dy, 0, k_out, w, 1, n_in, dx, 0, n_in, M, n_in, k_out, epilogue, nullptr, aux, ldaux, c2, 0, ws, ws_bytes, st);
+}
+
+int wgrad(const void* dy, int n_out, const void* x, int n_in, float* dw, int M, const uint32_t* live_kt, void* ws, size_t ws_bytes, ia_stream_t st) {
+  if (live_kt) return ia_gemm_wgrad_masked(dy, n_out, x, n_in, dw, n_in, n_out, n_in, M, live_kt, 1, ws, ws_bytes, st);
+  return ia_gemm_bf16(dy, 1, n_out, x, 1, n_in, dw, 1, n_in, n_out, n_in, M, IA_EPI_NONE, nullptr, nullptr, 0, nullptr, 1, ws, ws_bytes, st);
 }
 
 bool q_prescale(const ia_layer_cfg* c) { return (c->H & 127) == 0; }
@@ -217,21 +223,23 @@
   const bool drop = c->hidden_drop > 0.f;
   if (!c->pre_ln) {
     const uint8_t* const live = (c->masked_rows_dead && !c->cu_seqlens) ? key_mask : nullptr;
+    const uint32_t* const live_kt = live ? k.live_kt : nullptr;
+    if (live) IA_TRY(ia_ktile_mask(live, M, k.live_kt, st));
     IA_TRY(ia_ln_bwd2_rows(dy, dy2, nullptr, s.ffn, s.mean2, s.rstd2, w->ln2_g, k.g0, drop ? k.g1 : nullptr, g->ln2_g, g->ln2_b, g->b_fc2, M, H,
                            c->hidden_drop, c->seed, c->layer_id * 4u + 1u, live, k.ws, k.ws_bytes, 1, st));
     const char* d_ffn = drop ? k.g1 : k.g0;
-    IA_TRY(ia_gemm_bf16(d_ffn, 1, H, s.hact, 1, I, g->w_fc2, 1, I, H, I, M, IA_EPI_NONE, nullptr, nullptr, 0, nullptr, 1, k.gws, k.gws_bytes, st));
+    IA_TRY(wgrad(d_ffn, H, s.hact, I, (float*)g->w_fc2, M, live_kt, k.gws, k.gws_bytes, st));
     IA_TRY(dgrad(d_ffn, H, w->w_fc2, w->wt_fc2, I, k.gI, M, IA_EPI_DGELU_COLSUM, s.hpre, I, g->b_fc1, k.ws, k.ws_bytes, st));
-    IA_TRY(ia_gemm_bf16(k.gI, 1, I, s.ln, 1, H, g->w_fc1, 1, H, I, H, M, IA_EPI_NONE, nullptr, nullptr, 0, nullptr, 1, k.gws, k.gws_bytes, st));
+    IA_TRY(wgrad(k.gI, I, s.ln, H, (float*)g->w_fc1, M, live_kt, k.gws, k.gws_bytes, st));
     IA_TRY(dgrad(k.gI, I, w->w_fc1, w->wt_fc1, H, k.g2, M, IA_EPI_NONE, nullptr, 0, nullptr, nullptr, 0, st));
     char* dz1buf = dx2 ? (char*)dx2 : k.g0;
     IA_TRY(ia_ln_bwd2_rows(k.g2, k.g0, nullptr, s.proj, s.mean1, s.rstd1, w->ln1_g, dz1buf, drop ? k.g1 : nullptr, g->ln1_g, g->ln1_b, g->b_o, M, H,
                            c->hidden_drop, c->seed, c->layer_id * 4u + 0u, live, k.ws, k.ws_bytes, 1, st));
     const char* d_att = drop ? k.g1 : dz1buf;
-    IA_TRY(ia_gemm_bf16(d_att, 1, H, s.ctx, 1, H, g->w_o, 1, H, H, H, M, IA_EPI_NONE, nullptr, nullptr, 0, nullptr, 1, k.gws, k.gws_bytes, st));
+    IA_TRY(wgrad(d_att, H, s.ctx, H, (float*)g->w_o, M, live_kt, k.gws, k.gws_bytes, st));
     IA_TRY(dgrad(d_att, H, w->w_o, w->wt_o, H, k.g2, M, IA_EPI_NONE, nullptr, 0, nullptr, nullptr, 0, st));
     IA_TRY(attn_bwd(c, s.qkv, key_mask, s.ctx, k.g2, s.lse, k.delta, k.gqkv, g->b_qkv, k.ws, k.ws_bytes, scale, c->attn_drop, attn_seed, st));
-    IA_TRY(ia_gemm_bf16(k.gqkv, 1, 3 * H, x, 1, H, g->w_qkv, 1, H, 3 * H, H, M, IA_EPI_NONE, nullptr, nullptr, 0, nullptr, 1, k.gws, k.gws_bytes, st));
+    IA_TRY(wgrad(k.gqkv, 3 * H, x, H, (float*)g->w_qkv, M, live_kt, k.gws, k.gws_bytes, st));
     if (dx2)
       IA_TRY(dgrad(k.gqkv, 3 * H, w->w_qkv, w->wt_qkv, H, dx, M, IA_EPI_NONE, nullptr, 0, nullptr, nullptr, 0, st));
     else
diff --git a/item_alignment_amd/csrc/gemm.hip b/item_alignment_amd/csrc/gemm.hip
--- a/item_alignment_amd/csrc/gemm.hip
+++ b/item_alignment_amd/csrc/gemm.hip
@@ -14,9 +14,15 @@
 constexpr uint32_t OOB = 0xFFFFFFF0u;
 
 enum { EPI_NONE = 0, EPI_BIAS = 1, EPI_BIAS_GELU = 2, EPI_ADD = 3, EPI_DGELU = 4, EPI_BIAS_ADD = 5, EPI_DGELU_CS = 6, EPI_BIAS_GELU_ACT = 7 };
+constexpr int EPI_NONE_LIVE = 8;
 
 struct GemmArgs {
-  const bf16* A; const bf16* B; void* C; bf16* C2; const float* bias; const bf16* aux;
+  const bf16* A; const bf16* B; void* C; bf16* C2;
+  union {
+    const float* bias;
+    const uint32_t* live_kt;
+  };
+  const bf16* aux;
   int M, N, K;
   int lda, ldb, ldc, ldaux;
   uint64_t a_bytes, b_bytes;
@@ -461,6 +467,7 @@
 namespace t256w {
 constexpr int BM = 256, BN = 256, TILE_BYTES = 32768;
 constexpr int STAGE_BYTES = 16 * 64 * 4;
+constexpr int LIVE_MAX_KTILES = 64 * 32;
 constexpr int LDS_BYTES = 2 * 2 * TILE_BYTES + 8 * STAGE_BYTES;
 
 template <bool KS> struct Op;
@@ -557,10 +564,28 @@
     }
 }
 
-template <bool AKS, bool BKS, int PEND, bool PEEL_OK = true>
+struct LiveWalk {
+  uint64_t rest;
+  uint32_t w;
+  int wi, cur;
+};
+IA_DEV void live_start(LiveWalk& k, uint32_t mv) { k.rest = __ballot(mv != 0u); k.w = 0u; k.wi = 0; k.cur = -1; }
+IA_DEV int live_next(LiveWalk& k, uint32_t mv) {
+  const bool open = k.w == 0u, any = k.rest != 0ull;
+  const int wi = open ? (any ? __builtin_ctzll(k.rest) : 0) : k.wi;
+  const uint32_t fetched = __builtin_amdgcn_readlane(mv, wi);
+  const uint32_t w = open ? (any ? fetched : 0u) : k.w;
+  k.rest = open ? (k.rest & (k.rest - 1ull)) : k.rest;
+  const int idx = w != 0u ? wi * 32 + __builtin_ctz(w) : k.cur + 1;
+  k.w = w & (w - 1u); k.wi = wi; k.cur = idx;
+  return idx;
+}
+
+template <bool AKS, bool BKS, int PEND, bool PEEL_OK = true, bool LIVE = false>
 IA_DEV void main_loop(const GemmArgs& p, char* smem, f32x16 (&acc)[4][4], __amdgpu_buffer_rsrc_t rsA, __amdgpu_buffer_rsrc_t rsB, int xa, int xb,
                       int kt0, int ktaA0, int ktaB0, int n_tiles, int nk_all, int wm, int wn, int wave, int lane, bool prologue_only,
-                      bool stores_in_flight) {
+                      bool stores_in_flight, uint32_t live_mv = 0u) {
+  static_assert(!LIVE || (AKS && BKS), "the live-k-tile walk advances the running lane offsets of two k-strided operands");
   constexpr bool ROUND = !AKS && !BKS;
   const int li = lane & 31;
   const int gt = wave * 64 + lane;
@@ -575,16 +600,20 @@
   char* const my_part = smem + wave * 1024;
   const int dbg = IA_GEMM_DBG_HOOKS ? p.dbg : 0;
   const bool dma_on = !(dbg & 2);
+  [[maybe_unused]] LiveWalk lw;
+  int live0 = 0, live1 = 1;
+  if constexpr (LIVE) { live_start(lw, live_mv); live0 = live_next(lw, live_mv); live1 = live_next(lw, live_mv); }
 
   auto dma_piece = [&](int u, int i) {
     const bool isB = i >= 8;
     const int j = i & 7;
     char* dst = my_part + (isB ? TILE_BYTES : 0) + (u & 1) * 2 * TILE_BYTES + j * 4096;
-    const int kt = kt0 + u, kta = (dbg & 4) ? 0 : (isB ? ktaB0 : ktaA0) + u;
+    const int kt = kt0 + u;
+    const int kta = (dbg & 4) ? 0 : (isB ? ktaB0 : ktaA0) + (LIVE ? (u == 0 ? live0 : live1) : u);
     const bool ks = isB ? BKS : AKS;
     const uint32_t soff = (uint32_t)kta * (isB ? kstepB : kstepA) + (uint32_t)j * (isB ? stepB : stepA);
     if (ks) {
-      const uint32_t off = dma_on ? (isB ? voffB : voffA) + soff : OOB;
+      const uint32_t off = (dma_on && (!LIVE || u < n_tiles)) ? (isB ? voffB : voffA) + soff : OOB;
       __builtin_amdgcn_raw_ptr_buffer_load_lds(isB ? rsB : rsA, IA_LDS(dst), 16, off, 0, 0, 0);
     } else {
       const int lim = (u < n_tiles && dma_on) ? p.K - kt * BK : 0;
@@ -606,7 +635,9 @@
     __builtin_amdgcn_raw_ptr_buffer_load_lds(isB ? rsB : rsA, IA_LDS(dst), 16, off, (int)soff, 0, 0);
   };
 
-  uint32_t runA = voffA + (uint32_t)((dbg & 4) ? 0 : ktaA0 + 2) * kstepA, runB = voffB + (uint32_t)((dbg & 4) ? 0 : ktaB0 + 2) * kstepB;
+  int live2 = 2;
+  if constexpr (LIVE) { if (!prologue_only) live2 = live_next(lw, live_mv); }
+  uint32_t runA = voffA + (uint32_t)((dbg & 4) ? 0 : ktaA0 + live2) * kstepA, runB = voffB + (uint32_t)((dbg & 4) ? 0 : ktaB0 + live2) * kstepB;
   auto dma_run = [&](int u, int i) {
     const bool isB = i >= 8;
     if (!(isB ? BKS : AKS) || (dbg & 4)) { dma_piece(u, i); return; }
@@ -724,8 +755,15 @@
     });
     bo = bn;
     ++u;
-    if (AKS) { runA += kstepA; asm volatile("" : "+v"(runA)); }
-    if (BKS) { runB += kstepB; asm volatile("" : "+v"(runB)); }
+    if constexpr (LIVE) {
+      const int at = lw.cur;
+      const uint32_t hop = (uint32_t)(live_next(lw, live_mv) - at);
+      runA += hop * kstepA; asm volatile("" : "+v"(runA));
+      runB += hop * kstepB; asm volatile("" : "+v"(runB));
+    } else {
+      if (AKS) { runA += kstepA; asm volatile("" : "+v"(runA)); }
+      if (BKS) { runB += kstepB; asm volatile("" : "+v"(runB)); }
+    }
   } while (u < n_tiles);
   tie<0>(a0); tie<0>(b0);
 }
@@ -902,8 +940,11 @@
   if (full && (HAS_BIAS || HAS_AUX) && !(IA_DBG(p) & 256)) drain(std::true_type{}); else drain(std::false_type{});
 }
 
-template <bool AKS, bool BKS, int EPI, bool OUTF32>
+template <bool AKS, bool BKS, int EPI_, bool OUTF32>
 __global__ __launch_bounds__(256) void gemm_kernel(GemmArgs p) {
+  constexpr bool LIVE = EPI_ == EPI_NONE_LIVE;
+  constexpr int EPI = LIVE ? (int)EPI_NONE : EPI_;
+  static_assert(!LIVE || (AKS && BKS && OUTF32), "live k-tiles: the weight-gradient form only");
   extern __shared__ __attribute__((aligned(16))) char smem[];
   const int tid = threadIdx.x, lane0 = tid & 63;
   const int wave = __builtin_amdgcn_readfirstlane(tid >> 6);
@@ -920,7 +961,17 @@
     ordered = true;
   }
   const int kt0 = p.split_id * p.nk_per_split;
-  const int n_tiles = min(nk_all, kt0 + p.nk_per_split) - kt0;
+  int n_tiles = min(nk_all, kt0 + p.nk_per_split) - kt0;
+  uint32_t live_mv = 0u;
+  if constexpr (LIVE) {
+    const int nw = (nk_all + 31) >> 5, first = kt0 + 32 * lane0, wlo = first >> 5, sh = first & 31, left = n_tiles - 32 * lane0;
+    const uint32_t lo = wlo < nw ? p.live_kt[wlo] : 0u, hi = wlo + 1 < nw ? p.live_kt[wlo + 1] : 0u;
+    live_mv = sh ? (lo >> sh) | (hi << (32 - sh)) : lo;
+    live_mv = left >= 32 ? live_mv : (left > 0 ? live_mv & ((1u << left) - 1u) : 0u);
+    n_tiles = 0;
+    for (uint64_t rest = __ballot(live_mv != 0u); rest; rest &= rest - 1ull)
+      n_tiles += __builtin_popcount(__builtin_amdgcn_readlane(live_mv, __builtin_ctzll(rest)));
+  }
   constexpr int PEND = 2 * (16 * epi_stores_per_call<EPI, OUTF32>() + epi_extra_stores<EPI>());
   auto coords = [&](int tile, int& bm, int& bn) {
     if (ordered) tile_of_order(p, tile, bm, bn); else tile_of_index(p, tile, total_tiles, bm, bn);
@@ -932,8 +983,8 @@
     asm volatile("" : "+v"(lane));
     const uint64_t oa = (uint64_t)(AKS ? kt0 * BK : bm * BM) * p.lda, ob = (uint64_t)(BKS ? kt0 * BK : bn * BN) * p.ldb;
     constexpr bool PEEL_OK = !(EPI == EPI_BIAS && !OUTF32 && !BKS);
-    main_loop<AKS, BKS, PEND, PEEL_OK>(p, smem, acc, rsrc_at(p.A, p.a_bytes, oa), rsrc_at(p.B, p.b_bytes, ob), AKS ? bm * BM : 0, BKS ? bn * BN : 0, kt0,
-                              AKS ? 0 : kt0, BKS ? 0 : kt0, n_tiles, nk_all, wm, wn, wave, lane, prologue_only, stores_in_flight);
+    main_loop<AKS, BKS, PEND, PEEL_OK, LIVE>(p, smem, acc, rsrc_at(p.A, p.a_bytes, oa), rsrc_at(p.B, p.b_bytes, ob), AKS ? bm * BM : 0, BKS ? bn * BN : 0, kt0,
+                              AKS ? 0 : kt0, BKS ? 0 : kt0, n_tiles, nk_all, wm, wn, wave, lane, prologue_only, stores_in_flight, live_mv);
   };
 
   const bool dyn = p.tile_ctr != nullptr && !ordered;
@@ -1073,6 +1124,7 @@
   }
   leave();
 }
+
 }
 
 
@@ -1338,7 +1390,8 @@
 template <bool AKS, bool BKS, int EPI, bool OUTF32>
 int launch(GemmArgs a, bool big, hipStream_t st) {
   constexpr int vid = AKS * 1000 + BKS * 100 + EPI * 10 + (OUTF32 ? 1 : 0);
-  const bool rec = g_prof.on && g_prof.variant == vid && g_prof.n < g_prof.cap;
+  constexpr bool WGRAD = AKS && BKS && EPI == EPI_NONE && OUTF32;
+  const bool rec = g_prof.on && g_prof.variant == vid && g_prof.n < g_prof.cap && !(WGRAD && a.live_kt);
   if (rec) (void)hipEventRecord(g_prof.ev[2 * g_prof.n], st);
   if (big) {
     a.tiles_m = (a.M + t256w::BM - 1) / t256w::BM; a.tiles_n = (a.N + t256w::BN - 1) / t256w::BN;
@@ -1346,8 +1399,11 @@
     const int gx = a.splits > 1 ? ntile * a.splits : (ntile < 256 ? ntile : 256);
     a.tile_ctr = (a.splits == 1 && ntile > gx) ? next_ctr_slot() : nullptr;
     void (*kern)(GemmArgs) = t256w::gemm_kernel<AKS, BKS, EPI, OUTF32>;
-    static bool attr_set[2] = {false, false};
+    static bool attr_set[3] = {false, false, false};
     int la = 0;
+    if constexpr (WGRAD) {
+      if (a.live_kt) { kern = t256w::gemm_kernel<true, true, EPI_NONE_LIVE, true>; la = 2; }
+    }
     if constexpr (!AKS && !BKS && EPI == EPI_NONE && !OUTF32) {
       const char* e = getenv("IA_GEMM_LA");
       if ((e ? atoi(e) : 1) && a.splits == 1 && ntile > gx && !a.tile_ctr && a.K >= 2 * BK && !(IA_DBG(a))) { kern = t256la::gemm_kernel; la = 1; }
@@ -1391,7 +1447,8 @@
 
 static int gemm_core(const void* A, int a_kstrided, int lda, const void* B, int b_kstrided, int ldb, void* C, int c_is_f32, int ldc, int M,
                      int N, int K, int epilogue, const float* bias, const void* aux, int ldaux, void* C2, int accumulate, void* workspace,
-                     size_t workspace_bytes, const IaViewGemm* view, hipStream_t stream, int qcols = 0, float qscale = 1.f);
+                     size_t workspace_bytes, const IaViewGemm* view, hipStream_t stream, int qcols = 0, float qscale = 1.f,
+                     const uint32_t* live_kt = nullptr);
 
 extern "C" size_t ia_gemm_colsum_workspace_bytes(int M, int N) {
   if (M <= 0 || N <= 0) return 0;
@@ -1413,6 +1470,72 @@
                    col_scale);
 }
 
+static __host__ __device__ inline uint32_t ktile_live(const uint8_t* row_live, int M, int t) {
+  const uint8_t* r = row_live + (size_t)t * BK;
+  const int n = M - t * BK < BK ? M - t * BK : BK;
+  uint64_t any = 0;
+  if (n == BK && ((uintptr_t)r & 7) == 0) {
+    for (int i = 0; i < BK / 8; ++i) any |= reinterpret_cast<const uint64_t*>(r)[i];
+  } else {
+    for (int i = 0; i < n; ++i) any |= r[i];
+  }
+  return any != 0 ? 1u : 0u;
+}
+namespace {
+__global__ __launch_bounds__(256) void ktile_mask_kernel(const uint8_t* __restrict__ row_live, int M, int nk, uint32_t* __restrict__ mask) {
+  const int t = blockIdx.x * 256 + threadIdx.x;
+  const uint64_t b = __ballot(t < nk && ktile_live(row_live, M, t));
+  if ((threadIdx.x & 31) == 0 && t < nk) mask[t >> 5] = (uint32_t)(b >> (threadIdx.x & 32));
+}
+inline size_t al256(size_t b) { return (b + 255) & ~(size_t)255; }
+}
+
+extern "C" size_t ia_ktile_mask_bytes(int M_rows) {
+  if (M_rows <= 0) return 0;
+  return (size_t)(((M_rows + BK - 1) / BK + 31) / 32) * sizeof(uint32_t);
+}
+extern "C" int ia_ktile_mask(const uint8_t* row_live, int M_rows, uint32_t* mask, hipStream_t stream) {
+  (void)hipGetLastError();
+  if (!row_live || !mask || M_rows <= 0) return IA_ERR_ARG;
+  const int nk = (M_rows + BK - 1) / BK;
+  hipLaunchKernelGGL(ktile_mask_kernel, dim3((nk + 255) / 256), dim3(256), 0, stream, row_live, M_rows, nk, mask);
+  return ia_check_launch();
+}
+extern "C" int ia_ktile_mask_host(const uint8_t* row_live, int M_rows, uint32_t* mask) {
+  if (!row_live || !mask || M_rows <= 0) return IA_ERR_ARG;
+  const int nk = (M_rows + BK - 1) / BK;
+  for (int w = 0; w < (nk + 31) / 32; ++w) mask[w] = 0u;
+  for (int t = 0; t < nk; ++t) mask[t >> 5] |= ktile_live(row_live, M_rows, t) << (t & 31);
+  return IA_OK;
+}
+int ia_gemm_wgrad_masked(const void* dY, int ldy, const void* X, int ldx, float* dW, int ldw, int N_out, int N_in, int M_rows,
+                         const uint32_t* ktile_mask, int accumulate, void* workspace, size_t workspace_bytes, hipStream_t stream) {
+  return gemm_core(dY, 1, ldy, X, 1, ldx, dW, 1, ldw, N_out, N_in, M_rows, EPI_NONE, nullptr, nullptr, 0, nullptr, accumulate, workspace,
+                   workspace_bytes, nullptr, stream, 0, 1.f, ktile_mask);
+}
+extern "C" size_t ia_gemm_wgrad_rows_workspace_bytes(int N_out, int N_in, int M_rows) {
+  if (N_out <= 0 || N_in <= 0 || M_rows <= 0) return 0;
+  return al256(ia_gemm_workspace_bytes(N_out, N_in, M_rows, 1)) + ia_ktile_mask_bytes(M_rows);
+}
+extern "C" int ia_gemm_wgrad_rows_filters(int N_out, int N_in, int M_rows) {
+  if (N_out <= 0 || N_in <= 0 || M_rows <= 0) return 0;
+  const Plan pl = make_plan(N_out, N_in, M_rows, true);
+  const int nk = (M_rows + BK - 1) / BK;
+  return pl.big && (nk + pl.splits - 1) / pl.splits <= t256w::LIVE_MAX_KTILES ? 1 : 0;
+}
+extern "C" int ia_gemm_wgrad_rows(const void* dY, int ldy, const void* X, int ldx, float* dW, int ldw, int N_out, int N_in, int M_rows,
+                                  const uint8_t* row_live, int accumulate, void* workspace, size_t workspace_bytes, hipStream_t stream) {
+  if (!row_live)
+    return gemm_core(dY, 1, ldy, X, 1, ldx, dW, 1, ldw, N_out, N_in, M_rows, EPI_NONE, nullptr, nullptr, 0, nullptr, accumulate, workspace,
+                     workspace_bytes, nullptr, stream);
+  if (N_out <= 0 || N_in <= 0 || M_rows <= 0) return IA_ERR_ARG;
+  const size_t split_bytes = al256(ia_gemm_workspace_bytes(N_out, N_in, M_rows, 1));
+  if (!workspace || workspace_bytes < split_bytes + ia_ktile_mask_bytes(M_rows) || ((uintptr_t)workspace & 15)) return IA_ERR_WORKSPACE;
+  uint32_t* mask = reinterpret_cast<uint32_t*>((char*)workspace + split_bytes);
+  int rc = ia_ktile_mask(row_live, M_rows, mask, stream);
+  return rc ? rc : ia_gemm_wgrad_masked(dY, ldy, X, ldx, dW, ldw, N_out, N_in, M_rows, mask, accumulate, workspace, split_bytes, stream);
+}
+
 int ia_gemm_view(const IaViewGemm& v, hipStream_t stream) {
   if ((v.a_view && (v.a_kstrided || (v.a_view != 1 && v.a_view != -1))) || (v.b_view && (!v.b_kstrided || v.b_view < 1 || v.b_view > 2)) ||
       v.pw <= 2 || (!v.a_view && !v.b_view) || v.groups < 1 || v.lca < 3 || v.lcbk < 3 || v.lcbn < 3)
@@ -1441,7 +1564,7 @@
 
 static int gemm_core(const void* A, int a_kstrided, int lda, const void* B, int b_kstrided, int ldb, void* C, int c_is_f32, int ldc, int M,
                      int N, int K, int epilogue, const float* bias, const void* aux, int ldaux, void* C2, int accumulate, void* workspace,
-                     size_t workspace_bytes, const IaViewGemm* view, hipStream_t stream, int qcols, float qscale) {
+                     size_t workspace_bytes, const IaViewGemm* view, hipStream_t stream, int qcols, float qscale, const uint32_t* live_kt) {
   const uint64_t a_window = view ? view->a_window : 0, b_window = view ? view->b_window : 0;
   const int groups = view ? view->groups : 1;
   (void)hipGetLastError();
@@ -1486,6 +1609,7 @@
     const uint64_t wb = (b_kstrided ? slab : tile) * (uint64_t)ldb * 2 + (b_kstrided ? 0 : (uint64_t)K * 2);
     if (wa >= 0x7FFFFFF0ull || wb >= 0x7FFFFFF0ull) return IA_ERR_ARG;
   }
+  if (a_kstrided && b_kstrided && c_is_f32 && epilogue == EPI_NONE) g.live_kt = (big && g.nk_per_split <= t256w::LIVE_MAX_KTILES) ? live_kt : nullptr;
   const bool needs_bias = epilogue == EPI_BIAS || epilogue == EPI_BIAS_GELU || epilogue == EPI_BIAS_GELU_ACT || epilogue == EPI_BIAS_ADD;
   const bool needs_aux = epilogue == EPI_ADD || epilogue == EPI_DGELU || epilogue == EPI_BIAS_ADD || epilogue == EPI_DGELU_CS;
   if (needs_bias && !bias) return IA_ERR_ARG;
diff --git a/item_alignment_amd/ops.py b/item_alignment_amd/ops.py
--- a/item_alignment_amd/ops.py
+++ b/item_alignment_amd/ops.py
@@ -54,6 +54,31 @@
     return out
 
 
+def ktile_mask(row_live):
+    lib = _lib.load()
+    _need(row_live, torch.uint8, "row_live")
+    M = row_live.numel()
+    out = torch.empty(lib.ia_ktile_mask_bytes(M) // 4, device=row_live.device, dtype=torch.int32)
+    check(lib.ia_ktile_mask(row_live.data_ptr(), M, out.data_ptr(), stream_ptr()), "ia_ktile_mask")
+    return out
+
+
+def gemm_wgrad_rows(dy, x, row_live=None, *, out=None, accumulate=False):
+    lib = _lib.load()
+    _need(dy, BF16, "dy"); _need(x, BF16, "x"); _need(row_live, torch.uint8, "row_live")
+    (M, n_out), (Mx, n_in) = dy.shape, x.shape
+    if M != Mx or (row_live is not None and row_live.numel() != M):
+        raise ValueError("gemm_wgrad_rows: dy, x and row_live must have the same number of rows")
+    if out is None:
+        out = torch.empty((n_out, n_in), device=dy.device, dtype=F32)
+    _need(out, F32, "out")
+    ws_bytes = lib.ia_gemm_wgrad_rows_workspace_bytes(n_out, n_in, M)
+    ws = torch.empty(ws_bytes, device=dy.device, dtype=torch.uint8)
+    check(lib.ia_gemm_wgrad_rows(dy.data_ptr(), n_out, x.data_ptr(), n_in, out.data_ptr(), n_in, n_out, n_in, M, ptr(row_live),
+                                 int(accumulate), ws.data_ptr(), ws_bytes, stream_ptr()), "ia_gemm_wgrad_rows")
+    return out
+
+
 def ln_fwd(x, gamma, beta, eps, *, bias=None, residual=None, write_z=True, drop_p=0.0, seed=0, stream_id=0):
     lib = _lib.load()
     _need(x, BF16, "x"); _need(gamma, F32, "gamma"); _need(beta, F32, "beta"); _need(bias, F32, "bias"); _need(residual, BF16, "residual")
```

After: 626.1, median of 6. 1.03x the previous value.
